# openxrlab/xrslam

Hardware: AMD Instinct MI355X
Metric: frames/sec, full per-frame hot path (KLT tracker + sliding-window VI-BA), one sequence per GPU (higher is better)
Workload: dtype u8/i16 images, f32 LK with exact i64 reductions, f64 BA

## Files before the change

include/xrslam_hip.h:

```cpp
#ifndef XRSLAM_HIP_H
#define XRSLAM_HIP_H

#include <stddef.h>
#include <stdint.h>

#ifdef __cplusplus
extern "C" {
#endif

#define XRHIP_OK 0
#define XRHIP_ENODEVICE (-1)
#define XRHIP_EINVAL (-2)
#define XRHIP_EHIP (-3)
#define XRHIP_ENOMEM (-4)
#define XRHIP_EOVERFLOW (-5)
#define XRHIP_ESTATE (-6)

const char *xrhip_last_error(void);
const char *xrhip_kernel_revision(void);
int xrhip_device_count(void);
int xrhip_set_device(int device);
int xrhip_get_device(int *device);
int xrhip_bind_device(int device);

// ... 35 lines not shown
int xrhip_image_upload_scaled(xrhip_image *img, const void *pixels, int stride_bytes, int format, int bits, int limited_range,
                              int on_device, const xrhip_frame_geometry *geo);
int xrhip_image_upload_scaled_distorted(xrhip_image *img, const void *pixels, int stride_bytes, int format, int bits, int limited_range,
                                        int on_device, const xrhip_frame_geometry *geo);
int xrhip_debug_stream_span(xrhip_klt *ctx, int phase, double *ms);
int xrhip_debug_get_raw(xrhip_image *img, uint8_t *out);
int xrhip_debug_set_fused_pyramid(xrhip_klt *ctx, int on);
int xrhip_debug_get_level_padded(const xrhip_image *img, int level, uint8_t *out, int *rows, int *cols);
void xrhip_image_destroy(xrhip_image *img);

typedef struct xrhip_view_marker { int32_t x, y; uint32_t style; } xrhip_view_marker;
typedef struct xrhip_view_segment { int32_t x0, y0, x1, y1; uint32_t style; } xrhip_view_segment;
int xrhip_image_render_view(xrhip_image *img, const xrhip_view_segment *segs, int n_segs,
                            const xrhip_view_marker *markers, int n_markers,
                            const uint8_t *palette_bgr, int n_palette,
                            void *out, int stride_bytes, int channels, int on_device);
int xrhip_debug_view_timing(xrhip_klt *ctx, int enable, double *ms_sum, long long *n, int reset);

int xrhip_image_preprocess(xrhip_image *img, double clip_limit, int tiles_x, int tiles_y);

int xrhip_image_release(xrhip_image *img);

int xrhip_image_prefetch_detect(xrhip_image *img);
int xrhip_image_detect(xrhip_image *img, const double *existing_xy, int n_exist, int max_points,
                       double min_distance, double *out_xy, int *n_out);

int xrhip_image_track(const xrhip_image *cur, const xrhip_image *next, const double *curr_xy,
                      double *next_xy_inout, int has_guess, uint8_t *status, int n);

int xrhip_image_lk(const xrhip_image *prev, const xrhip_image *next, const float *prev_xy, float *next_xy_inout,
                   uint8_t *status, int n);

int xrhip_image_level_dims(const xrhip_image *img, int level, int *w, int *h);
int xrhip_image_download_level(const xrhip_image *img, int level, uint8_t *img_out, int16_t *deriv_out);
int xrhip_image_download_harris(xrhip_image *img, float *resp_out);

typedef struct xrhip_klt_stats {
    double ms_preprocess;
    double ms_track;
    double ms_detect;
    long long n_preprocess, n_track, n_detect;
    long long lk_templates;
    long long lk_iterations;
    long long lk_points;
    long long detect_full_list;
} xrhip_klt_stats;
typedef struct xrhip_lk_params { int win; int max_level; int max_count; double epsilon; } xrhip_lk_params;
int xrhip_klt_set_lk_params(xrhip_klt *ctx, const xrhip_lk_params *p);
int xrhip_klt_get_lk_params(const xrhip_klt *ctx, xrhip_lk_params *out);
int xrhip_debug_force_general_lk(xrhip_klt *ctx, int on);
int xrhip_klt_set_profiling(xrhip_klt *ctx, int enable);
int xrhip_klt_get_stats(xrhip_klt *ctx, xrhip_klt_stats *out, int reset);
int xrhip_klt_synchronize(xrhip_klt *ctx);


#define XRHIP_STATE_DIM 16
#define XRHIP_ES_DIM 15
#define XRHIP_IMU_DIM 281

#define XRHIP_FIX_POSE 1
#define XRHIP_FIX_MOTION 2

typedef struct xrhip_ba_problem {
    int n_frames;
    double *frame_state;
    const uint8_t *frame_fix;
    double cam_q_bc[4], cam_p_bc[3];
    double imu_q_bi[4], imu_p_bi[3];
    double sqrt_inv_cov[2];
    int n_landmarks;
    double *inv_depth;
    const uint8_t *landmark_fix;
    int n_obs;
    const int *obs_tgt, *obs_ref, *obs_lm;
    const double *obs_z_tgt, *obs_z_ref;
    int n_rot;
    const int *rot_tgt, *rot_ref;
    const double *rot_z_tgt, *rot_z_ref;
    int n_imu;
    const int *imu_i, *imu_j;
    const double *imu_data;
    int prior_n;
    const int *prior_frames;
    const double *prior_sqrt_info;
    const double *prior_infovec;
    const double *prior_lin;
    int max_iterations;
} xrhip_ba_problem;

#define XRHIP_BA_CONVERGENCE 0
#define XRHIP_BA_NO_CONVERGENCE 1
#define XRHIP_BA_FAILURE 2

typedef struct xrhip_ba_summary {
    int iterations;
    int successful_steps;
    int termination;
    int usable;
    double initial_cost, final_cost;
    double ms_solve;
} xrhip_ba_summary;

typedef struct xrhip_marg_problem {
    int n_frames;
    int victim;
    const double *frame_state;
    double cam_q_bc[4], cam_p_bc[3], imu_q_bi[4], imu_p_bi[3], sqrt_inv_cov[2];
    int prior_n;
    const int *prior_frames;
    const double *prior_sqrt_info, *prior_infovec, *prior_lin;
    int n_imu;
    const int *imu_i, *imu_j;
    const double *imu_data;
    int n_landmarks;
    const double *inv_depth;
    int n_obs;
    const int *obs_tgt, *obs_ref, *obs_lm;
    const double *obs_z_tgt, *obs_z_ref;
} xrhip_marg_problem;

typedef struct xrhip_ba xrhip_ba;
int xrhip_ba_create(int max_frames, int max_landmarks, int max_obs, xrhip_ba **out);
void xrhip_ba_destroy(xrhip_ba *ctx);
int xrhip_ba_solve(xrhip_ba *ctx, const xrhip_ba_problem *problem, xrhip_ba_summary *summary);
int xrhip_ba_solve_overlapped(xrhip_ba *ctx, const xrhip_ba_problem *problem, xrhip_ba_summary *summary, void (*host_work)(void *), void *arg);

int xrhip_ba_solve_chained(xrhip_ba *ctx_first, const xrhip_ba_problem *first, xrhip_ba_summary *summary_first, int link_first,
                           xrhip_ba *ctx_second, const xrhip_ba_problem *second, xrhip_ba_summary *summary_second, int link_second,
                           void (*host_work)(void *), void *arg);
int xrhip_ba_solve_begin(xrhip_ba *ctx, const xrhip_ba_problem *first);
int xrhip_ba_solve_linked(xrhip_ba *ctx_second, const xrhip_ba_problem *second, xrhip_ba_summary *summary_second, int link_second,
                          xrhip_ba *ctx_first, int link_first, void (*host_work)(void *), void *arg);
int xrhip_ba_solve_end(xrhip_ba *ctx, xrhip_ba_summary *summary);
int xrhip_ba_solve_abort(xrhip_ba *ctx);

typedef struct xrhip_ba_stats {
    long n_solve_try;
    long n_trials;
    double ms_solve_try;
    long n_timed;
    double flops_solve_try;
    long n_tiny;
    long n_chain_timed;
    double ms_chain;
    double bytes_chain;
    long n_cov_launches;
} xrhip_ba_stats;
int xrhip_ba_set_profiling(xrhip_ba *ctx, int enable);
int xrhip_ba_get_stats(xrhip_ba *ctx, xrhip_ba_stats *out, int reset);
int xrhip_ba_marginalize(xrhip_ba *ctx, const xrhip_marg_problem *problem, double *out_sqrt_info,
                         double *out_infovec, double *out_lin);
int xrhip_ba_marginalize_begin(xrhip_ba *ctx, const xrhip_marg_problem *problem);
int xrhip_ba_marginalize_end(xrhip_ba *ctx, double *out_sqrt_info, double *out_infovec, double *out_lin);
int xrhip_ba_preintegrate(xrhip_ba *ctx, const double *samples, int n, double t_end, const double *bg,
                          const double *ba, const double *noise_cov36, int compute_jacobian,
                          int compute_covariance, double *out);
int xrhip_ba_preintegrate_batch(xrhip_ba *ctx, const double *samples, const int *sample_begin,
                                const int *sample_count, const double *t_end, const double *bg, const double *ba,
                                int n_jobs, const double *noise_cov36, int compute_jacobian, int compute_covariance,
                                double *out);

int xrhip_ba_preintegrate_begin(xrhip_ba *ctx, const double *samples, const int *sample_begin, const int *sample_count,
                                const double *t_end, const double *bg, const double *ba, int n_jobs,
                                const double *noise_cov36, int compute_jacobian, int compute_covariance);
int xrhip_ba_preintegrate_end(xrhip_ba *ctx, double *out);
int xrhip_ba_preintegrate_early(xrhip_ba *ctx, int job, double *out_delta11);
int xrhip_ba_preintegrate_cancel(xrhip_ba *ctx);
int xrhip_ba_preintegrate_after_solve(xrhip_ba *ctx, const double *samples, const int *sample_begin, const int *sample_count,
                                      const double *t_end, const int *bias_frame, int n_jobs, const double *noise_cov36,
                                      int compute_jacobian, int compute_covariance);

typedef struct xrhip_group xrhip_group;
int xrhip_group_create(xrhip_group **out);
int xrhip_group_destroy(xrhip_group *group);
int xrhip_klt_join_group(xrhip_klt *ctx, xrhip_group *group);
int xrhip_ba_join_group(xrhip_ba *ctx, xrhip_group *group);
int xrhip_klt_frame_gate(xrhip_klt *ctx);
int xrhip_klt_group_busy(xrhip_klt *ctx, int busy);
#define XRHIP_GK_CALL 0
#define XRHIP_GK_UPLOAD 1
#define XRHIP_GK_PREPROCESS 2
#define XRHIP_GK_TRACK 3
#define XRHIP_GK_DETECT 4
#define XRHIP_GK_CHAIN 5
#define XRHIP_GK_PREINT 6
#define XRHIP_GK_WROUND 7
#define XRHIP_GK_WTRIALS 8
#define XRHIP_GK_GATE 11
typedef struct xrhip_group_stats {
    long long batches[12];
    long long entries[12];
    double ms[12];
    long long timed[12];
} xrhip_group_stats;
int xrhip_group_set_profiling(xrhip_group *group, int enable);
int xrhip_group_get_stats(xrhip_group *group, xrhip_group_stats *out, int reset);
int xrhip_group_queue_split(xrhip_group *group);

typedef struct xrhip_cov_request {
    int n_sel; const int *sel_frames;
    double *out_blocks;
    double *out_inv_depth_var;
    int *status;
    double *rcond_estimate;
} xrhip_cov_request;
int xrhip_ba_covariance(xrhip_ba *ctx, const xrhip_ba_problem *problem, const xrhip_cov_request *req);
int xrhip_ba_debug_cov_times(xrhip_ba *ctx, double *ms4);

int xrhip_ba_debug_linearize(xrhip_ba *ctx, const xrhip_ba_problem *problem, double *H, double *g, double *hll,
                             double *gl, double *W, double *cost);
int xrhip_ba_debug_schur(xrhip_ba *ctx, const double *W, const double *w, int L, int P, double *out);
int xrhip_ba_debug_marg_guard(xrhip_ba *ctx, double *lambda_bound, int *status8);
int xrhip_ba_debug_set_schur_precision(xrhip_ba *ctx, int mode);
int xrhip_ba_debug_last_route(xrhip_ba *ctx, int *out8);
int xrhip_study_schur_precision(const double *W, const double *w, int L, int P, int reps, double *out64, double *out32,
                                double *out16, float ms_per_launch[3]);
void xrhip_debug_kprof(long long *out32, int reset);
void xrhip_debug_lkprof(long long *out8, int reset);

#ifdef __cplusplus
}
#endif
#endif
```

xrslam_amd/abi.py:

```python
import copy
import ctypes as C

import numpy as np

STATE_DIM = 16
ES_DIM = 15
IMU_DIM = 281
FIX_POSE = 1
FIX_MOTION = 2

_dp = C.POINTER(C.c_double)
_ip = C.POINTER(C.c_int)
_bp = C.POINTER(C.c_uint8)


class BaProblem(C.Structure):
    _fields_ = [
        ("n_frames", C.c_int), ("frame_state", _dp), ("frame_fix", _bp),
        ("cam_q_bc", C.c_double * 4), ("cam_p_bc", C.c_double * 3),
        ("imu_q_bi", C.c_double * 4), ("imu_p_bi", C.c_double * 3),
        ("sqrt_inv_cov", C.c_double * 2),
        ("n_landmarks", C.c_int), ("inv_depth", _dp), ("landmark_fix", _bp),
        ("n_obs", C.c_int), ("obs_tgt", _ip), ("obs_ref", _ip), ("obs_lm", _ip),
        ("obs_z_tgt", _dp), ("obs_z_ref", _dp),
        ("n_rot", C.c_int), ("rot_tgt", _ip), ("rot_ref", _ip), ("rot_z_tgt", _dp), ("rot_z_ref", _dp),
        ("n_imu", C.c_int), ("imu_i", _ip), ("imu_j", _ip), ("imu_data", _dp),
        ("prior_n", C.c_int), ("prior_frames", _ip), ("prior_sqrt_info", _dp), ("prior_infovec", _dp),
        ("prior_lin", _dp),
        ("max_iterations", C.c_int),
    ]


class BaSummary(C.Structure):
    _fields_ = [("iterations", C.c_int), ("successful_steps", C.c_int), ("termination", C.c_int),
                ("usable", C.c_int), ("initial_cost", C.c_double), ("final_cost", C.c_double),
                ("ms_solve", C.c_double)]


class CovRequest(C.Structure):
    _fields_ = [("n_sel", C.c_int), ("sel_frames", _ip), ("out_blocks", _dp), ("out_inv_depth_var", _dp), ("status", _ip),
                ("rcond_estimate", _dp)]


class MargProblem(C.Structure):
    _fields_ = [
        ("n_frames", C.c_int), ("victim", C.c_int), ("frame_state", _dp),
        ("cam_q_bc", C.c_double * 4), ("cam_p_bc", C.c_double * 3),
        ("imu_q_bi", C.c_double * 4), ("imu_p_bi", C.c_double * 3),
        ("sqrt_inv_cov", C.c_double * 2),
        ("prior_n", C.c_int), ("prior_frames", _ip), ("prior_sqrt_info", _dp), ("prior_infovec", _dp),
        ("prior_lin", _dp),
        ("n_imu", C.c_int), ("imu_i", _ip), ("imu_j", _ip), ("imu_data", _dp),
        ("n_landmarks", C.c_int), ("inv_depth", _dp),
        ("n_obs", C.c_int), ("obs_tgt", _ip), ("obs_ref", _ip), ("obs_lm", _ip),
        ("obs_z_tgt", _dp), ("obs_z_ref", _dp),
    ]


def _arr(a, dtype):
    return np.ascontiguousarray(a, dtype=dtype)


def _dpp(a):
    return a.ctypes.data_as(_dp)


def _ipp(a):
    return a.ctypes.data_as(_ip)


class _Factors:

    def _set_obs(self, o):
        o = o or {}
        self.obs_tgt = _arr(o.get("tgt", []), np.int32)
        self.obs_ref = _arr(o.get("ref", []), np.int32)
        self.obs_lm = _arr(o.get("lm", []), np.int32)
        self.obs_z_tgt = _arr(o.get("z_tgt", np.zeros((0, 3))), np.float64).reshape(-1, 3)
        self.obs_z_ref = _arr(o.get("z_ref", np.zeros((0, 3))), np.float64).reshape(-1, 3)

    def _set_imu(self, m):
        m = m or {}
        self.imu_i = _arr(m.get("i", []), np.int32)
        self.imu_j = _arr(m.get("j", []), np.int32)
        self.imu_data = _arr(m.get("data", np.zeros((0, IMU_DIM))), np.float64).reshape(-1, IMU_DIM)

    def _set_prior(self, p):
        p = p or {}
        self.prior_frames = _arr(p.get("frames", []), np.int32)
        n = ES_DIM * len(self.prior_frames)
        self.prior_sqrt_info = _arr(p.get("sqrt_info", np.zeros((n, n))), np.float64).reshape(n, n)
        self.prior_infovec = _arr(p.get("infovec", np.zeros(n)), np.float64)
        self.prior_lin = _arr(p.get("lin", np.zeros((len(self.prior_frames), STATE_DIM))), np.float64)

    def _fill_common(self, s):
        s.cam_q_bc[:] = list(self.cam_ext[:4])
        s.cam_p_bc[:] = list(self.cam_ext[4:7])
        s.imu_q_bi[:] = list(self.imu_ext[:4])
        s.imu_p_bi[:] = list(self.imu_ext[4:7])
        s.sqrt_inv_cov[:] = list(self.sqrt_inv_cov[:2])
        s.n_obs = len(self.obs_tgt)
        s.obs_tgt, s.obs_ref, s.obs_lm = _ipp(self.obs_tgt), _ipp(self.obs_ref), _ipp(self.obs_lm)
        s.obs_z_tgt, s.obs_z_ref = _dpp(self.obs_z_tgt), _dpp(self.obs_z_ref)
        s.n_imu = len(self.imu_i)
        s.imu_i, s.imu_j, s.imu_data = _ipp(self.imu_i), _ipp(self.imu_j), _dpp(self.imu_data)
        s.prior_n = len(self.prior_frames)
        s.prior_frames = _ipp(self.prior_frames)
        s.prior_sqrt_info, s.prior_infovec = _dpp(self.prior_sqrt_info), _dpp(self.prior_infovec)
        s.prior_lin = _dpp(self.prior_lin)


class BaProblemData(_Factors):

    def __init__(self, frame_state, frame_fix, cam_ext, imu_ext, sqrt_inv_cov, inv_depth, landmark_fix=None,
                 obs=None, rot=None, imu=None, prior=None, max_iterations=30):
        self.frame_state = _arr(frame_state, np.float64).reshape(-1, STATE_DIM).copy()
        self.frame_fix = _arr(frame_fix, np.uint8).copy()
        self.cam_ext = _arr(cam_ext, np.float64)
        self.imu_ext = _arr(imu_ext, np.float64)
        self.sqrt_inv_cov = _arr(sqrt_inv_cov, np.float64)
        self.inv_depth = _arr(inv_depth, np.float64).copy()
        nl = len(self.inv_depth)
        self.landmark_fix = _arr(landmark_fix if landmark_fix is not None else np.zeros(nl), np.uint8).copy()
        self._set_obs(obs)
        r = rot or {}
        self.rot_tgt = _arr(r.get("tgt", []), np.int32)
        self.rot_ref = _arr(r.get("ref", []), np.int32)
        self.rot_z_tgt = _arr(r.get("z_tgt", np.zeros((0, 3))), np.float64).reshape(-1, 3)
        self.rot_z_ref = _arr(r.get("z_ref", np.zeros((0, 3))), np.float64).reshape(-1, 3)
        self._set_imu(imu)
        self._set_prior(prior)
        self.max_iterations = int(max_iterations)

    def copy(self):
        return copy.deepcopy(self)

    def struct(self):
        s = BaProblem()
        s.n_frames = len(self.frame_state)
        s.frame_state = _dpp(self.frame_state)
        s.frame_fix = self.frame_fix.ctypes.data_as(_bp)
        s.n_landmarks = len(self.inv_depth)
        s.inv_depth = _dpp(self.inv_depth)
        s.landmark_fix = self.landmark_fix.ctypes.data_as(_bp)
        self._fill_common(s)
        s.n_rot = len(self.rot_tgt)
        s.rot_tgt, s.rot_ref = _ipp(self.rot_tgt), _ipp(self.rot_ref)
        s.rot_z_tgt, s.rot_z_ref = _dpp(self.rot_z_tgt), _dpp(self.rot_z_ref)
        s.max_iterations = self.max_iterations
        return s


class MargProblemData(_Factors):
    def __init__(self, frame_state, victim, cam_ext, imu_ext, sqrt_inv_cov, prior, imu, inv_depth, obs):
        self.frame_state = _arr(frame_state, np.float64).reshape(-1, STATE_DIM).copy()
        self.victim = int(victim)
        self.cam_ext = _arr(cam_ext, np.float64)
        self.imu_ext = _arr(imu_ext, np.float64)
        self.sqrt_inv_cov = _arr(sqrt_inv_cov, np.float64)
        self._set_prior(prior)
        self._set_imu(imu)
        self.inv_depth = _arr(inv_depth, np.float64).copy()
        self._set_obs(obs)

    def struct(self):
        s = MargProblem()
        s.n_frames = len(self.frame_state)
        s.victim = self.victim
        s.frame_state = _dpp(self.frame_state)
        self._fill_common(s)
        s.n_landmarks = len(self.inv_depth)
        s.inv_depth = _dpp(self.inv_depth)
        return s
PIXFMT_GRAY8, PIXFMT_BGR8, PIXFMT_BGRA8, PIXFMT_RGB8, PIXFMT_RGBA8, PIXFMT_GRAY16, PIXFMT_YUYV, PIXFMT_UYVY, PIXFMT_NV12, \
    PIXFMT_I420, PIXFMT_P010 = range(11)
PIXFMT_BYTES = {PIXFMT_GRAY8: 1, PIXFMT_BGR8: 3, PIXFMT_BGRA8: 4, PIXFMT_RGB8: 3, PIXFMT_RGBA8: 4, PIXFMT_GRAY16: 2, PIXFMT_YUYV: 2,
                PIXFMT_UYVY: 2, PIXFMT_NV12: 1, PIXFMT_I420: 1, PIXFMT_P010: 2}


class FrameGeometry(C.Structure):
    _fields_ = [("src_width", C.c_int), ("src_height", C.c_int), ("crop_x", C.c_int), ("crop_y", C.c_int), ("crop_width", C.c_int),
                ("crop_height", C.c_int)]
```

xrslam_amd/ba.py:

```python
import ctypes as C

import numpy as np

from . import _lib, abi
from ._lib import check

_L = None

HOST_WORK = C.CFUNCTYPE(None, C.c_void_p)


def configure(lib):
    vp = C.c_void_p
    lib.xrhip_ba_create.argtypes = [C.c_int, C.c_int, C.c_int, C.POINTER(vp)]
    lib.xrhip_ba_destroy.argtypes = [vp]
    lib.xrhip_ba_destroy.restype = None
    lib.xrhip_ba_solve.argtypes = [vp, C.POINTER(abi.BaProblem), C.POINTER(abi.BaSummary)]
    if hasattr(lib, "xrhip_ba_solve_overlapped"):
        lib.xrhip_ba_solve_overlapped.argtypes = [vp, C.POINTER(abi.BaProblem), C.POINTER(abi.BaSummary), HOST_WORK, vp]
    if hasattr(lib, "xrhip_ba_marginalize"):
        lib.xrhip_ba_marginalize.argtypes = [vp, C.POINTER(abi.MargProblem), vp, vp, vp]
    if hasattr(lib, "xrhip_ba_marginalize_begin"):
        lib.xrhip_ba_marginalize_begin.argtypes = [vp, C.POINTER(abi.MargProblem)]
        lib.xrhip_ba_marginalize_end.argtypes = [vp, vp, vp, vp]
    if hasattr(lib, "xrhip_ba_preintegrate"):
        lib.xrhip_ba_preintegrate.argtypes = [vp, vp, C.c_int, C.c_double, vp, vp, vp, C.c_int, C.c_int, vp]
    if hasattr(lib, "xrhip_ba_preintegrate_begin"):
        lib.xrhip_ba_preintegrate_begin.argtypes = [vp, vp, vp, vp, vp, vp, vp, C.c_int, vp, C.c_int, C.c_int]
    if hasattr(lib, "xrhip_ba_preintegrate_end"):
        lib.xrhip_ba_preintegrate_end.argtypes = [vp, vp]
    if hasattr(lib, "xrhip_ba_preintegrate_early"):
        lib.xrhip_ba_preintegrate_early.argtypes = [vp, C.c_int, vp]
    if hasattr(lib, "xrhip_ba_solve_chained"):
        lib.xrhip_ba_solve_chained.argtypes = [vp, C.POINTER(abi.BaProblem), C.POINTER(abi.BaSummary), C.c_int, vp,
                                               C.POINTER(abi.BaProblem), C.POINTER(abi.BaSummary), C.c_int, HOST_WORK, vp]
    if hasattr(lib, "xrhip_ba_solve_begin"):
        lib.xrhip_ba_solve_begin.argtypes = [vp, C.POINTER(abi.BaProblem)]
        lib.xrhip_ba_solve_end.argtypes = [vp, C.POINTER(abi.BaSummary)]
        lib.xrhip_ba_solve_abort.argtypes = [vp]
    if hasattr(lib, "xrhip_ba_preintegrate_cancel"):
        lib.xrhip_ba_preintegrate_cancel.argtypes = [vp]
    if hasattr(lib, "xrhip_ba_preintegrate_after_solve"):
        lib.xrhip_ba_preintegrate_after_solve.argtypes = [vp, vp, vp, vp, vp, vp, C.c_int, vp, C.c_int, C.c_int]
    if hasattr(lib, "xrhip_ba_debug_linearize"):
        lib.xrhip_ba_debug_linearize.argtypes = [vp, C.POINTER(abi.BaProblem), vp, vp, vp, vp, vp, vp]
    if hasattr(lib, "xrhip_ba_debug_schur"):
        lib.xrhip_ba_debug_schur.argtypes = [vp, vp, vp, C.c_int, C.c_int, vp]
    if hasattr(lib, "xrhip_ba_debug_set_schur_precision"):
        lib.xrhip_ba_debug_set_schur_precision.argtypes = [vp, C.c_int]
    if hasattr(lib, "xrhip_ba_debug_last_route"):
        lib.xrhip_ba_debug_last_route.argtypes = [vp, vp]
    return lib


def L():
    global _L
    if _L is None:
        _L = configure(_lib.lib())
    return _L


def _p(a):
    return a.ctypes.data_as(C.c_void_p)


def study_schur_precision(W, w, reps=20):
    lib = L()
    W = np.ascontiguousarray(W, np.float64)
    w = np.ascontiguousarray(w, np.float64)
    Ln, P = W.shape
    outs = [np.zeros((P, P)) for _ in range(3)]
    ms = (C.c_float * 3)()
    lib.xrhip_study_schur_precision.argtypes = [C.c_void_p, C.c_void_p, C.c_int, C.c_int, C.c_int, C.c_void_p, C.c_void_p,
                                                C.c_void_p, C.POINTER(C.c_float)]
    check(lib.xrhip_study_schur_precision(_p(W), _p(w), Ln, P, int(reps), _p(outs[0]), _p(outs[1]), _p(outs[2]), ms))
    names = ("f64", "f32", "bf16")
    return dict(zip(names, outs)), dict(zip(names, [float(v) for v in ms]))


class BaContext:

    def __init__(self, max_frames=24, max_landmarks=1024, max_obs=8192, lib=None):
        self._lib = lib if lib is not None else L()
        h = C.c_void_p()
        check(self._lib.xrhip_ba_create(int(max_frames), int(max_landmarks), int(max_obs), C.byref(h)))
        self._h = h

    def close(self):
        if getattr(self, "_h", None):
            self._lib.xrhip_ba_destroy(self._h)
            self._h = None

    def __del__(self):
        try:
            self.close()
        except Exception:
            pass

    def solve(self, pd, host_work=None):
        s = pd.struct()
        sm = abi.BaSummary()
        if host_work is None:
            check(self._lib.xrhip_ba_solve(self._h, C.byref(s), C.byref(sm)))
        else:
            raised = []

            def run(_arg):
                try:
                    host_work()
                except BaseException as e:
                    raised.append(e)
            cb = HOST_WORK(run)
            rc = self._lib.xrhip_ba_solve_overlapped(self._h, C.byref(s), C.byref(sm), cb, None)
            if raised:
                raise raised[0]
            check(rc)
        return sm

    def solve_chained(self, pd_first, link_first, second_ctx, pd_second, link_second, host_work=None):
        s1, s2 = pd_first.struct(), pd_second.struct()
        m1, m2 = abi.BaSummary(), abi.BaSummary()
        raised = []

        def run(_arg):
            try:
                if host_work is not None:
                    host_work()
            except BaseException as e:
                raised.append(e)
        cb = HOST_WORK(run)
        rc = self._lib.xrhip_ba_solve_chained(self._h, C.byref(s1), C.byref(m1), int(link_first), second_ctx._h, C.byref(s2),
                                              C.byref(m2), int(link_second), cb, None)
        if raised:
            raise raised[0]
        check(rc)
        return m1, m2

    def solve_begin(self, pd):
        self._begun = (pd, pd.struct())
        rc = self._lib.xrhip_ba_solve_begin(self._h, C.byref(self._begun[1]))
        if rc < 0:
            check(rc)
        return rc == 1

    def solve_end(self):
        sm = abi.BaSummary()
        check(self._lib.xrhip_ba_solve_end(self._h, C.byref(sm)))
        self._begun = None
        return sm

    def solve_abort(self):
        check(self._lib.xrhip_ba_solve_abort(self._h))
        self._begun = None

    def preintegrate_begin(self, samples, t_end, bg, ba, noise36, jac=True, cov=True):
        samples = np.ascontiguousarray(samples, np.float64).reshape(-1, 7)
        bg, ba, noise36 = [np.ascontiguousarray(v, np.float64) for v in (bg, ba, noise36)]
        begin, count = (np.array([v], np.int32) for v in (0, len(samples)))
        t = np.array([t_end], np.float64)
        check(self._lib.xrhip_ba_preintegrate_begin(self._h, _p(samples), _p(begin), _p(count), _p(t), _p(bg), _p(ba), 1, _p(noise36),
                                                    int(jac), int(cov)))

    def preintegrate_early(self, job=0):
        out = np.zeros(11)
        check(self._lib.xrhip_ba_preintegrate_early(self._h, int(job), _p(out)))
        return out

    def marginalize(self, md):
        s = md.struct()
        k = len(md.frame_state) - 1
        n = 15 * k
        si = np.zeros((n, n))
        iv = np.zeros(n)
        lin = np.zeros((k, 16))
        check(self._lib.xrhip_ba_marginalize(self._h, C.byref(s), _p(si), _p(iv), _p(lin)))
        return si, iv, lin

    def marg_guard(self):
        lam = C.c_double()
        st = (C.c_int * 8)()
        self._lib.xrhip_ba_debug_marg_guard.argtypes = [C.c_void_p, C.POINTER(C.c_double), C.POINTER(C.c_int)]
        check(self._lib.xrhip_ba_debug_marg_guard(self._h, C.byref(lam), st))
        return lam.value, list(st)

    def marginalize_begin(self, md):
        self._marg_k = len(md.frame_state) - 1
        check(self._lib.xrhip_ba_marginalize_begin(self._h, C.byref(md.struct())))

    def marginalize_end(self):
        k = self._marg_k
        n = 15 * k
        si = np.zeros((n, n))
        iv = np.zeros(n)
        lin = np.zeros((k, 16))
        check(self._lib.xrhip_ba_marginalize_end(self._h, _p(si), _p(iv), _p(lin)))
        return si, iv, lin

    def preintegrate(self, samples, t_end, bg, ba, noise36, jac=True, cov=True):
        samples = np.ascontiguousarray(samples, np.float64).reshape(-1, 7)
        bg, ba, noise36 = [np.ascontiguousarray(v, np.float64) for v in (bg, ba, noise36)]
        out = np.zeros(abi.IMU_DIM)
        check(self._lib.xrhip_ba_preintegrate(self._h, _p(samples), len(samples), float(t_end), _p(bg), _p(ba), _p(noise36),
                                        int(jac), int(cov), _p(out)))
        return out

    def preintegrate_after_solve(self, samples, t_end, bias_frame, noise36, jac=True, cov=True):
        samples = np.ascontiguousarray(samples, np.float64).reshape(-1, 7)
        noise36 = np.ascontiguousarray(noise36, np.float64)
        begin, count, frame = (np.array([v], np.int32) for v in (0, len(samples), bias_frame))
        t = np.array([t_end], np.float64)
        check(self._lib.xrhip_ba_preintegrate_after_solve(self._h, _p(samples), _p(begin), _p(count), _p(t), _p(frame), 1, _p(noise36),
                                                    int(jac), int(cov)))

    def preintegrate_end(self, n_jobs=1):
        out = np.zeros((n_jobs, abi.IMU_DIM))
        check(self._lib.xrhip_ba_preintegrate_end(self._h, _p(out)))
        return out[0] if n_jobs == 1 else out

    def debug_linearize(self, pd):
        s = pd.struct()
        F, Ln = len(pd.frame_state), len(pd.inv_depth)
        H = np.zeros((15 * F, 15 * F))
        g = np.zeros(15 * F)
        hll = np.zeros(max(Ln, 1))
        gl = np.zeros(max(Ln, 1))
        W = np.zeros((max(Ln, 1), 6 * F))
        cost = C.c_double()
        check(self._lib.xrhip_ba_debug_linearize(self._h, C.byref(s), _p(H), _p(g), _p(hll), _p(gl), _p(W), C.byref(cost)))
        return dict(H=H, g=g, hll=hll[:Ln], gl=gl[:Ln], W=W[:Ln], cost=cost.value)

    def covariance(self, pd, sel, landmarks=False, prefill=None):
        sel = np.ascontiguousarray(sel, np.int32).reshape(-1)
        fill = np.nan if prefill is None else prefill
        blocks = np.full((len(sel), 15, 15), fill)
        var = np.full(max(len(pd.inv_depth), 1), fill) if landmarks else None
        status = np.full(1, -1, np.int32)
        rcond = np.zeros(1)
        s = pd.struct()
        rq = abi.CovRequest(len(sel), sel.ctypes.data_as(C.POINTER(C.c_int)), blocks.ctypes.data_as(C.POINTER(C.c_double)),
                            var.ctypes.data_as(C.POINTER(C.c_double)) if landmarks else None,
                            status.ctypes.data_as(C.POINTER(C.c_int)), rcond.ctypes.data_as(C.POINTER(C.c_double)))
        self._lib.xrhip_ba_covariance.argtypes = [C.c_void_p, C.POINTER(abi.BaProblem), C.POINTER(abi.CovRequest)]
        check(self._lib.xrhip_ba_covariance(self._h, C.byref(s), C.byref(rq)))
        return dict(blocks=blocks, var=var[:len(pd.inv_depth)] if landmarks else None, status=int(status[0]), rcond=float(rcond[0]))

    def stats(self, reset=False):
        from .harness.runner import BaStats
        st = BaStats()
        self._lib.xrhip_ba_get_stats.argtypes = [C.c_void_p, C.c_void_p, C.c_int]
        check(self._lib.xrhip_ba_get_stats(self._h, C.byref(st), 1 if reset else 0))
        return st

    def cov_times(self):
        out = np.zeros(4)
        self._lib.xrhip_ba_debug_cov_times.argtypes = [C.c_void_p, C.c_void_p]
        check(self._lib.xrhip_ba_debug_cov_times(self._h, _p(out)))
        return out

    ROUTES = {0: "none", 1: "tiny", 2: "chain", 3: "small_mid", 4: "multi"}

    def debug_last_route(self):
        out = np.zeros(8, np.int32)
        check(self._lib.xrhip_ba_debug_last_route(self._h, _p(out)))
        v = [int(x) for x in out]
        return dict(route=self.ROUTES[v[0]], use_lds=v[1], sred_tiled=v[2], block=v[3], wide_trials=v[4], wide_first=v[5], na=v[6],
                    F=v[7])

    def set_schur_precision(self, mode):
        check(self._lib.xrhip_ba_debug_set_schur_precision(self._h, int(mode)))

    def debug_schur(self, W, w):
        W = np.ascontiguousarray(W, np.float64)
        w = np.ascontiguousarray(w, np.float64)
        Ln, P = W.shape
        out = np.zeros((P, P))
        check(self._lib.xrhip_ba_debug_schur(self._h, _p(W), _p(w), Ln, P, _p(out)))
        return out
```

xrslam_amd/csrc/ba_api.hip:

```cpp
#include "../../include/xrslam_hip.h"
#include "ba_kernels.hip.h"
#include "ba_chain.hip.h"
#include "ba_plan.hpp"
#include "marg_kernels.hip.h"
#include "cov_kernels.hip.h"
#include "host/covariance.hpp"
#include "common.hip.h"
#include "group.hip.h"

#include <cstdlib>
#include <chrono>
#include <algorithm>
#include <cmath>
#include <cstring>
#include <limits>
#include <vector>

using namespace xrhip;

namespace {

struct Arena {
    char *dev = nullptr, *host = nullptr;
    size_t cap = 0, used = 0;
    size_t take(size_t bytes) {
        size_t off = (used + 255) & ~size_t(255);
        used = off + bytes;
        return off;
    }
};

inline int round_up(int v, int m) { return (v + m - 1) / m * m; }

struct ChainPayload {
    StageArgs stage;
    ChainArgs chain;
    size_t lds = 0;
    bool with_preint = false;
    PreintArgs preint;
};
struct ChainSubmitted {
    int seq = 0;
    hipStream_t stream = nullptr;
    GroupRequest *rq = nullptr;
    hipEvent_t e0 = nullptr, e1 = nullptr;
};
struct WindowPayload {
    WinEntry e;
    bool relin = false;
    bool with_stage = false;
    StageArgs stage;
    int np = 0;
    gptr<const double> pS, pinfo;
    gptr<double> pLam, pc0;
    size_t lds_lin = 0, lds_solve = 0, lds_wide = 0;
};

}

struct xrhip_ba {
    hipStream_t stream = nullptr;
    int device = 0;
    xrhip_group *group = nullptr;
    GroupRequest rq_chain, rq_preint, rq_window;
    WindowPayload a_window;
    ChainPayload a_chain;
    PreintArgs a_preint;
    GroupRequest *preint_rq = nullptr;
    hipStream_t preint_stream = nullptr;
    struct Begun {
        bool active = false;
        const xrhip_ba_problem *P = nullptr;
        BaDims d{};
        SolvePlan plan;
        BaPtrs p{};
        ChainSubmitted sub;
        std::chrono::steady_clock::time_point t0;
        bool handed_over = false;
        std::chrono::steady_clock::time_point t_hand;
    } begun;
    Arena in;
    char *work = nullptr;
    size_t work_cap = 0;
    char *work2 = nullptr;
    size_t work2_cap = 0;
    char *h_stage = nullptr;
    size_t h_stage_cap = 0;
    BaCtl *h_ctl = nullptr;
    int *h_seq = nullptr;
    int seq = 0;
    struct MargPending {
        bool pending = false;
        int K = 0, victim = 0, R = 0;
        std::vector<double> lin;
        int *dst = nullptr, *dsup = nullptr;
        double *lam = nullptr;
        double *As = nullptr, *bs = nullptr, *B = nullptr, *V = nullptr, *Ss = nullptr, *ivs = nullptr, *dsi = nullptr, *div = nullptr;
    } marg;
    int preint_pending = 0;
    size_t preint_o_out = 0, preint_o_st = 0;
    int preint_deferred = 0, preint_def_jac = 0, preint_def_cov = 0;
    size_t preint_o_jobs = 0, preint_o_smp = 0, preint_o_noise = 0;
    bool profiling = false;
    struct Timed {
        hipEvent_t e0, e1;
        double flops_fixed, flops_per_trial;
        int iter_before;
    };
    std::vector<Timed> pending;
    struct TimedChain {
        hipEvent_t e0, e1;
        double bytes;
    };
    std::vector<TimedChain> pending_chain;
    std::vector<std::pair<hipEvent_t, hipEvent_t>> free_events;
    xrhip_ba_stats stats = {0, 0, 0.0, 0, 0.0, 0, 0, 0.0, 0.0, 0};
    char *cov_dev = nullptr;
    size_t cov_cap = 0;
    hipEvent_t cov_ev[5] = {nullptr, nullptr, nullptr, nullptr, nullptr};
    double cov_ms[4] = {0.0, 0.0, 0.0, 0.0};
    const TinyArgs *tiny_args = nullptr;
    hipStream_t stream2 = nullptr;
    hipEvent_t ev_mid = nullptr, ev_spec = nullptr;
    hipEvent_t ev_marg = nullptr;
    char *work_spec = nullptr;
    size_t work_spec_cap = 0;
    bool spec_outstanding = false;
    long spec_launched = 0, spec_taken = 0;
    const uint4 *stage_src = nullptr;
    uint4 *stage_dst = nullptr;
    size_t stage_n16 = 0;
    void (*overlap_fn)(void *) = nullptr;
    void *overlap_arg = nullptr;
    double *h_out = nullptr;
    size_t h_out_cap = 0;
    int lds_limit = 150 * 1024;
    int schur_mode = 0;
    SolvePlan plan;
    BaDims dims{};
    BaPtrs ptrs{};
    bool have_lin = false;
};

static int ensure_arena(xrhip_ba *c, size_t in_bytes, size_t work_bytes, size_t out_doubles) {
    if (in_bytes > c->in.cap) {
        if (c->in.dev) hipFree(c->in.dev);
        if (c->in.host) hipHostFree(c->in.host);
        c->in.dev = c->in.host = nullptr;
        size_t cap = std::max(in_bytes * 2, size_t(1) << 20);
        XR_HIP(hipMalloc(&c->in.dev, cap));
        XR_HIP(hipHostMalloc(&c->in.host, cap, hipHostMallocDefault));
        c->in.cap = cap;
    }
    if (work_bytes > c->work_cap) {
        if (c->work) hipFree(c->work);
        c->work = nullptr;
        size_t cap = std::max(work_bytes * 2, size_t(1) << 20);
        XR_HIP(hipMalloc(&c->work, cap));
        c->work_cap = cap;
    }
    if (out_doubles > c->h_out_cap) {
        if (c->h_out) hipHostFree(c->h_out);
        c->h_out = nullptr;
        XR_HIP(hipHostMalloc(&c->h_out, sizeof(double) * out_doubles * 2, hipHostMallocDefault));
        c->h_out_cap = out_doubles * 2;
    }
    return XRHIP_OK;
}

static int validate(const xrhip_ba_problem *P) {
    if (!P || P->n_frames <= 0 || !P->frame_state || !P->frame_fix) return xr_fail(XRHIP_EINVAL, "xrhip_ba_solve: frames missing");
    if (P->n_landmarks < 0 || P->n_obs < 0 || P->n_rot < 0 || P->n_imu < 0 || P->prior_n < 0)
        return xr_fail(XRHIP_EINVAL, "xrhip_ba_solve: negative count");
    for (int o = 0; o < P->n_obs; ++o)
        if (P->obs_tgt[o] < 0 || P->obs_tgt[o] >= P->n_frames || P->obs_ref[o] < 0 || P->obs_ref[o] >= P->n_frames ||
            P->obs_lm[o] < 0 || P->obs_lm[o] >= P->n_landmarks || P->obs_tgt[o] == P->obs_ref[o])
            return xr_fail(XRHIP_EINVAL, "xrhip_ba_solve: observation index out of range");
    for (int o = 0; o < P->n_rot; ++o)
        if (P->rot_tgt[o] < 0 || P->rot_tgt[o] >= P->n_frames || P->rot_ref[o] < 0 || P->rot_ref[o] >= P->n_frames)
            return xr_fail(XRHIP_EINVAL, "xrhip_ba_solve: rotation factor index out of range");
    for (int k = 0; k < P->n_imu; ++k)
        if (P->imu_i[k] < 0 || P->imu_i[k] >= P->n_frames || P->imu_j[k] < 0 || P->imu_j[k] >= P->n_frames ||
            P->imu_i[k] == P->imu_j[k])
            return xr_fail(XRHIP_EINVAL, "xrhip_ba_solve: imu factor index out of range");
    for (int k = 0; k < P->prior_n; ++k)
        if (P->prior_frames[k] < 0 || P->prior_frames[k] >= P->n_frames)
            return xr_fail(XRHIP_EINVAL, "xrhip_ba_solve: prior frame index out of range");
    return XRHIP_OK;
}

static int launch_stage_copy(xrhip_ba *c, hipStream_t s) {
    const int blocks = (int)std::min<size_t>((c->stage_n16 + 255) / 256, 128);
    Batch<StageArgs> b;
    std::memset(&b, 0, sizeof(b));
    b.e[0] = StageArgs{c->stage_src, c->stage_dst, c->stage_n16};
    hipLaunchKernelGGL(kb_stage, dim3(blocks, 1, 1), dim3(256), 0, s, b);
    XR_HIP(hipGetLastError());
    return XRHIP_OK;
}

static int launch_preint_batch(GroupRequest **r, int n, hipStream_t s, hipStream_t = nullptr) {
    for (int base = 0; base < n; base += XB) {
        const int m = std::min(XB, n - base);
        Batch<PreintArgs> b;
        std::memset(&b, 0, sizeof(b));
        int most = 1;
        for (int i = 0; i < m; ++i) {
            b.e[i] = *static_cast<const PreintArgs *>(r[base + i]->payload);
            most = std::max(most, b.e[i].n_jobs);
        }
        hipLaunchKernelGGL(kp_preintegrate, dim3(most, 1, m), dim3(PI_NT), 0, s, b);
    }
    XR_HIP(hipGetLastError());
    return XRHIP_OK;
}

static int launch_chain_batch(GroupRequest **r, int n, hipStream_t s, hipStream_t = nullptr) {
    std::vector<StageArgs> stages;
    std::vector<std::pair<ChainArgs, size_t>> first, second;
    std::vector<PreintArgs> preints;
    for (int i = 0; i < n; ++i) {
        const ChainPayload &p = *static_cast<const ChainPayload *>(r[i]->payload);
        stages.push_back(p.stage);
        (p.chain.link_src ? second : first).emplace_back(p.chain, p.lds);
        if (p.with_preint) preints.push_back(p.preint);
    }
    for (size_t base = 0; base < stages.size(); base += XB) {
        const int m = (int)std::min<size_t>(XB, stages.size() - base);
        Batch<StageArgs> bs;
        std::memset(&bs, 0, sizeof(bs));
        size_t most16 = 0;
        for (int i = 0; i < m; ++i) {
            bs.e[i] = stages[base + i];
            most16 = std::max(most16, bs.e[i].n16);
        }
        hipLaunchKernelGGL(kb_stage, dim3((int)std::min<size_t>((most16 + 255) / 256, 128), 1, m), dim3(256), 0, s, bs);
    }
    for (const auto *list : {&first, &second})
        for (size_t base = 0; base < list->size(); base += XB) {
            const int m = (int)std::min<size_t>(XB, list->size() - base);
            Batch<ChainArgs> bc;
            std::memset(&bc, 0, sizeof(bc));
            size_t lds = 0;
            for (int i = 0; i < m; ++i) {
                bc.e[i] = (*list)[base + i].first;
                lds = std::max(lds, (*list)[base + i].second);
            }
            hipLaunchKernelGGL(kb_chain, dim3(1, 1, m), dim3(CHAIN_THREADS), lds, s, bc);
        }
    for (size_t base = 0; base < preints.size(); base += XB) {
        const int m = (int)std::min<size_t>(XB, preints.size() - base);
        Batch<PreintArgs> bp;
        std::memset(&bp, 0, sizeof(bp));
        int most_jobs = 1;
        for (int i = 0; i < m; ++i) {
            bp.e[i] = preints[base + i];
            most_jobs = std::max(most_jobs, bp.e[i].n_jobs);
        }
        hipLaunchKernelGGL(kp_preintegrate, dim3(most_jobs, 1, m), dim3(PI_NT), 0, s, bp);
    }
    XR_HIP(hipGetLastError());
    return XRHIP_OK;
}

static int launch_wround_batch(GroupRequest **r, int n, hipStream_t s, hipStream_t = nullptr) {
    for (int base = 0; base < n; base += XB) {
        const int m = std::min(XB, n - base);
        const WindowPayload *w[XB];
        for (int i = 0; i < m; ++i) w[i] = static_cast<const WindowPayload *>(r[base + i]->payload);
        Batch<StageArgs> bs;
        std::memset(&bs, 0, sizeof(bs));
        size_t most16 = 0;
        for (int i = 0; i < m; ++i)
            if (w[i]->with_stage) {
                bs.e[i] = w[i]->stage;
                most16 = std::max(most16, bs.e[i].n16);
            }
        if (most16) hipLaunchKernelGGL(kb_stage, dim3((int)std::min<size_t>((most16 + 255) / 256, 128), 1, m), dim3(256), 0, s, bs);
        for (int i = 0; i < m; ++i)
            if (w[i]->with_stage && w[i]->np) {
                const int np = w[i]->np;
                hipLaunchKernelGGL(kb_prior_lambda, dim3(((np + 15) / 16) * ((np + 15) / 16 + 1)), dim3(256), 0, s, np, w[i]->pS, w[i]->pLam, w[i]->pinfo,
                                   w[i]->pc0);
            }
        Batch<WinEntry> b;
        std::memset(&b, 0, sizeof(b));
        int g_lin = 0, g_lv = 0, g_asm = 0, g_sa = 0;
        size_t lds_lin = 0, lds_solve = 0, lds_wide = 0;
        for (int i = 0; i < m; ++i) {
            b.e[i] = w[i]->e;
            if (!w[i]->relin) b.e[i].g_lin = b.e[i].g_lv = b.e[i].g_asm = 0;
            g_lin = std::max(g_lin, b.e[i].g_lin);
            g_lv = std::max(g_lv, b.e[i].g_lv);
            g_asm = std::max(g_asm, b.e[i].g_asm);
            g_sa = std::max(g_sa, b.e[i].g_sa);
            lds_lin = std::max(lds_lin, w[i]->lds_lin);
            lds_solve = std::max(lds_solve, w[i]->lds_solve);
            lds_wide = std::max(lds_wide, w[i]->lds_wide);
        }
        if (g_lin) {
            hipLaunchKernelGGL(kw_lin_all, dim3(g_lin, 1, m), dim3(256), lds_lin, s, b);
            hipLaunchKernelGGL(kw_landmark_vision, dim3(std::max(g_lv, 1), 1, m), dim3(64), 0, s, b);
            hipLaunchKernelGGL(kw_assemble, dim3(std::max(g_asm, 1), 1, m), dim3(256), 0, s, b);
        }
        hipLaunchKernelGGL(kw_prepare, dim3(1, 1, m), dim3(256), 0, s, b);
        hipLaunchKernelGGL(kw_schur_aux, dim3(std::max(g_sa, 1), 1, m), dim3(256), 0, s, b);
        hipLaunchKernelGGL(kw_solve_try, dim3(1, 1, m), dim3(512), lds_solve, s, b);
        for (int i = 0; i < m; ++i) b.e[i].first = 1;
        hipLaunchKernelGGL(kw_trials_wide, dim3(WIDE_G, 1, m), dim3(256), lds_wide, s, b);
    }
    XR_HIP(hipGetLastError());
    return XRHIP_OK;
}
static int launch_wtrials_batch(GroupRequest **r, int n, hipStream_t s, hipStream_t = nullptr) {
    for (int base = 0; base < n; base += XB) {
        const int m = std::min(XB, n - base);
        Batch<WinEntry> b;
        std::memset(&b, 0, sizeof(b));
        size_t lds_wide = 0;
        for (int i = 0; i < m; ++i) {
            const WindowPayload *w = static_cast<const WindowPayload *>(r[base + i]->payload);
            b.e[i] = w->e;
            b.e[i].first = 0;
            b.e[i].mode = 0;
            lds_wide = std::max(lds_wide, w->lds_wide);
        }
        hipLaunchKernelGGL(kw_trials_wide, dim3(WIDE_G, 1, m), dim3(256), lds_wide, s, b);
    }
    XR_HIP(hipGetLastError());
    return XRHIP_OK;
}

namespace {
struct RegisterBaLaunchers {
    RegisterBaLaunchers() {
        group_register(GK_PREINT, launch_preint_batch);
        group_register(GK_CHAIN, launch_chain_batch);
        group_register(GK_WROUND, launch_wround_batch);
        group_register(GK_WTRIALS, launch_wtrials_batch);
    }
} g_register_ba_launchers;
}

static int stage_problem(xrhip_ba *c, const xrhip_ba_problem *P, BaDims &d, SolvePlan &pl, BaPtrs &p, Ext &cam, Ext &imu, bool defer_copy = false) {
    d.F = P->n_frames;
    d.n = 15 * d.F;
    d.PF = round_up(6 * d.F, 16);
    d.L = P->n_landmarks;
    d.Lp = std::max(16, round_up(d.L, 16));
    d.M = P->n_obs;
    d.MR = P->n_rot;
    d.NI = P->n_imu;
    d.NP = P->prior_n;
    d.np = 15 * d.NP;
    d.NV = d.n + d.L;
    d.robust = 1;
    d.schur_mode = c->schur_mode;
    const int F = d.F, L = d.L, M = d.M, MR = d.MR, NI = d.NI, NP = d.NP, np = d.np, n = d.n;

    std::vector<uint8_t> lact(std::max(L, 1), 0);
    for (int o = 0; o < M; ++o) lact[P->obs_lm[o]] = 1;
    for (int l = 0; l < L; ++l)
        if (P->landmark_fix && P->landmark_fix[l]) lact[l] = 0;
    std::vector<int> lm_start(L + 1, 0), lm_obs(std::max(M, 1));
    for (int o = 0; o < M; ++o) lm_start[P->obs_lm[o] + 1]++;
    for (int l = 0; l < L; ++l) lm_start[l + 1] += lm_start[l];
    {
        std::vector<int> fill(lm_start.begin(), lm_start.end() - 1);
        for (int o = 0; o < M; ++o) lm_obs[fill[P->obs_lm[o]]++] = o;
    }
    std::vector<int> pair_start((size_t)F * F + 1, 0), pair_items(std::max(4 * M, 1));
    auto pair_count = [&](int a, int b) { pair_start[(size_t)a * F + b + 1]++; };
    for (int o = 0; o < M; ++o) {
        const int t = P->obs_tgt[o], r = P->obs_ref[o];
        pair_count(t, t);
        pair_count(r, r);
        pair_count(t, r);
        pair_count(r, t);
    }
    for (size_t i = 0; i < (size_t)F * F; ++i) pair_start[i + 1] += pair_start[i];
    {
        std::vector<int> fill(pair_start.begin(), pair_start.end() - 1);
        for (int o = 0; o < M; ++o) {
            const int t = P->obs_tgt[o], r = P->obs_ref[o];
            pair_items[fill[(size_t)t * F + t]++] = (o << 1) | 0;
            pair_items[fill[(size_t)r * F + r]++] = (o << 1) | 1;
            pair_items[fill[(size_t)t * F + r]++] = (o << 1) | 0;
            pair_items[fill[(size_t)r * F + t]++] = (o << 1) | 1;
        }
    }
    std::vector<int> rotf_start(F + 1, 0), rotf_items(std::max(MR, 1));
    for (int o = 0; o < MR; ++o) rotf_start[P->rot_tgt[o] + 1]++;
    for (int f = 0; f < F; ++f) rotf_start[f + 1] += rotf_start[f];
    {
        std::vector<int> fill(rotf_start.begin(), rotf_start.end() - 1);
        for (int o = 0; o < MR; ++o) rotf_items[fill[P->rot_tgt[o]]++] = o;
    }
    std::vector<int> act_idx;
    for (int a = 0; a < 15 * F; ++a) {
        const int f = a / 15, k = a % 15;
        if (k < 6 ? !(P->frame_fix[f] & XRHIP_FIX_POSE) : !(P->frame_fix[f] & XRHIP_FIX_MOTION)) act_idx.push_back(a);
    }
    d.na = (int)act_idx.size();
    std::vector<int> act_inv((size_t)15 * F, -1);
    for (size_t i = 0; i < act_idx.size(); ++i) act_inv[act_idx[i]] = (int)i;
    d.nla = 0;
    for (int l = 0; l < L; ++l) d.nla += lact[l] ? 1 : 0;
    d.lm_rows = d.Lp;
    d.nfree = 0;
    for (int f = 0; f < F; ++f) d.nfree += (P->frame_fix[f] & 3) != 3 ? 1 : 0;
    d.nffp = 0;
    for (int o = 0; o < M; ++o)
        d.nffp += (!(P->frame_fix[P->obs_tgt[o]] & XRHIP_FIX_POSE) && !(P->frame_fix[P->obs_ref[o]] & XRHIP_FIX_POSE)) ? 1 : 0;
    std::vector<int> imuf(2 * F, -1), priorf(F, -1);
    for (int k = 0; k < NI; ++k) {
        if (imuf[2 * P->imu_j[k]] >= 0 || imuf[2 * P->imu_i[k] + 1] >= 0)
            return xr_fail(XRHIP_EINVAL, "xrhip_ba_solve: a frame may end at most one IMU factor and start at most one");
        imuf[2 * P->imu_j[k]] = k;
        imuf[2 * P->imu_i[k] + 1] = k;
    }
    for (int k = 0; k < NP; ++k) priorf[P->prior_frames[k]] = k;

    Arena &A = c->in;
    A.used = 0;
    struct Item {
        size_t off;
        const void *src;
        size_t bytes;
    };
    std::vector<Item> items;
    auto put = [&](const void *src, size_t bytes) {
        size_t off = A.take(std::max(bytes, size_t(8)));
        items.push_back({off, src, bytes});
        return off;
    };
    std::vector<double> bias_ref((size_t)6 * std::max(NI, 1));
    for (int k = 0; k < NI; ++k)
        for (int i = 0; i < 6; ++i) bias_ref[6 * k + i] = P->frame_state[16 * P->imu_i[k] + 10 + i];
    BaCtl ctl;
    std::memset(&ctl, 0, sizeof(ctl));
    ctl.radius = 1e4;
    ctl.mu = 1e-8;
    ctl.first = 1;
    ctl.linear_ok = 1;
    ctl.max_iterations = P->max_iterations;
    ctl.termination = XRHIP_BA_NO_CONVERGENCE;
    ctl.accepted_slot = -1;
    const size_t o_state = put(P->frame_state, sizeof(double) * 16 * F);
    const size_t o_fix = put(P->frame_fix, F);
    const size_t o_depth = put(P->inv_depth, sizeof(double) * L);
    const size_t o_lact = put(lact.data(), std::max(L, 1));
    const size_t o_ot = put(P->obs_tgt, sizeof(int) * M), o_or = put(P->obs_ref, sizeof(int) * M);
    const size_t o_ol = put(P->obs_lm, sizeof(int) * M);
    const size_t o_zt = put(P->obs_z_tgt, sizeof(double) * 3 * M), o_zr = put(P->obs_z_ref, sizeof(double) * 3 * M);
    const size_t o_rt = put(P->rot_tgt, sizeof(int) * MR), o_rr = put(P->rot_ref, sizeof(int) * MR);
    const size_t o_rzt = put(P->rot_z_tgt, sizeof(double) * 3 * MR), o_rzr = put(P->rot_z_ref, sizeof(double) * 3 * MR);
    const size_t o_ii = put(P->imu_i, sizeof(int) * NI), o_ij = put(P->imu_j, sizeof(int) * NI);
    const size_t o_idata = put(P->imu_data, sizeof(double) * XRHIP_IMU_DIM * NI);
    const size_t o_bref = put(bias_ref.data(), sizeof(double) * 6 * NI);
    const size_t o_pf = put(P->prior_frames, sizeof(int) * NP);
    const size_t o_pS = put(P->prior_sqrt_info, sizeof(double) * (size_t)np * np);
    const size_t o_pi = put(P->prior_infovec, sizeof(double) * np);
    const size_t o_pl = put(P->prior_lin, sizeof(double) * 16 * NP);
    const size_t o_lms = put(lm_start.data(), sizeof(int) * (L + 1)), o_lmo = put(lm_obs.data(), sizeof(int) * M);
    const size_t o_ps = put(pair_start.data(), sizeof(int) * ((size_t)F * F + 1));
    const size_t o_pit = put(pair_items.data(), sizeof(int) * 4 * M);
    const size_t o_rfs = put(rotf_start.data(), sizeof(int) * (F + 1)), o_rfi = put(rotf_items.data(), sizeof(int) * MR);
    const size_t o_imuf = put(imuf.data(), sizeof(int) * 2 * F), o_prf = put(priorf.data(), sizeof(int) * F);
    const size_t o_act = put(act_idx.data(), sizeof(int) * act_idx.size());
    const size_t o_ainv = put(act_inv.data(), sizeof(int) * act_inv.size());
    const size_t o_ctl = put(&ctl, sizeof(ctl));
    const size_t o_args = put(nullptr, sizeof(TinyArgs));
    const size_t in_bytes = A.used + 256;

    size_t w = 0;
    auto carve = [&](size_t bytes) {
        size_t off = (w + 255) & ~size_t(255);
        w = off + std::max(bytes, size_t(8));
        return off;
    };
    const size_t D8 = sizeof(double);
    const size_t w_cand = carve(D8 * 16 * F * TRY_B), w_dcand = carve(D8 * L * TRY_B);
    const size_t w_pLam = carve(D8 * (size_t)np * np), w_pc0 = carve(D8 * np);
    const size_t w_orec = carve(D8 * OREC * M), w_ocost = carve(D8 * M);
    const size_t w_rrec = carve(D8 * RREC * MR), w_rcost = carve(D8 * MR);
    const size_t w_ir = carve(D8 * 15 * NI), w_iJi = carve(D8 * 225 * NI), w_iJj = carve(D8 * 225 * NI);
    const size_t w_ic = carve(D8 * NI);
    const size_t w_pr = carve(D8 * np), w_pt = carve(D8 * np), w_pJq = carve(D8 * 9 * NP), w_pc = carve(D8 * (1 + (np + 15) / 16));
    const size_t w_H = carve(D8 * (size_t)n * n), w_g = carve(D8 * n);
    const size_t w_hll = carve(D8 * d.Lp), w_gl = carve(D8 * d.Lp), w_Wt = carve(D8 * (size_t)d.Lp * d.PF);
    const size_t w_sp = carve(D8 * n), w_sl = carve(D8 * d.Lp), w_om = carve(D8 * d.Lp);
    const size_t w_T = carve(D8 * (size_t)d.PF * d.PF), w_S = carve(D8 * (size_t)n * n);
    const size_t w_dD = carve(D8 * d.NV), w_gr = carve(D8 * d.NV), w_gn = carve(D8 * d.NV), w_gs = carve(D8 * d.NV);
    const size_t w_st = carve(D8 * d.NV), w_de = carve(D8 * d.NV * TRY_B), w_part = carve(D8 * (size_t)(aux_quad_blocks_n(d.n, std::max(d.L, 1)) + 8));
    const size_t w_wog = carve(D8 * d.PF * WOG_CH);
    const size_t w_wide = carve(D8 * WIDE_G * 4 * WIDE_B);
    const size_t w_Hv = carve(D8 * 36 * (size_t)F * F * VIS_CH), w_gv = carve(D8 * 6 * F * VIS_CH);
    int rc = ensure_arena(c, in_bytes, w + 256, (size_t)16 * F + L + 8);
    if (rc) return rc;
    for (const Item &it : items)
        if (it.bytes && it.src) std::memcpy(A.host + it.off, it.src, it.bytes);

    char *I = A.dev, *W = c->work;
    p.state = (double *)(I + o_state);
    p.cand = (double *)(W + w_cand);
    p.fix = (const uint8_t *)(I + o_fix);
    p.depth = (double *)(I + o_depth);
    p.depth_cand = (double *)(W + w_dcand);
    p.lact = (const uint8_t *)(I + o_lact);
    p.obs_tgt = (const int *)(I + o_ot);
    p.obs_ref = (const int *)(I + o_or);
    p.obs_lm = (const int *)(I + o_ol);
    p.obs_zt = (const double *)(I + o_zt);
    p.obs_zr = (const double *)(I + o_zr);
    p.rot_tgt = (const int *)(I + o_rt);
    p.rot_ref = (const int *)(I + o_rr);
    p.rot_zt = (const double *)(I + o_rzt);
    p.rot_zr = (const double *)(I + o_rzr);
    p.imu_i = (const int *)(I + o_ii);
    p.imu_j = (const int *)(I + o_ij);
    p.imu_data = (const double *)(I + o_idata);
    p.bias_ref = (double *)(I + o_bref);
    p.prior_frames = (const int *)(I + o_pf);
    p.pS = (const double *)(I + o_pS);
    p.pinfo = (const double *)(I + o_pi);
    p.plin = (const double *)(I + o_pl);
    p.pLam = (double *)(W + w_pLam);
    p.pc0 = (double *)(W + w_pc0);
    p.lm_start = (const int *)(I + o_lms);
    p.lm_obs = (const int *)(I + o_lmo);
    p.pair_start = (const int *)(I + o_ps);
    p.pair_items = (const int *)(I + o_pit);
    p.rotf_start = (const int *)(I + o_rfs);
    p.rotf_items = (const int *)(I + o_rfi);
    p.imuf = (const int *)(I + o_imuf);
    p.priorf = (const int *)(I + o_prf);
    p.act_idx = (const int *)(I + o_act);
    p.act_inv = (const int *)(I + o_ainv);
    p.Hv = (double *)(W + w_Hv);
    p.gv = (double *)(W + w_gv);
    p.orec = (double *)(W + w_orec);
    p.ocost = (double *)(W + w_ocost);
    p.rrec = (double *)(W + w_rrec);
    p.rcost = (double *)(W + w_rcost);
    p.imu_r = (double *)(W + w_ir);
    p.imu_Ji = (double *)(W + w_iJi);
    p.imu_Jj = (double *)(W + w_iJj);
    p.imu_cost = (double *)(W + w_ic);
    p.pr = (double *)(W + w_pr);
    p.pt = (double *)(W + w_pt);
    p.pJq = (double *)(W + w_pJq);
    p.pcost = (double *)(W + w_pc);
    p.Hpp = (double *)(W + w_H);
    p.gp = (double *)(W + w_g);
    p.hll = (double *)(W + w_hll);
    p.gl = (double *)(W + w_gl);
    p.Wt = (double *)(W + w_Wt);
    p.sp = (double *)(W + w_sp);
    p.sl = (double *)(W + w_sl);
    p.omega = (double *)(W + w_om);
    p.T = (double *)(W + w_T);
    p.Sred = (double *)(W + w_S);
    p.diagD = (double *)(W + w_dD);
    p.grad = (double *)(W + w_gr);
    p.gn = (double *)(W + w_gn);
    p.gs = (double *)(W + w_gs);
    p.step = (double *)(W + w_st);
    p.delta = (double *)(W + w_de);
    p.partial = (double *)(W + w_part);
    p.wog = (double *)(W + w_wog);
    p.wide_part = (double *)(W + w_wide);
    p.ctl = (BaCtl *)(I + o_ctl);
    XR_HIP(hipHostGetDevicePointer((void **)&p.host_ctl, c->h_ctl, 0));
    XR_HIP(hipHostGetDevicePointer((void **)&p.host_out, c->h_out, 0));
    XR_HIP(hipHostGetDevicePointer((void **)&p.host_seq, c->h_seq, 0));
    cam.q = Q4{P->cam_q_bc[0], P->cam_q_bc[1], P->cam_q_bc[2], P->cam_q_bc[3]};
    cam.p = V3{P->cam_p_bc[0], P->cam_p_bc[1], P->cam_p_bc[2]};
    imu.q = Q4{P->imu_q_bi[0], P->imu_q_bi[1], P->imu_q_bi[2], P->imu_q_bi[3]};
    imu.p = V3{P->imu_p_bi[0], P->imu_p_bi[1], P->imu_p_bi[2]};
    pl = plan_solve(d, (size_t)c->lds_limit, ba_switches());
    d.sred_tiled = pl.sred_tiled;
    {
        TinyArgs *ta = reinterpret_cast<TinyArgs *>(A.host + o_args);
        ta->d = d;
        ta->p = p;
        ta->cam = cam;
        ta->imu = imu;
        ta->sx = P->sqrt_inv_cov[0];
        ta->sy = P->sqrt_inv_cov[1];
        c->tiny_args = reinterpret_cast<const TinyArgs *>(I + o_args);
    }
    {
        char *host_dev = nullptr;
        XR_HIP(hipHostGetDevicePointer((void **)&host_dev, A.host, 0));
        c->stage_src = (const uint4 *)host_dev;
        c->stage_dst = (uint4 *)A.dev;
        c->stage_n16 = (in_bytes + 15) / 16;
        if (!defer_copy) return launch_stage_copy(c, c->stream);
    }
    return XRHIP_OK;
}

static int landmark_vision_blocks(const BaDims &d) { return d.lm_rows + d.F * d.F * VIS_CH; }
static int assemble_blocks(const BaDims &d) { return (d.n * d.n + 255) / 256; }
static size_t lin_all_lds(const BaDims &d) { return sizeof(double) * (size_t)std::max(d.np, 1); }
static int schur_aux_blocks(const BaDims &d) {
    const int tiles = d.PF / 16;
    const int nrest = sred_rest_blocks(d);
    return nrest + (d.nla ? tiles * tiles + aux_quad_blocks_n(d.n, d.L) + aux_wog_blocks(d.F) : aux_quad_blocks_n(d.n, d.L)) + 1;
}

static void launch_linearize(xrhip_ba *c, const BaDims &d, const SolvePlan &pl, const BaPtrs &p, const Ext &cam, const Ext &imu, double sx,
                             double sy, bool for_solver) {
    hipStream_t s = c->stream;
    hipLaunchKernelGGL(kb_lin_all, dim3(lin_all_blocks(d.M, d.MR, d.NI, d.np)), dim3(256), lin_all_lds(d), s, d, p, cam, imu, sx, sy);
    hipLaunchKernelGGL(kb_landmark_vision, dim3(landmark_vision_blocks(d)), dim3(64), 0, s, d, p);
    if (for_solver && pl.route == ROUTE_SMALL_MID) return;
    hipLaunchKernelGGL(kb_assemble, dim3(assemble_blocks(d)), dim3(256), 0, s, d, p);
    if (for_solver) hipLaunchKernelGGL(kb_prepare, dim3(1), dim3(256), 0, s, d, p);
    else hipLaunchKernelGGL(kb_sum_cost, dim3(1), dim3(256), 0, s, d, p);
}

constexpr int LINEARIZE_LAUNCHES = 4;

static void launch_schur_aux(const BaDims &d, const BaPtrs &p, hipStream_t s) {
    hipLaunchKernelGGL(kb_schur_aux, dim3(schur_aux_blocks(d)), dim3(256), 0, s, d, p);
}

static int take_event_pair(xrhip_ba *c, hipEvent_t *e0, hipEvent_t *e1) {
    if (!c->free_events.empty()) {
        *e0 = c->free_events.back().first;
        *e1 = c->free_events.back().second;
        c->free_events.pop_back();
    } else {
        XR_HIP(hipEventCreate(e0));
        XR_HIP(hipEventCreate(e1));
    }
    return XRHIP_OK;
}

static int launch_solve_try(xrhip_ba *c, const BaDims &d, const SolvePlan &pl, const BaPtrs &p, const Ext &cam, const Ext &imu, double sx,
                            double sy, bool prepare, int mode, int seq, bool skip_front = false, const BaPtrs *spec_set = nullptr) {
    const bool mark_mid = spec_set != nullptr;
    const int commit = (spec_set && skip_front) ? 1 : 0;
    double *state2 = spec_set ? static_cast<double *>(spec_set->state) : nullptr;
    double *depth2 = spec_set ? static_cast<double *>(spec_set->depth) : nullptr;
    BaCtl *ctl2 = spec_set ? static_cast<BaCtl *>(spec_set->ctl) : nullptr;
    hipStream_t s = c->stream;
    const bool mid = pl.route == ROUTE_SMALL_MID;
    if (!skip_front) {
        if (mid) hipLaunchKernelGGL(kb_small_mid, dim3(1), dim3(256), 0, s, d, p, prepare ? 0 : 1);
        if (!mid && prepare) hipLaunchKernelGGL(kb_prepare, dim3(1), dim3(256), 0, s, d, p);
        if (!mid) launch_schur_aux(d, p, s);
    }
    const size_t lds = pl.try_lds;
    const int use_lds = pl.use_lds, wide = pl.wide_trials ? 1 : 0;
    hipEvent_t e0 = nullptr, e1 = nullptr;
    if (c->profiling) {
        int rc = take_event_pair(c, &e0, &e1);
        if (rc) return rc;
        XR_HIP(hipEventRecord(e0, s));
    }
    if (pl.wide_first)
        hipLaunchKernelGGL((kb_solve_try<512, true>), dim3(1), dim3(512), lds, s, d, p, cam, imu, sx, sy, use_lds, mode, seq, 2, state2, depth2, ctl2, commit);
    else if (pl.block == 256)
        hipLaunchKernelGGL((kb_solve_try<256, false>), dim3(1), dim3(256), lds, s, d, p, cam, imu, sx, sy, use_lds, mode, seq, wide,
                           (double *)nullptr, (double *)nullptr, (BaCtl *)nullptr, 0);
    else
        hipLaunchKernelGGL((kb_solve_try<512, false>), dim3(1), dim3(512), lds, s, d, p, cam, imu, sx, sy, use_lds, mode, seq, wide,
                           (double *)nullptr, (double *)nullptr, (BaCtl *)nullptr, 0);
    XR_HIP(hipGetLastError());
    if (c->profiling) XR_HIP(hipEventRecord(e1, s));
    if (pl.wide_first) {
        hipStream_t st = s;
        if (mark_mid) {
            XR_HIP(hipEventRecord(c->ev_mid, s));
            XR_HIP(hipStreamWaitEvent(c->stream2, c->ev_mid, 0));
            st = c->stream2;
        }
        hipLaunchKernelGGL(kb_trials_wide, dim3(WIDE_G), dim3(256), pl.wide_lds, st, d, p, cam, imu, sx, sy, seq, 1, mode);
        XR_HIP(hipGetLastError());
    }
    if (c->profiling) {
        const double na = d.na;
        c->pending.push_back({e0, e1, na * na * na / 3.0 + 2.0 * na * na,
                              pl.wide_first ? 0.0 : 450.0 * d.M + 3000.0 * d.NI + 2.0 * (double)d.np * d.np, -1});
    }
    c->stats.n_solve_try++;
    return XRHIP_OK;
}

static void run_overlap(xrhip_ba *c) {
    if (!c->overlap_fn) return;
    void (*fn)(void *) = c->overlap_fn;
    c->overlap_fn = nullptr;
    fn(c->overlap_arg);
}
static int wait_mailbox(xrhip_ba *c, int seq, hipStream_t publisher = nullptr, GroupRequest *rq = nullptr) {
    run_overlap(c);
    return wait_flag(c->h_seq, seq, publisher ? publisher : c->stream, rq, "xrhip_ba_solve");
}

static long long g_kprof[32];
static void kprof_accumulate(const BaCtl &ctl, int na) {
    static const int min_na = std::getenv("XRHIP_KPROF_MIN_NA") ? std::atoi(std::getenv("XRHIP_KPROF_MIN_NA")) : 0;
    static const int max_na = std::getenv("XRHIP_KPROF_MAX_NA") ? std::atoi(std::getenv("XRHIP_KPROF_MAX_NA")) : 1 << 30;
    if (na < min_na || na > max_na) return;
    for (int i = 0; i < 31; ++i) g_kprof[i] += ctl.prof[i];
    g_kprof[31] += 1;
}

extern "C" {

static void ba_resolve_pending(xrhip_ba *c) {
    for (auto &t : c->pending) {
        float ms = 0.f;
        if (hipEventSynchronize(t.e1) == hipSuccess && hipEventElapsedTime(&ms, t.e0, t.e1) == hipSuccess) {
            c->stats.ms_solve_try += ms;
            c->stats.n_timed += 1;
            c->stats.flops_solve_try += t.flops_fixed + t.flops_per_trial * std::max(t.iter_before, 0);
        }
        c->free_events.push_back({t.e0, t.e1});
    }
    c->pending.clear();
    for (auto &t : c->pending_chain) {
        float ms = 0.f;
        if (hipEventSynchronize(t.e1) == hipSuccess && hipEventElapsedTime(&ms, t.e0, t.e1) == hipSuccess) {
            c->stats.ms_chain += ms;
            c->stats.n_chain_timed += 1;
            c->stats.bytes_chain += t.bytes;
        }
        c->free_events.push_back({t.e0, t.e1});
    }
    c->pending_chain.clear();
}

int xrhip_ba_set_profiling(xrhip_ba *c, int enable) {
    if (!c) return xr_fail(XRHIP_EINVAL, "xrhip_ba_set_profiling: null context");
    if (!enable) ba_resolve_pending(c);
    c->profiling = enable != 0;
    return XRHIP_OK;
}

int xrhip_ba_get_stats(xrhip_ba *c, xrhip_ba_stats *out, int reset) {
    if (!c || !out) return xr_fail(XRHIP_EINVAL, "xrhip_ba_get_stats: null argument");
    ba_resolve_pending(c);
    *out = c->stats;
    if (reset) c->stats = {0, 0, 0.0, 0, 0.0, 0, 0, 0.0, 0.0, 0};
    return XRHIP_OK;
}

void xrhip_debug_kprof(long long *out32, int reset) {
    for (int i = 0; i < 32; ++i) {
        if (out32) out32[i] = g_kprof[i];
        if (reset) g_kprof[i] = 0;
    }
}

int xrhip_ba_create(int max_frames, int max_landmarks, int max_obs, xrhip_ba **out) {
    if (!out || max_frames <= 0 || max_landmarks < 0 || max_obs < 0) return xr_fail(XRHIP_EINVAL, "xrhip_ba_create: bad arguments");
    int rc = xr_require_device();
    if (rc) return rc;
    xrhip_ba *c = new xrhip_ba();
    XR_HIP(hipGetDevice(&c->device));
    XR_HIP(hipStreamCreateWithFlags(&c->stream, hipStreamNonBlocking));
    XR_HIP(hipStreamCreateWithFlags(&c->stream2, hipStreamNonBlocking));
    XR_HIP(hipEventCreateWithFlags(&c->ev_mid, hipEventDisableTiming));
    XR_HIP(hipEventCreateWithFlags(&c->ev_spec, hipEventDisableTiming));
    XR_HIP(hipHostMalloc(&c->h_ctl, sizeof(BaCtl), hipHostMallocDefault));
    XR_HIP(hipHostMalloc(&c->h_seq, 64, hipHostMallocDefault));
    *c->h_seq = 0;
    XR_HIP(hipFuncSetAttribute((const void *)kb_solve_try<512, true>, hipFuncAttributeMaxDynamicSharedMemorySize, c->lds_limit));
    XR_HIP(hipFuncSetAttribute((const void *)kb_solve_try<512, false>, hipFuncAttributeMaxDynamicSharedMemorySize, c->lds_limit));
    XR_HIP(hipFuncSetAttribute((const void *)kb_solve_try<256, false>, hipFuncAttributeMaxDynamicSharedMemorySize, c->lds_limit));
    XR_HIP(hipFuncSetAttribute((const void *)kb_chain, hipFuncAttributeMaxDynamicSharedMemorySize, c->lds_limit));
    XR_HIP(hipFuncSetAttribute((const void *)kb_trials_wide, hipFuncAttributeMaxDynamicSharedMemorySize, c->lds_limit));
    XR_HIP(hipFuncSetAttribute((const void *)kw_solve_try, hipFuncAttributeMaxDynamicSharedMemorySize, c->lds_limit));
    XR_HIP(hipFuncSetAttribute((const void *)kw_trials_wide, hipFuncAttributeMaxDynamicSharedMemorySize, c->lds_limit));
    XR_HIP(hipFuncSetAttribute((const void *)km_chol, hipFuncAttributeMaxDynamicSharedMemorySize, c->lds_limit));
    XR_HIP(hipFuncSetAttribute((const void *)km_jacobi, hipFuncAttributeMaxDynamicSharedMemorySize, c->lds_limit));
    size_t in_guess = (size_t)max_obs * 96 + (size_t)max_frames * max_frames * 15 * 15 * 8 + (size_t)max_frames * 3000 + 65536;
    rc = ensure_arena(c, in_guess, in_guess * 4, (size_t)16 * max_frames + max_landmarks + 8);
    if (rc) return rc;
    *out = c;
    return XRHIP_OK;
}

int xrhip_ba_join_group(xrhip_ba *c, xrhip_group *g) {
    if (!c) return xr_fail(XRHIP_EINVAL, "xrhip_ba_join_group: null context");
    if (c->group == g) return XRHIP_OK;
    if (g && group_device(g) != c->device)
        return xr_fail(XRHIP_EINVAL, "xrhip_ba_join_group: the context and the group live on different devices");
    if (c->preint_pending) {
        if (c->preint_rq) {
            int rc = group_wait_launched(c->preint_rq);
            if (rc) return rc;
        }
        XR_HIP(hipStreamSynchronize(c->preint_stream ? c->preint_stream : c->stream));
        c->preint_rq = nullptr;
        c->preint_stream = c->stream;
    }
    XR_HIP(hipStreamSynchronize(c->stream));
    if (c->group) {
        int rc = group_drain(c->group, GQ_CHAIN, c);
        if (!rc) rc = group_drain(c->group, GQ_PREINT, c);
        if (!rc) rc = group_drain(c->group, GQ_WINDOW, c);
        if (rc) return rc;
        group_member_remove(c->group, false);
    }
    c->group = g;
    if (g) group_member_add(g, false);
    return XRHIP_OK;
}

void xrhip_ba_destroy(xrhip_ba *c) {
    if (!c) return;
    if (c->begun.active) xrhip_ba_solve_abort(c);
    if (c->group) {
        xrhip_ba_preintegrate_cancel(c);
        xrhip_ba_join_group(c, nullptr);
    }
    hipStreamSynchronize(c->stream);
    if (c->stream2) hipStreamSynchronize(c->stream2);
    if (std::getenv("XRHIP_HOSTPROF") && c->spec_launched)
        std::fprintf(stderr, "[hostprof] speculative linearisations: %ld launched, %ld taken\n", c->spec_launched, c->spec_taken);
    hipFree(c->work_spec);
    hipFree(c->cov_dev);
    for (hipEvent_t e : c->cov_ev)
        if (e) hipEventDestroy(e);
    if (c->ev_mid) hipEventDestroy(c->ev_mid);
    if (c->ev_marg) hipEventDestroy(c->ev_marg);
    if (c->ev_spec) hipEventDestroy(c->ev_spec);
    if (c->stream2) hipStreamDestroy(c->stream2);
    hipFree(c->in.dev);
    hipHostFree(c->in.host);
    hipFree(c->work);
    hipFree(c->work2);
    hipHostFree(c->h_stage);
    hipHostFree(c->h_ctl);
    hipHostFree(c->h_seq);
    ba_resolve_pending(c);
    for (auto &e : c->free_events) {
        hipEventDestroy(e.first);
        hipEventDestroy(e.second);
    }
    hipHostFree(c->h_out);
    hipStreamDestroy(c->stream);
    delete c;
}

static int preint_launch_deferred(xrhip_ba *c, const xrhip_ba_problem *P, const double *state_dev);
static int preint_fill_deferred(xrhip_ba *c, const xrhip_ba_problem *P, const double *state_dev, PreintArgs *out, bool *have);

static int ba_solve_impl(xrhip_ba *c, const xrhip_ba_problem *P, xrhip_ba_summary *summary);
int xrhip_ba_solve(xrhip_ba *c, const xrhip_ba_problem *P, xrhip_ba_summary *summary) {
    if (!c) return xr_fail(XRHIP_EINVAL, "xrhip_ba_solve: null context");
    if (c->begun.active) return xr_fail(XRHIP_ESTATE, "xrhip_ba_solve: a solve begun on this context has not been collected (xrhip_ba_solve_end)");
    const int rc = ba_solve_impl(c, P, summary);
    if (rc) c->preint_deferred = 0;
    return rc;
}
int xrhip_ba_solve_overlapped(xrhip_ba *c, const xrhip_ba_problem *P, xrhip_ba_summary *summary, void (*host_work)(void *), void *arg) {
    if (!c) return xr_fail(XRHIP_EINVAL, "xrhip_ba_solve_overlapped: null context");
    c->overlap_fn = host_work;
    c->overlap_arg = arg;
    const int rc = xrhip_ba_solve(c, P, summary);
    run_overlap(c);
    return rc;
}
static int preint_deferred_check(xrhip_ba *c, const xrhip_ba_problem *P) {
    const PreintJob *jobs = (const PreintJob *)(c->h_stage + c->preint_o_jobs);
    for (int k = 0; k < c->preint_deferred; ++k)
        if (jobs[k].bias_frame < 0 || jobs[k].bias_frame >= P->n_frames) {
            c->preint_deferred = 0;
            return xr_fail(XRHIP_EINVAL, "xrhip_ba_preintegrate_after_solve: bias frame is not a frame of the solve");
        }
    return XRHIP_OK;
}

static bool any_free_block(const xrhip_ba_problem *P) {
    for (int f = 0; f < P->n_frames; ++f)
        if ((P->frame_fix[f] & 3) != 3) return true;
    return false;
}
static bool inputs_finite(const xrhip_ba_problem *P) {
    bool ok = true;
    for (int i = 0; i < 16 * P->n_frames; ++i) ok &= std::isfinite(P->frame_state[i]);
    for (int o = 0; o < P->n_obs; ++o) ok &= std::isfinite(P->inv_depth[P->obs_lm[o]]);
    return ok;
}
static void refuse_summary(xrhip_ba_summary *sm) {
    if (!sm) return;
    std::memset(sm, 0, sizeof(*sm));
    sm->termination = XRHIP_BA_FAILURE;
    sm->usable = 0;
    sm->initial_cost = sm->final_cost = std::numeric_limits<double>::quiet_NaN();
}
static void fill_summary(const BaCtl &ctl, float ms, xrhip_ba_summary *sm) {
    if (!sm) return;
    std::memset(sm, 0, sizeof(*sm));
    sm->iterations = ctl.iteration;
    sm->successful_steps = ctl.successful_steps;
    sm->termination = ctl.termination;
    sm->usable = ctl.termination != XRHIP_BA_FAILURE;
    sm->initial_cost = ctl.initial_cost;
    sm->final_cost = ctl.x_cost;
    sm->ms_solve = ms;
}
static float ms_since(std::chrono::steady_clock::time_point t0, std::chrono::steady_clock::time_point t1 = std::chrono::steady_clock::now()) {
    return std::chrono::duration<float, std::milli>(t1 - t0).count();
}

static double chain_bytes(const BaDims &d, const BaCtl &ctl) {
    const double nf = (double)d.M + d.MR, rounds = ctl.successful_steps + 1.0, trials = ctl.iteration;
    return rounds * (384.0 * nf + 8.0 * (double)d.na * d.na + 2248.0 * d.NI) + trials * (280.0 * nf + 2248.0 * d.NI);
}

static int submit_chain(xrhip_ba *c, const xrhip_ba_problem *P, const SolvePlan &pl, const BaPtrs &p, const double *link_src, int link_dst,
                        hipStream_t own_stream, xrhip_ba *timed, ChainSubmitted *out) {
    int rc = c->group ? group_wait_launched(&c->rq_chain) : XRHIP_OK;
    if (rc) return rc;
    ChainPayload &cp = c->a_chain;
    rc = preint_fill_deferred(c, P, p.state, &cp.preint, &cp.with_preint);
    if (rc) return rc;
    ChainSubmitted sub;
    sub.seq = ++c->seq;
    cp.stage = StageArgs{c->stage_src, c->stage_dst, c->stage_n16};
    cp.chain = ChainArgs{c->tiny_args, sub.seq, 4 * (P->max_iterations + 8), pl.chain_opts, link_src, link_dst};
    cp.lds = pl.chain_lds;
    c->rq_chain.kind = GK_CHAIN;
    c->rq_chain.owner = c;
    c->rq_chain.payload = &cp;
    c->plan = pl;
    if (c->group) {
        sub.stream = group_stream(c->group, GQ_CHAIN);
        sub.rq = &c->rq_chain;
        rc = group_submit(c->group, GQ_CHAIN, &c->rq_chain);
        if (rc) return rc;
    } else {
        sub.stream = own_stream;
        if (timed->profiling) {
            rc = take_event_pair(timed, &sub.e0, &sub.e1);
            if (rc) return rc;
        }
        rc = launch_stage_copy(c, sub.stream);
        if (rc) return rc;
        Batch<ChainArgs> bc;
        std::memset(&bc, 0, sizeof(bc));
        bc.e[0] = cp.chain;
        if (sub.e0) XR_HIP(hipEventRecord(sub.e0, sub.stream));
        hipLaunchKernelGGL(kb_chain, dim3(1, 1, 1), dim3(CHAIN_THREADS), cp.lds, sub.stream, bc);
        XR_HIP(hipGetLastError());
        if (sub.e1) XR_HIP(hipEventRecord(sub.e1, sub.stream));
        if (cp.with_preint) {
            GroupRequest one;
            one.payload = &cp.preint;
            GroupRequest *pone = &one;
            rc = launch_preint_batch(&pone, 1, sub.stream);
            if (rc) return rc;
        }
    }
    if (cp.with_preint) {
        c->preint_pending = c->preint_deferred;
        c->preint_deferred = 0;
        c->preint_rq = sub.rq;
        c->preint_stream = sub.stream;
    }
    *out = sub;
    return XRHIP_OK;
}

static int collect_chain(xrhip_ba *c, const xrhip_ba_problem *P, const BaDims &d, const BaPtrs &p, const ChainSubmitted &sub, xrhip_ba *timed,
                         const char *who) {
    if (c->h_ctl->status != ST_DONE) {
        char msg[128];
        std::snprintf(msg, sizeof(msg), "%s: trust-region loop did not terminate", who);
        return xr_fail(XRHIP_ESTATE, msg);
    }
    std::memcpy(P->frame_state, c->h_out, sizeof(double) * 16 * d.F);
    const double bytes = chain_bytes(d, *c->h_ctl);
    if (sub.e0) {
        timed->pending_chain.push_back({sub.e0, sub.e1, bytes});
    } else if (c->profiling && c->group) {
        c->stats.n_chain_timed++;
        c->stats.bytes_chain += bytes;
    }
    c->stats.n_tiny++;
    kprof_accumulate(*c->h_ctl, d.na);
    c->dims = d;
    c->ptrs = p;
    c->have_lin = true;
    return XRHIP_OK;
}

int xrhip_ba_solve_begin(xrhip_ba *c, const xrhip_ba_problem *P) {
    if (!c || !P) return xr_fail(XRHIP_EINVAL, "xrhip_ba_solve_begin: null argument");
    if (c->begun.active) return xr_fail(XRHIP_ESTATE, "xrhip_ba_solve_begin: a solve is already in flight on this context");
    int rc = validate(P);
    if (rc) return rc;
    const BaSwitches &sw = ba_switches();
    if (sw.no_chained_solves || (c->group && !sw.group_chained_solves) || c->preint_deferred || !any_free_block(P) || !inputs_finite(P))
        return 0;
    xrhip_ba::Begun &B = c->begun;
    B.t0 = std::chrono::steady_clock::now();
    Ext cam, imu;
    rc = stage_problem(c, P, B.d, B.plan, B.p, cam, imu, true);
    if (rc) return rc;
    if (B.plan.route != ROUTE_CHAIN) return 0;
    rc = submit_chain(c, P, B.plan, B.p, nullptr, -1, c->stream, c, &B.sub);
    if (rc) return rc;
    B.P = P;
    B.active = true;
    B.handed_over = false;
    return 1;
}

int xrhip_ba_solve_end(xrhip_ba *c, xrhip_ba_summary *summary) {
    if (!c) return xr_fail(XRHIP_EINVAL, "xrhip_ba_solve_end: null context");
    xrhip_ba::Begun &B = c->begun;
    if (!B.active) return xr_fail(XRHIP_ESTATE, "xrhip_ba_solve_end: nothing in flight");
    B.active = false;
    int rc = wait_flag(c->h_seq, B.sub.seq, B.sub.stream, B.sub.rq, "xrhip_ba_solve_end");
    if (rc) return rc;
    rc = collect_chain(c, B.P, B.d, B.p, B.sub, c, "xrhip_ba_solve_end");
    if (rc) return rc;
    fill_summary(*c->h_ctl, B.handed_over ? ms_since(B.t0, B.t_hand) : ms_since(B.t0), summary);
    B.handed_over = false;
    return XRHIP_OK;
}

int xrhip_ba_solve_abort(xrhip_ba *c) {
    if (!c) return xr_fail(XRHIP_EINVAL, "xrhip_ba_solve_abort: null context");
    xrhip_ba::Begun &B = c->begun;
    if (!B.active) return XRHIP_OK;
    B.active = false;
    if (B.sub.rq) group_wait_launched(B.sub.rq);
    XR_HIP(hipStreamSynchronize(B.sub.stream));
    if (B.sub.e0) c->free_events.push_back({B.sub.e0, B.sub.e1});
    return XRHIP_OK;
}

int xrhip_ba_solve_linked(xrhip_ba *c2, const xrhip_ba_problem *P2, xrhip_ba_summary *s2, int link_second, xrhip_ba *c1, int link_first,
                          void (*host_work)(void *), void *arg) {
    if (!c1 || !c2 || c1 == c2 || !P2) return xr_fail(XRHIP_EINVAL, "xrhip_ba_solve_linked: two distinct contexts and a problem are needed");
    xrhip_ba::Begun &A = c1->begun;
    if (!A.active) return xr_fail(XRHIP_ESTATE, "xrhip_ba_solve_linked: the first context has no solve in flight (xrhip_ba_solve_begin)");
    int rc = validate(P2);
    if (rc) return rc;
    if (link_first < 0 || link_first >= A.d.F || link_second < 0 || link_second >= P2->n_frames)
        return xr_fail(XRHIP_EINVAL, "xrhip_ba_solve_linked: linked frame is not a frame of its problem");
    auto sequential = [&]() {
        int r = wait_flag(c1->h_seq, A.sub.seq, A.sub.stream, A.sub.rq, "xrhip_ba_solve_linked");
        if (r) return r;
        std::memcpy(P2->frame_state + 16 * (size_t)link_second, c1->h_out + 16 * (size_t)link_first, sizeof(double) * 16);
        return xrhip_ba_solve_overlapped(c2, P2, s2, host_work, arg);
    };
    if (c1->group != c2->group || c2->begun.active || !any_free_block(P2) || !inputs_finite(P2)) return sequential();
    const auto t_begin = std::chrono::steady_clock::now();
    BaDims d2;
    SolvePlan pl2;
    BaPtrs p2;
    Ext cam2, imu2;
    rc = stage_problem(c2, P2, d2, pl2, p2, cam2, imu2, true);
    if (rc) return rc;
    if (pl2.route != ROUTE_CHAIN) return sequential();
    ChainSubmitted sub;
    rc = submit_chain(c2, P2, pl2, p2, static_cast<const double *>(A.p.state) + 16 * (size_t)link_first, link_second, A.sub.stream, c1, &sub);
    if (rc) return rc;
    A.handed_over = true;
    A.t_hand = t_begin;
    if (host_work) host_work(arg);
    rc = wait_flag(c2->h_seq, sub.seq, sub.stream, sub.rq, "xrhip_ba_solve_linked");
    if (rc) return rc;
    rc = collect_chain(c2, P2, d2, p2, sub, c1, "xrhip_ba_solve_linked");
    if (rc) return rc;
    fill_summary(*c2->h_ctl, ms_since(t_begin), s2);
    return XRHIP_OK;
}

int xrhip_ba_solve_chained(xrhip_ba *c1, const xrhip_ba_problem *P1, xrhip_ba_summary *s1, int link_first, xrhip_ba *c2,
                           const xrhip_ba_problem *P2, xrhip_ba_summary *s2, int link_second, void (*host_work)(void *), void *arg) {
    if (!c1 || !c2 || c1 == c2 || !P1 || !P2) return xr_fail(XRHIP_EINVAL, "xrhip_ba_solve_chained: two distinct contexts and two problems are needed");
    int rc = validate(P1);
    if (!rc) rc = validate(P2);
    if (rc) return rc;
    if (link_first < 0 || link_first >= P1->n_frames || link_second < 0 || link_second >= P2->n_frames)
        return xr_fail(XRHIP_EINVAL, "xrhip_ba_solve_chained: linked frame is not a frame of its problem");
    const int begun = xrhip_ba_solve_begin(c1, P1);
    if (begun < 0) return begun;
    if (begun == 0) {
        rc = xrhip_ba_solve_overlapped(c1, P1, s1, host_work, arg);
        if (rc) return rc;
        std::memcpy(P2->frame_state + 16 * (size_t)link_second, P1->frame_state + 16 * (size_t)link_first, sizeof(double) * 16);
        return xrhip_ba_solve(c2, P2, s2);
    }
    rc = xrhip_ba_solve_linked(c2, P2, s2, link_second, c1, link_first, host_work, arg);
    const int rc1 = xrhip_ba_solve_end(c1, s1);
    return rc ? rc : rc1;
}

static int ba_solve_impl(xrhip_ba *c, const xrhip_ba_problem *P, xrhip_ba_summary *summary) {
    int rc = validate(P);
    if (rc) return rc;
    rc = preint_deferred_check(c, P);
    if (rc) return rc;
    c->plan = SolvePlan{};
    c->plan.F = P->n_frames;
    bool any_free = any_free_block(P);
    if (!any_free) {
        std::vector<char> used(std::max(P->n_landmarks, 1), 0);
        for (int o = 0; o < P->n_obs; ++o) used[P->obs_lm[o]] = 1;
        for (int l = 0; l < P->n_landmarks; ++l)
            if (used[l] && !(P->landmark_fix && P->landmark_fix[l])) any_free = true;
    }
    if (!any_free) {
        if (summary) {
            std::memset(summary, 0, sizeof(*summary));
            summary->termination = XRHIP_BA_CONVERGENCE;
            summary->usable = 1;
        }
        return preint_launch_deferred(c, P, nullptr);
    }
    if (!inputs_finite(P)) {
        refuse_summary(summary);
        return preint_launch_deferred(c, P, nullptr);
    }
    BaDims d;
    SolvePlan pl;
    BaPtrs p;
    Ext cam, imu;
    const auto t_begin = std::chrono::steady_clock::now();
    {
        HostProfScope hp(8, "ba_solve: stage_problem");
        rc = stage_problem(c, P, d, pl, p, cam, imu, true);
    }
    if (rc) return rc;
    HostProfScope hp_rounds(9, "ba_solve: rounds (launch+wait)");
    if (pl.route == ROUTE_CHAIN) {
        ChainSubmitted sub;
        rc = submit_chain(c, P, pl, p, nullptr, -1, c->stream, c, &sub);
        if (rc) return rc;
        rc = wait_mailbox(c, sub.seq, sub.stream, sub.rq);
        if (rc) return rc;
        rc = collect_chain(c, P, d, p, sub, c, "xrhip_ba_solve");
        if (rc) return rc;
        fill_summary(*c->h_ctl, ms_since(t_begin), summary);
        return XRHIP_OK;
    }
    c->plan = pl;
    const BaSwitches &sw = ba_switches();
    const bool wbatch = c->group && !sw.group_no_window_batch && pl.wide_first && d.nla > 0 && !sw.group_spec;
    if (!wbatch) {
        rc = launch_stage_copy(c, c->stream);
        if (rc) return rc;
    }
    if (!d.nla) d.lm_rows = 0;
    const double sx = P->sqrt_inv_cov[0], sy = P->sqrt_inv_cov[1];
    hipStream_t s = c->stream;
    if (d.np && !wbatch) hipLaunchKernelGGL(kb_prior_lambda, dim3(((d.np + 15) / 16) * ((d.np + 15) / 16 + 1)), dim3(256), 0, s, d.np, p.pS, p.pLam, p.pinfo, p.pc0);
    bool done = false, relinearise = true;
    bool wfirst = true;
    hipStream_t wstream = wbatch ? group_stream(c->group, GQ_WINDOW) : nullptr;
    auto submit_window = [&](int kind, int seq_, int mode_) -> int {
        int r = group_wait_launched(&c->rq_window);
        if (r) return r;
        WindowPayload &wp = c->a_window;
        wp.e = WinEntry{c->tiny_args, lin_all_blocks(d.M, d.MR, d.NI, d.np), landmark_vision_blocks(d), assemble_blocks(d), schur_aux_blocks(d),
                        pl.use_lds, mode_, seq_, 1};
        wp.relin = relinearise;
        wp.with_stage = wfirst;
        wp.stage = StageArgs{c->stage_src, c->stage_dst, c->stage_n16};
        wp.np = d.np;
        wp.pS = p.pS;
        wp.pLam = p.pLam;
        wp.pinfo = p.pinfo;
        wp.pc0 = p.pc0;
        wp.lds_lin = lin_all_lds(d);
        wp.lds_solve = pl.try_lds;
        wp.lds_wide = pl.wide_lds;
        c->rq_window.kind = kind;
        c->rq_window.owner = c;
        c->rq_window.payload = &wp;
        wfirst = false;
        return group_submit(c->group, GQ_WINDOW, &c->rq_window);
    };
    int mode = 1, iter_seen = 0;
    struct BusyElsewhere {
        xrhip_group *g;
        explicit BusyElsewhere(xrhip_group *gg) : g(gg) { group_busy_elsewhere(g, 1); }
        ~BusyElsewhere() { group_busy_elsewhere(g, -1); }
    } busy_elsewhere(c->group);
    if (pl.route == ROUTE_TINY) {
        const int seq = ++c->seq;
        hipLaunchKernelGGL(kb_tiny, dim3(1), dim3(256), pl.try_lds, s, c->tiny_args, pl.use_lds, seq, 4 * (P->max_iterations + 8));
        XR_HIP(hipGetLastError());
        rc = wait_mailbox(c, seq);
        if (rc) return rc;
        if (c->h_ctl->status != ST_DONE) return xr_fail(XRHIP_ESTATE, "xrhip_ba_solve: trust-region loop did not terminate");
        c->stats.n_tiny++;
        done = true;
    }
    const bool spec = !sw.no_spec && pl.wide_first && !(c->group && !sw.group_spec);
    BaPtrs p2 = p;
    if (spec) {
        const size_t extra = sizeof(double) * (16 * (size_t)d.F + (size_t)std::max(d.L, 1)) + sizeof(BaCtl) + 1024;
        if (c->work_spec_cap < c->work_cap + extra) {
            if (c->work_spec) hipFree(c->work_spec);
            c->work_spec = nullptr;
            XR_HIP(hipMalloc(&c->work_spec, c->work_cap + extra));
            c->work_spec_cap = c->work_cap + extra;
        }
        auto shift = [&](auto &member) {
            using T = std::remove_reference_t<decltype(*(static_cast<decltype(&*member)>(nullptr)))>;
            member = reinterpret_cast<T *>(c->work_spec + (reinterpret_cast<const char *>(static_cast<T *>(member)) - c->work));
        };
        shift(p2.orec); shift(p2.ocost); shift(p2.rrec); shift(p2.rcost);
        shift(p2.imu_r); shift(p2.imu_Ji); shift(p2.imu_Jj); shift(p2.imu_cost);
        shift(p2.pr); shift(p2.pt); shift(p2.pJq); shift(p2.pcost);
        shift(p2.hll); shift(p2.gl); shift(p2.Wt); shift(p2.Hv); shift(p2.gv);
        shift(p2.Hpp); shift(p2.gp); shift(p2.diagD); shift(p2.gs); shift(p2.omega);
        shift(p2.T); shift(p2.Sred); shift(p2.partial); shift(p2.wog);
        char *x = c->work_spec + ((c->work_cap + 255) & ~size_t(255));
        p2.state = reinterpret_cast<double *>(x);
        p2.depth = reinterpret_cast<double *>(x + sizeof(double) * 16 * (size_t)d.F);
        p2.ctl = reinterpret_cast<BaCtl *>(x + ((sizeof(double) * (16 * (size_t)d.F + (size_t)std::max(d.L, 1)) + 255) & ~size_t(255)));
    }
    auto swap_sets = [&]() {
        std::swap(p.orec, p2.orec); std::swap(p.ocost, p2.ocost); std::swap(p.rrec, p2.rrec); std::swap(p.rcost, p2.rcost);
        std::swap(p.imu_r, p2.imu_r); std::swap(p.imu_Ji, p2.imu_Ji); std::swap(p.imu_Jj, p2.imu_Jj); std::swap(p.imu_cost, p2.imu_cost);
        std::swap(p.pr, p2.pr); std::swap(p.pt, p2.pt); std::swap(p.pJq, p2.pJq); std::swap(p.pcost, p2.pcost);
        std::swap(p.hll, p2.hll); std::swap(p.gl, p2.gl); std::swap(p.Wt, p2.Wt); std::swap(p.Hv, p2.Hv); std::swap(p.gv, p2.gv);
        std::swap(p.Hpp, p2.Hpp); std::swap(p.gp, p2.gp); std::swap(p.diagD, p2.diagD); std::swap(p.gs, p2.gs); std::swap(p.omega, p2.omega);
        std::swap(p.T, p2.T); std::swap(p.Sred, p2.Sred); std::swap(p.partial, p2.partial); std::swap(p.wog, p2.wog);
    };
    bool spec_ready = false;
    for (int guard = 0; guard < 4 * (P->max_iterations + 8) && !done; ++guard) {
        const int seq = ++c->seq;
        if (wbatch) {
            rc = submit_window(GK_WROUND, seq, mode);
        } else if (spec_ready) {
            rc = launch_solve_try(c, d, pl, p, cam, imu, sx, sy, false, mode, seq, true, &p2);
        } else {
            if (relinearise) launch_linearize(c, d, pl, p, cam, imu, sx, sy, true);
            rc = launch_solve_try(c, d, pl, p, cam, imu, sx, sy, !relinearise, mode, seq, false, spec ? &p2 : nullptr);
        }
        if (rc) return rc;
        spec_ready = false;
        bool spec_launched = false;
        if (spec) {
            BaPtrs q = p2;
            launch_linearize(c, d, pl, q, cam, imu, sx, sy, true);
            launch_schur_aux(d, q, s);
            XR_HIP(hipGetLastError());
            spec_launched = true;
            c->spec_launched++;
        }
        rc = wbatch ? wait_mailbox(c, seq, wstream, &c->rq_window)
                    : wait_mailbox(c, seq, spec ? c->stream2 : nullptr);
        if (rc) return rc;
        const bool first_batch_accept = spec_launched && c->h_ctl->status == ST_ACCEPTED && c->h_ctl->accepted_slot == 0;
        {
            const int it_now = c->h_ctl->iteration;
            const int trials = std::max(0, it_now - iter_seen);
            iter_seen = it_now;
            c->stats.n_trials += trials;
            if (c->profiling && !wbatch && !c->pending.empty()) c->pending.back().iter_before = trials;
        }
        int st = c->h_ctl->status;
        for (int wguard = 0; st == ST_NEED_TRIALS && wguard < 64; ++wguard) {
            const int wseq = ++c->seq;
            if (wbatch) {
                rc = submit_window(GK_WTRIALS, wseq, 0);
                if (rc) return rc;
                rc = wait_mailbox(c, wseq, wstream, &c->rq_window);
            } else {
                hipLaunchKernelGGL(kb_trials_wide, dim3(WIDE_G), dim3(256), pl.wide_lds, spec ? c->stream2 : s, d, p, cam, imu, sx, sy, wseq, 0, 0);
                XR_HIP(hipGetLastError());
                rc = wait_mailbox(c, wseq, spec ? c->stream2 : nullptr);
            }
            if (rc) return rc;
            const int it_now = c->h_ctl->iteration;
            c->stats.n_trials += std::max(0, it_now - iter_seen);
            iter_seen = it_now;
            st = c->h_ctl->status;
        }
        if (st == ST_DONE) {
            done = true;
        } else if (st == ST_ACCEPTED) {
            relinearise = true;
            mode = 1;
            if (first_batch_accept) {
                swap_sets();
                spec_ready = true;
                c->spec_taken++;
            }
        } else if (st == ST_RESOLVE || st == ST_RESOLVE_INNER) {
            relinearise = false;
            mode = (st == ST_RESOLVE) ? 2 : 3;
        } else {
            return xr_fail(XRHIP_ESTATE, "xrhip_ba_solve: unexpected device status");
        }
    }
    if (!done) return xr_fail(XRHIP_ESTATE, "xrhip_ba_solve: trust-region loop did not terminate");
    std::memcpy(P->frame_state, c->h_out, sizeof(double) * 16 * d.F);
    if (d.L && d.nla) std::memcpy(P->inv_depth, c->h_out + 16 * d.F, sizeof(double) * d.L);
    rc = preint_launch_deferred(c, P, nullptr);
    if (rc) return rc;
    kprof_accumulate(*c->h_ctl, d.na);
    fill_summary(*c->h_ctl, ms_since(t_begin), summary);
    c->dims = d;
    c->ptrs = p;
    c->have_lin = true;
    return XRHIP_OK;
}

int xrhip_ba_debug_marg_guard(xrhip_ba *c, double *lambda_bound, int *status8) {
    if (!c || !lambda_bound || !status8) return xr_fail(XRHIP_EINVAL, "xrhip_ba_debug_marg_guard: null argument");
    if (c->marg.pending || !c->marg.lam) return xr_fail(XRHIP_ESTATE, "xrhip_ba_debug_marg_guard: no collected marginalisation on this context");
    XR_HIP(hipStreamSynchronize(c->stream));
    XR_HIP(hipMemcpy(lambda_bound, c->marg.lam, sizeof(double), hipMemcpyDeviceToHost));
    XR_HIP(hipMemcpy(status8, c->marg.dst, sizeof(int) * 8, hipMemcpyDeviceToHost));
    return XRHIP_OK;
}

int xrhip_ba_debug_set_schur_precision(xrhip_ba *c, int mode) {
// ... 89 lines not shown
        XR_HIP(hipStreamSynchronize(c->stream));
        if (c->cov_dev) hipFree(c->cov_dev);
        c->cov_dev = nullptr;
        c->cov_cap = 0;
        const size_t cap = std::max((w + 256) * 2, size_t(1) << 20);
        XR_HIP(hipMalloc(&c->cov_dev, cap));
        c->cov_cap = cap;
    }
    char *S = c->cov_dev;
    CovStatus *st = (CovStatus *)(S + o_st);
    double *A = (double *)(S + o_A), *Li = (double *)(S + o_Li), *ds = (double *)(S + o_ds), *B = (double *)(S + o_B);
    double *Sig = (double *)(S + o_Sig), *dout = (double *)(S + o_out), *dvar = (double *)(S + o_var);
    int *dcols = (int *)(S + o_cols);
    std::vector<int> cols(16 * (size_t)(n_sel + nt), -1);
    for (int k = 0; k < n_sel; ++k)
        for (int q = 0; q < 15; ++q) cols[16 * (size_t)k + q] = act_inv[15 * req->sel_frames[k] + q];
    for (int t = 0; t < nt; ++t)
        for (int q = 0; q < 16; ++q) cols[16 * (size_t)(n_sel + t) + q] = (16 * t + q < na) ? 16 * t + q : -1;
    hipStream_t s = c->stream;
    const bool timed = c->profiling;
    if (timed)
        for (hipEvent_t &e : c->cov_ev)
            if (!e) XR_HIP(hipEventCreate(&e));
    long launches = 1;
    XR_HIP(hipMemsetAsync(st, 0, sizeof(CovStatus), s));
    XR_HIP(hipMemcpyAsync(dcols, cols.data(), sizeof(int) * cols.size(), hipMemcpyHostToDevice, s));
    if (timed) XR_HIP(hipEventRecord(c->cov_ev[0], s));
    if (d.np) {
        hipLaunchKernelGGL(kb_prior_lambda, dim3(((d.np + 15) / 16) * ((d.np + 15) / 16 + 1)), dim3(256), 0, s, d.np, p.pS, p.pLam, p.pinfo, p.pc0);
        ++launches;
    }
    launch_linearize(c, d, pl, p, cam, imu, P->sqrt_inv_cov[0], P->sqrt_inv_cov[1], false);
    launches += LINEARIZE_LAUNCHES;
    if (d.nla) {
        hipLaunchKernelGGL(kc_weights, dim3((d.L + 255) / 256), dim3(256), 0, s, d.L, p.lact, p.hll, p.omega);
        const int tiles = d.PF / 16;
        hipLaunchKernelGGL(kb_schur_mfma, dim3(tiles * tiles), dim3(256), 0, s, d, p);
        launches += 2;
    }
    hipLaunchKernelGGL(kc_compact, dim3((unsigned)(((size_t)n16 * n16 + 255) / 256)), dim3(256), 0, s, d, p, n16, A, ds);
    if (timed) XR_HIP(hipEventRecord(c->cov_ev[1], s));
    hipLaunchKernelGGL(kc_factor, dim3(1), dim3(COV_NT), 0, s, na, n16, A, Li, st);
    if (timed) XR_HIP(hipEventRecord(c->cov_ev[2], s));
    launches += 2;
    if (full) {
        hipLaunchKernelGGL(kc_selected_inverse, dim3(nt), dim3(256), 0, s, na, n16, A, Li, ds, dcols + 16 * (size_t)n_sel, B, 1, Sig, st);
        ++launches;
        if (n_sel) {
            hipLaunchKernelGGL(kc_gather_blocks, dim3(n_sel), dim3(256), 0, s, n16, Sig, dcols, dout, st);
            ++launches;
        }
    } else {
        for (int base = 0; base < n_sel; base += SEL_BATCH) {
            hipLaunchKernelGGL(kc_selected_inverse, dim3(std::min(SEL_BATCH, n_sel - base)), dim3(256), 0, s, na, n16, A, Li, ds,
                               dcols + 16 * (size_t)base, B, 0, dout + 225 * (size_t)base, st);
            ++launches;
        }
    }
    if (timed) XR_HIP(hipEventRecord(c->cov_ev[3], s));
    if (full) {
        hipLaunchKernelGGL(kc_landmark_var, dim3((d.L + 3) / 4), dim3(64), 0, s, d, p, n16, Sig, dvar, st);
        ++launches;
    }
    if (timed) XR_HIP(hipEventRecord(c->cov_ev[4], s));
    XR_HIP(hipGetLastError());
    c->stats.n_cov_launches += launches;
    CovStatus hst;
    XR_HIP(hipMemcpyAsync(&hst, st, sizeof(CovStatus), hipMemcpyDeviceToHost, s));
    XR_HIP(hipStreamSynchronize(s));
    *req->status = hst.status ? 1 : 0;
    if (hst.status) {
        std::snprintf(xr_err_buf(), 512, "xrhip_ba_covariance: pivot %d of %d is not positive to working precision (status 1)", hst.pivot, na);
        return XRHIP_OK;
    }
    if (req->rcond_estimate) *req->rcond_estimate = hst.max_pivot > 0.0 ? hst.min_pivot / hst.max_pivot : 0.0;
    if (n_sel) XR_HIP(hipMemcpyAsync(req->out_blocks, dout, D8 * 225 * (size_t)n_sel, hipMemcpyDeviceToHost, s));
    if (full) XR_HIP(hipMemcpyAsync(req->out_inv_depth_var, dvar, D8 * d.L, hipMemcpyDeviceToHost, s));
    XR_HIP(hipStreamSynchronize(s));
    if (want_var && !full) std::memset(req->out_inv_depth_var, 0, D8 * d.L);
    if (timed) {
        float ms = 0.f;
        for (int k = 0; k < 4; ++k) {
            const int a = k == 3 ? 0 : k + 1, b = k == 3 ? 4 : k + 2;
            c->cov_ms[k] = hipEventElapsedTime(&ms, c->cov_ev[a], c->cov_ev[b]) == hipSuccess ? ms : 0.0;
        }
        if (!full) c->cov_ms[2] = 0.0;
    }
    return XRHIP_OK;
}

int xrhip_ba_debug_cov_times(xrhip_ba *c, double *ms4) {
    if (!c || !ms4) return xr_fail(XRHIP_EINVAL, "xrhip_ba_debug_cov_times: null argument");
    std::memcpy(ms4, c->cov_ms, sizeof(c->cov_ms));
    return XRHIP_OK;
}

int xrhip_ba_debug_schur(xrhip_ba *c, const double *W, const double *w, int L, int P, double *out) {
    if (!c || !W || !w || !out || L <= 0 || P <= 0) return xr_fail(XRHIP_EINVAL, "xrhip_ba_debug_schur: bad arguments");
    BaDims d;
    std::memset(&d, 0, sizeof(d));
    BaPtrs p;
    std::memset(&p, 0, sizeof(p));
    d.PF = round_up(P, 16);
    d.L = L;
    d.Lp = std::max(16, round_up(L, 16));
    std::vector<double> wt((size_t)d.Lp * d.PF, 0.0), om(d.Lp, 0.0);
    for (int l = 0; l < L; ++l) {
        om[l] = w[l];
        for (int a = 0; a < P; ++a) wt[(size_t)l * d.PF + a] = W[(size_t)l * P + a];
    }
    double *dW = nullptr, *dw = nullptr, *dT = nullptr;
    XR_HIP(hipMalloc(&dW, sizeof(double) * wt.size()));
    XR_HIP(hipMalloc(&dw, sizeof(double) * om.size()));
    XR_HIP(hipMalloc(&dT, sizeof(double) * (size_t)d.PF * d.PF));
    XR_HIP(hipMemcpy(dW, wt.data(), sizeof(double) * wt.size(), hipMemcpyHostToDevice));
    XR_HIP(hipMemcpy(dw, om.data(), sizeof(double) * om.size(), hipMemcpyHostToDevice));
    p.Wt = dW;
    p.omega = dw;
    p.T = dT;
    const int tiles = d.PF / 16;
    hipLaunchKernelGGL(kb_schur_mfma, dim3(tiles * tiles), dim3(256), 0, c->stream, d, p);
    XR_HIP(hipGetLastError());
    XR_HIP(hipStreamSynchronize(c->stream));
    std::vector<double> T((size_t)d.PF * d.PF);
    XR_HIP(hipMemcpy(T.data(), dT, sizeof(double) * T.size(), hipMemcpyDeviceToHost));
    for (int a = 0; a < P; ++a)
        for (int b = 0; b < P; ++b) out[(size_t)a * P + b] = T[(size_t)a * d.PF + b];
    hipFree(dW);
    hipFree(dw);
    hipFree(dT);
    return XRHIP_OK;
}

}

static int ensure_work2(xrhip_ba *c, size_t dev_bytes, size_t host_bytes) {
    if (dev_bytes > c->work2_cap) {
        if (c->work2) hipFree(c->work2);
        c->work2 = nullptr;
        size_t cap = std::max(dev_bytes * 2, size_t(1) << 20);
        XR_HIP(hipMalloc(&c->work2, cap));
        c->work2_cap = cap;
    }
    if (host_bytes > c->h_stage_cap) {
        if (c->h_stage) hipHostFree(c->h_stage);
        c->h_stage = nullptr;
        size_t cap = std::max(host_bytes * 2, size_t(1) << 20);
        XR_HIP(hipHostMalloc(&c->h_stage, cap, hipHostMallocDefault));
        c->h_stage_cap = cap;
    }
    return XRHIP_OK;
}

extern "C" {


static int marg_launch(xrhip_ba *c, const xrhip_marg_problem *M) {
    if (c->marg.pending) return xr_fail(XRHIP_ESTATE, "xrhip_ba_marginalize: a marginalisation is already in flight");
    if (M->n_frames < 2 || M->victim < 0 || M->victim >= M->n_frames)
        return xr_fail(XRHIP_EINVAL, "xrhip_ba_marginalize: bad frame count / victim");
    const int K = M->n_frames;
    std::vector<double> state(M->frame_state, M->frame_state + 16 * (size_t)K);
    std::vector<uint8_t> fix(K, 0);
    std::vector<double> depth(M->inv_depth, M->inv_depth + std::max(M->n_landmarks, 0));
    std::vector<uint8_t> lfix(std::max(M->n_landmarks, 1), 0);
    xrhip_ba_problem P;
    std::memset(&P, 0, sizeof(P));
    P.n_frames = K;
    P.frame_state = state.data();
    P.frame_fix = fix.data();
    std::memcpy(P.cam_q_bc, M->cam_q_bc, sizeof(P.cam_q_bc));
    std::memcpy(P.cam_p_bc, M->cam_p_bc, sizeof(P.cam_p_bc));
    std::memcpy(P.imu_q_bi, M->imu_q_bi, sizeof(P.imu_q_bi));
    std::memcpy(P.imu_p_bi, M->imu_p_bi, sizeof(P.imu_p_bi));
    std::memcpy(P.sqrt_inv_cov, M->sqrt_inv_cov, sizeof(P.sqrt_inv_cov));
    P.n_landmarks = M->n_landmarks;
    P.inv_depth = depth.data();
    P.landmark_fix = lfix.data();
    P.n_obs = M->n_obs;
    P.obs_tgt = M->obs_tgt;
    P.obs_ref = M->obs_ref;
    P.obs_lm = M->obs_lm;
    P.obs_z_tgt = M->obs_z_tgt;
    P.obs_z_ref = M->obs_z_ref;
    P.n_imu = M->n_imu;
    P.imu_i = M->imu_i;
    P.imu_j = M->imu_j;
    P.imu_data = M->imu_data;
    P.prior_n = M->prior_n;
    P.prior_frames = M->prior_frames;
    P.prior_sqrt_info = M->prior_sqrt_info;
    P.prior_infovec = M->prior_infovec;
    P.prior_lin = M->prior_lin;
    P.max_iterations = 0;
    int rc = validate(&P);
    if (rc) return rc;
    BaDims d;
    SolvePlan pl;
    BaPtrs p;
    Ext cam, imu;
    rc = stage_problem(c, &P, d, pl, p, cam, imu);
    if (rc) return rc;
    d.robust = 0;
    d.schur_mode = 0;
    const int N = d.n, R = N - 15;
    if (R > 512) return xr_fail(XRHIP_EINVAL, "xrhip_ba_marginalize: window too large");
    const size_t D8 = sizeof(double);
    size_t w = 0;
    auto carve = [&](size_t bytes) {
        size_t off = (w + 255) & ~size_t(255);
        w = off + std::max(bytes, size_t(8));
        return off;
    };
    const size_t o_Hm = carve(D8 * (size_t)N * N), o_bm = carve(D8 * N), o_T2 = carve(D8 * (size_t)R * 15);
    const size_t o_A = carve(D8 * (size_t)R * R), o_bp = carve(D8 * R), o_B = carve(D8 * (size_t)R * R);
    const size_t o_V = carve(D8 * (size_t)R * R), o_si = carve(D8 * (size_t)R * R), o_iv = carve(D8 * R);
    const size_t o_st = carve(sizeof(int) * 8), o_lam = carve(D8 * 2), o_sup = carve(sizeof(int) * (size_t)R);
    const size_t o_As = carve(D8 * (size_t)R * R), o_bs = carve(D8 * R), o_Ss = carve(D8 * (size_t)R * R), o_ivs = carve(D8 * R);
    rc = ensure_work2(c, w + 256, D8 * ((size_t)R * R + R) + 64 + sizeof(int) * 8);
    if (rc) return rc;
    char *W2 = c->work2;
    double *Hm = (double *)(W2 + o_Hm), *bm = (double *)(W2 + o_bm), *T2 = (double *)(W2 + o_T2);
    double *A = (double *)(W2 + o_A), *bp = (double *)(W2 + o_bp), *B = (double *)(W2 + o_B), *V = (double *)(W2 + o_V);
    double *dsi = (double *)(W2 + o_si), *div = (double *)(W2 + o_iv);
    int *dst = (int *)(W2 + o_st);
    hipStream_t s = c->stream;
    XR_HIP(hipMemsetAsync(dst, 0, sizeof(int) * 8, s));
    if (d.np) hipLaunchKernelGGL(kb_prior_lambda, dim3(((d.np + 15) / 16) * ((d.np + 15) / 16 + 1)), dim3(256), 0, s, d.np, p.pS, p.pLam, p.pinfo, p.pc0);
    launch_linearize(c, d, pl, p, cam, imu, M->sqrt_inv_cov[0], M->sqrt_inv_cov[1], false);
    hipLaunchKernelGGL(km_omega, dim3((std::max(d.L, 1) + 255) / 256), dim3(256), 0, s, d, p);
    const int tiles = d.PF / 16;
    hipLaunchKernelGGL(kb_schur_mfma, dim3(tiles * tiles), dim3(256), 0, s, d, p);
    hipLaunchKernelGGL(km_wog, dim3(aux_wog_blocks(d.F)), dim3(256), 0, s, d, p);
    hipLaunchKernelGGL(km_permute, dim3((N * N + 255) / 256), dim3(256), 0, s, d, p, M->victim, Hm, bm);
    hipLaunchKernelGGL(km_victim, dim3(1), dim3(256), 0, s, N, Hm, T2, dst);
    hipLaunchKernelGGL(km_complement, dim3((R * R + 255) / 256), dim3(256), 0, s, N, Hm, bm, T2, A, bp);
    double *hs = (double *)c->h_stage;
    int *dsup = (int *)(W2 + o_sup), *dsn = dst + 1;
    double *As = (double *)(W2 + o_As), *bs = (double *)(W2 + o_bs), *Ss = (double *)(W2 + o_Ss), *ivs = (double *)(W2 + o_ivs);
    const int lds_doubles = c->lds_limit / (int)D8;
    hipLaunchKernelGGL(km_support, dim3(1), dim3(512), 0, s, R, A, bp, dsup, dsn, As, bs);
    hipLaunchKernelGGL(km_chol, dim3(1), dim3(512), (size_t)c->lds_limit, s, dsn, lds_doubles, As, bs, dsup, R, dsi, div,
                       (double *)(W2 + o_lam), dst);
    XR_HIP(hipGetLastError());
    hipLaunchKernelGGL(km_jacobi, dim3(1), dim3(1024), (size_t)c->lds_limit, s, dst + 5, lds_doubles, As, bs, B, V, Ss, ivs, 60, dst + 2,
                       dsup, R, dsi, div);
    XR_HIP(hipGetLastError());
    XR_HIP(hipMemcpyAsync(hs, dsi, D8 * (size_t)R * R, hipMemcpyDeviceToHost, s));
    XR_HIP(hipMemcpyAsync(hs + (size_t)R * R, div, D8 * R, hipMemcpyDeviceToHost, s));
    XR_HIP(hipMemcpyAsync(hs + (size_t)R * R + R, dst, sizeof(int) * 8, hipMemcpyDeviceToHost, s));
    if (!c->ev_marg) XR_HIP(hipEventCreateWithFlags(&c->ev_marg, hipEventDisableTiming));
    XR_HIP(hipEventRecord(c->ev_marg, s));
    xrhip_ba::MargPending &mp = c->marg;
    mp.pending = true;
    mp.K = K;
    mp.victim = M->victim;
    mp.R = R;
    mp.lin.assign(M->frame_state, M->frame_state + 16 * (size_t)K);
    mp.dst = dst;
    mp.dsup = dsup;
    mp.lam = (double *)(W2 + o_lam);
    mp.As = As;
    mp.bs = bs;
    mp.B = B;
    mp.V = V;
    mp.Ss = Ss;
    mp.ivs = ivs;
    mp.dsi = dsi;
    mp.div = div;
    return XRHIP_OK;
}

static int marg_collect(xrhip_ba *c, double *out_sqrt_info, double *out_infovec, double *out_lin) {
    xrhip_ba::MargPending &mp = c->marg;
    if (!mp.pending) return xr_fail(XRHIP_ESTATE, "xrhip_ba_marginalize_end: nothing in flight");
    mp.pending = false;
    hipStream_t s = c->stream;
    const size_t D8 = sizeof(double);
    const int R = mp.R, K = mp.K;
    double *hs = (double *)c->h_stage;
    XR_HIP(hipEventSynchronize(c->ev_marg));
    int hst[8];
    std::memcpy(hst, hs + (size_t)R * R + R, sizeof(hst));
    if (hst[0]) return xr_fail(XRHIP_ESTATE, "xrhip_ba_marginalize: singular victim block");
    if (hst[4] && std::getenv("XRHIP_HOSTPROF"))
        std::fprintf(stderr, "[hostprof] marginalisation took the eigen path on the device: guard %s, support %d of %d, %d sweeps\n",
                     hst[3] ? "failed" : "ok", hst[1], R, hst[2]);
    if ((hst[2] != 0 || hst[3] != 0) && !hst[4]) {
        if (std::getenv("XRHIP_HOSTPROF"))
            std::fprintf(stderr, "[hostprof] marginalisation falls back to the eigen path: cholesky %s, guard %s, support %d of %d\n",
                         hst[2] ? "failed" : "ok", hst[3] ? "failed" : "ok", hst[1], R);
        const int lds_doubles = c->lds_limit / (int)D8;
        int *dsn = mp.dst + 1;
        hipLaunchKernelGGL(km_jacobi, dim3(1), dim3(1024), (size_t)c->lds_limit, s, dsn, lds_doubles, mp.As, mp.bs, mp.B, mp.V, mp.Ss,
                           mp.ivs, 60, mp.dst + 2);
        hipLaunchKernelGGL(km_expand, dim3((R * R + 255) / 256), dim3(256), 0, s, R, mp.dsup, dsn, mp.Ss, mp.ivs, mp.dsi, mp.div);
        XR_HIP(hipGetLastError());
        XR_HIP(hipMemcpyAsync(hs, mp.dsi, D8 * (size_t)R * R, hipMemcpyDeviceToHost, s));
        XR_HIP(hipMemcpyAsync(hs + (size_t)R * R, mp.div, D8 * R, hipMemcpyDeviceToHost, s));
        XR_HIP(hipStreamSynchronize(s));
    }
    std::memcpy(out_sqrt_info, hs, D8 * (size_t)R * R);
    std::memcpy(out_infovec, hs + (size_t)R * R, D8 * R);
    int j = 0;
    for (int i = 0; i < K; ++i) {
        if (i == mp.victim) continue;
        std::memcpy(out_lin + 16 * (size_t)j, mp.lin.data() + 16 * (size_t)i, D8 * 16);
        ++j;
    }
    return XRHIP_OK;
}

int xrhip_ba_marginalize(xrhip_ba *c, const xrhip_marg_problem *M, double *out_sqrt_info, double *out_infovec,
                         double *out_lin) {
    if (!c || !M || !out_sqrt_info || !out_infovec || !out_lin) return xr_fail(XRHIP_EINVAL, "xrhip_ba_marginalize: null argument");
    int rc = marg_launch(c, M);
    if (rc) return rc;
    return marg_collect(c, out_sqrt_info, out_infovec, out_lin);
}

int xrhip_ba_marginalize_begin(xrhip_ba *c, const xrhip_marg_problem *M) {
    if (!c || !M) return xr_fail(XRHIP_EINVAL, "xrhip_ba_marginalize_begin: null argument");
    return marg_launch(c, M);
}

int xrhip_ba_marginalize_end(xrhip_ba *c, double *out_sqrt_info, double *out_infovec, double *out_lin) {
    if (!c || !out_sqrt_info || !out_infovec || !out_lin) return xr_fail(XRHIP_EINVAL, "xrhip_ba_marginalize_end: null argument");
    return marg_collect(c, out_sqrt_info, out_infovec, out_lin);
}

static int preint_stage(xrhip_ba *c, const double *samples, const int *sample_begin, const int *sample_count,
                        const double *t_end, const double *bg, const double *ba, const int *bias_frame, int n_jobs,
                        const double *noise_cov36) {
    if (c->preint_pending || c->preint_deferred)
        return xr_fail(XRHIP_ESTATE, "xrhip_ba_preintegrate_begin: a batch is already in flight on this context");
    int total = 0;
    for (int k = 0; k < n_jobs; ++k) {
        if (sample_count[k] <= 0 || sample_begin[k] < 0) return xr_fail(XRHIP_EINVAL, "xrhip_ba_preintegrate: empty IMU segment");
        total = std::max(total, sample_begin[k] + sample_count[k]);
    }
    const size_t D8 = sizeof(double);
    const size_t b_jobs = sizeof(PreintJob) * n_jobs, b_smp = D8 * 7 * (size_t)total, b_noise = D8 * 36;
    const size_t o_jobs = 0, o_smp = (b_jobs + 255) & ~size_t(255), o_noise = (o_smp + b_smp + 255) & ~size_t(255);
    const size_t o_out = (o_noise + b_noise + 255) & ~size_t(255), o_st = o_out + D8 * XRHIP_IMU_DIM * (size_t)n_jobs;
    const size_t bytes = o_st + 2 * sizeof(int) * n_jobs + 256;
    int rc = ensure_work2(c, 0, bytes);
    if (rc) return rc;
    char *H = c->h_stage;
    PreintJob *jobs = (PreintJob *)(H + o_jobs);
    for (int k = 0; k < n_jobs; ++k) {
        jobs[k].sample_begin = sample_begin[k];
        jobs[k].sample_count = sample_count[k];
        jobs[k].t_end = t_end[k];
        for (int i = 0; i < 3; ++i) {
            jobs[k].bg[i] = bg ? bg[3 * k + i] : 0.0;
            jobs[k].ba[i] = ba ? ba[3 * k + i] : 0.0;
        }
        jobs[k].bias_frame = bias_frame ? bias_frame[k] : -1;
        jobs[k].pad_ = 0;
    }
    std::memcpy(H + o_smp, samples, b_smp);
    std::memcpy(H + o_noise, noise_cov36, b_noise);
    std::memset(H + o_st, 0, 2 * sizeof(int) * n_jobs);
    c->preint_o_jobs = o_jobs;
    c->preint_o_smp = o_smp;
    c->preint_o_noise = o_noise;
    c->preint_o_out = o_out;
    c->preint_o_st = o_st;
    return XRHIP_OK;
}

static int preint_args(xrhip_ba *c, int n_jobs, int jac, int cov, const double *state_dev, PreintArgs *a) {
    char *Dv = nullptr;
    XR_HIP(hipHostGetDevicePointer((void **)&Dv, c->h_stage, 0));
    *a = PreintArgs{(const PreintJob *)(Dv + c->preint_o_jobs), (const double *)(Dv + c->preint_o_smp), (const double *)(Dv + c->preint_o_noise),
                    jac ? 1 : 0, cov ? 1 : 0, (double *)(Dv + c->preint_o_out), (int *)(Dv + c->preint_o_st),
                    (int *)(Dv + c->preint_o_st) + n_jobs, state_dev, n_jobs, {}};
    const PreintJob *hj = (const PreintJob *)(c->h_stage + c->preint_o_jobs);
    for (int k = 0; k < std::min(n_jobs, PI_HEAD); ++k) a->head[k] = hj[k];
    return XRHIP_OK;
}

static int preint_launch(xrhip_ba *c, int n_jobs, int jac, int cov, const double *state_dev) {
    if (c->group) {
        int rc = group_wait_launched(&c->rq_preint);
        if (rc) return rc;
    }
    int rc = preint_args(c, n_jobs, jac, cov, state_dev, &c->a_preint);
    if (rc) return rc;
    c->rq_preint.kind = GK_PREINT;
    c->rq_preint.owner = c;
    c->rq_preint.payload = &c->a_preint;
    if (c->group) {
        rc = group_submit(c->group, GQ_PREINT, &c->rq_preint);
        c->preint_rq = &c->rq_preint;
        c->preint_stream = group_stream(c->group, GQ_PREINT);
    } else {
        GroupRequest *one = &c->rq_preint;
        rc = launch_preint_batch(&one, 1, c->stream);
        c->preint_rq = nullptr;
        c->preint_stream = c->stream;
    }
    if (rc) return rc;
    c->preint_pending = n_jobs;
    c->preint_deferred = 0;
    return XRHIP_OK;
}

static int preint_fill_deferred(xrhip_ba *c, const xrhip_ba_problem *P, const double *state_dev, PreintArgs *out, bool *have) {
    *have = false;
    if (!c->preint_deferred) return XRHIP_OK;
    int rc = preint_deferred_check(c, P);
    if (!rc) rc = preint_args(c, c->preint_deferred, c->preint_def_jac, c->preint_def_cov, state_dev, out);
    if (rc) return rc;
    *have = true;
    return XRHIP_OK;
}

static int preint_launch_deferred(xrhip_ba *c, const xrhip_ba_problem *P, const double *state_dev) {
    if (!c->preint_deferred) return XRHIP_OK;
    const int rc = preint_deferred_check(c, P);
    if (rc) return rc;
    const int n_jobs = c->preint_deferred;
    PreintJob *jobs = (PreintJob *)(c->h_stage + c->preint_o_jobs);
    for (int k = 0; k < n_jobs; ++k) {
        const int f = jobs[k].bias_frame;
        if (!state_dev) {
            for (int i = 0; i < 3; ++i) {
                jobs[k].bg[i] = P->frame_state[16 * f + 10 + i];
                jobs[k].ba[i] = P->frame_state[16 * f + 13 + i];
            }
            jobs[k].bias_frame = -1;
        }
    }
    return preint_launch(c, n_jobs, c->preint_def_jac, c->preint_def_cov, state_dev);
}

int xrhip_ba_preintegrate_begin(xrhip_ba *c, const double *samples, const int *sample_begin, const int *sample_count,
                                const double *t_end, const double *bg, const double *ba, int n_jobs,
                                const double *noise_cov36, int compute_jacobian, int compute_covariance) {
    if (!c || !samples || !sample_begin || !sample_count || !t_end || !bg || !ba || !noise_cov36 || n_jobs <= 0)
        return xr_fail(XRHIP_EINVAL, "xrhip_ba_preintegrate: bad arguments");
    int rc = preint_stage(c, samples, sample_begin, sample_count, t_end, bg, ba, nullptr, n_jobs, noise_cov36);
    if (rc) return rc;
    return preint_launch(c, n_jobs, compute_jacobian, compute_covariance, nullptr);
}

int xrhip_ba_preintegrate_after_solve(xrhip_ba *c, const double *samples, const int *sample_begin, const int *sample_count,
                                      const double *t_end, const int *bias_frame, int n_jobs, const double *noise_cov36,
                                      int compute_jacobian, int compute_covariance) {
    if (!c || !samples || !sample_begin || !sample_count || !t_end || !bias_frame || !noise_cov36 || n_jobs <= 0)
        return xr_fail(XRHIP_EINVAL, "xrhip_ba_preintegrate_after_solve: bad arguments");
    for (int k = 0; k < n_jobs; ++k)
        if (bias_frame[k] < 0) return xr_fail(XRHIP_EINVAL, "xrhip_ba_preintegrate_after_solve: negative bias frame");
    int rc = preint_stage(c, samples, sample_begin, sample_count, t_end, nullptr, nullptr, bias_frame, n_jobs, noise_cov36);
    if (rc) return rc;
    c->preint_deferred = n_jobs;
    c->preint_def_jac = compute_jacobian ? 1 : 0;
    c->preint_def_cov = compute_covariance ? 1 : 0;
    return XRHIP_OK;
}

int xrhip_ba_preintegrate_cancel(xrhip_ba *c) {
    if (!c) return xr_fail(XRHIP_EINVAL, "xrhip_ba_preintegrate_cancel: null context");
    if (c->preint_pending) {
        if (c->preint_rq) group_wait_launched(c->preint_rq);
        XR_HIP(hipStreamSynchronize(c->preint_stream ? c->preint_stream : c->stream));
        c->preint_pending = 0;
    }
    c->preint_deferred = 0;
    return XRHIP_OK;
}

int xrhip_ba_preintegrate_early(xrhip_ba *c, int job, double *out_delta11) {
    if (!c || !out_delta11 || job < 0) return xr_fail(XRHIP_EINVAL, "xrhip_ba_preintegrate_early: bad arguments");
    if (!c->preint_pending || job >= c->preint_pending)
        return xr_fail(XRHIP_ESTATE, "xrhip_ba_preintegrate_early: no such job in flight");
    char *H = c->h_stage;
    const int n_jobs = c->preint_pending;
    volatile int *early = (volatile int *)(H + c->preint_o_st) + n_jobs;
    if (c->preint_rq) {
// ... 60 lines not shown
```

xrslam_amd/csrc/host/map.hpp:

```cpp
#pragma once
#include <deque>
#include <functional>
#include <map>
#include <memory>
#include <optional>
#include <vector>

#include "../../../include/xrslam_hip.h"
#include "geometry.hpp"

namespace xrh {

inline constexpr size_t nil() { return size_t(-1); }

struct ImuData {
    double t;
    V3 w, a;
};

enum FrameTag { FT_KEYFRAME = 0, FT_NO_TRANSLATION, FT_FIX_POSE, FT_FIX_MOTION, FT_COUNT };
enum TrackTag { TT_VALID = 0, TT_TRIANGULATED, TT_FIX_INVD, TT_TRASH, TT_STATIC, TT_OUTLIER, TT_TEMP, TT_COUNT };

struct Extrinsic {
    Quat q_cs;
// ... 40 lines not shown
    size_t frame = 0, track = 0;
};

class Frame {
  public:
    size_t id = 0;
    unsigned long ba_gen = 0;
    int ba_index = -1;
    bool tags[FT_COUNT] = {false, false, false, false};
    Map *map = nullptr;
    Intrinsics K;
    double sqrt_inv_cov[2] = {1, 1};
    std::shared_ptr<HipImage> image;
    PoseState pose;
    MotionState motion;
    Extrinsic camera, imu;
    PreInt preintegration, keyframe_preintegration;
    std::vector<std::unique_ptr<Frame>> subframes;
    std::vector<V3> bearings;
    std::vector<Track *> tracks;

    bool &tag(FrameTag t) { return tags[t]; }
    bool tag(FrameTag t) const { return tags[t]; }
    size_t keypoint_num() const { return bearings.size(); }
    const V3 &get_keypoint(size_t i) const { return bearings[i]; }
    Track *get_track(size_t i) const { return tracks[i]; }
    Track *get_track(size_t i, Map *allocation_map);
    void append_keypoint(const V3 &b) {
        bearings.push_back(b);
        tracks.push_back(nullptr);
    }
    std::unique_ptr<Frame> clone() const {
        auto f = std::make_unique<Frame>();
        f->id = id;
        for (int i = 0; i < FT_COUNT; ++i) f->tags[i] = tags[i];
        f->K = K;
        f->sqrt_inv_cov[0] = sqrt_inv_cov[0];
        f->sqrt_inv_cov[1] = sqrt_inv_cov[1];
        f->image = image;
        f->pose = pose;
        f->motion = motion;
        f->camera = camera;
        f->imu = imu;
        f->preintegration = preintegration;
        f->bearings = bearings;
        f->tracks.assign(bearings.size(), nullptr);
        return f;
    }
    PoseState get_pose(const Extrinsic &s) const { return {pose.q * s.q_cs, pose.p + pose.q * s.p_cs}; }
    void set_pose(const Extrinsic &s, const PoseState &ps) {
        pose.q = ps.q * s.q_cs.conjugate();
        pose.p = ps.p - pose.q * s.p_cs;
    }
};

struct FrameIdLess {
    bool operator()(const Frame *a, const Frame *b) const { return a->id < b->id; }
};

class FrameRefs {
  public:
    using value_type = std::pair<Frame *, size_t>;
    using const_iterator = std::vector<value_type>::const_iterator;
    const_iterator begin() const { return v_.begin(); }
    const_iterator end() const { return v_.end(); }
    size_t size() const { return v_.size(); }
    bool empty() const { return v_.empty(); }
    const_iterator find(Frame *f) const {
        auto it = lower(f);
        return (it != v_.end() && !FrameIdLess()(f, it->first)) ? it : v_.end();
    }
    size_t count(Frame *f) const { return find(f) != v_.end() ? 1 : 0; }
    size_t at(Frame *f) const {
        auto it = find(f);
        if (it == v_.end()) throw std::out_of_range("FrameRefs::at");
        return it->second;
    }
    size_t &operator[](Frame *f) {
        auto it = v_.begin() + (lower(f) - v_.begin());
        if (it == v_.end() || FrameIdLess()(f, it->first)) it = v_.insert(it, value_type(f, 0));
        return it->second;
    }
    void erase(Frame *f) {
        auto it = find(f);
        if (it != v_.end()) v_.erase(v_.begin() + (it - v_.begin()));
    }

  private:
    const_iterator lower(Frame *f) const {
        return std::lower_bound(v_.begin(), v_.end(), f, [](const value_type &a, Frame *b) { return FrameIdLess()(a.first, b); });
    }
    std::vector<value_type> v_;
};

struct LandmarkState {
    double inv_depth = 0, reprojection_error = 0;
};

class Track {
  public:
    size_t id = 0;
    unsigned long ba_gen = 0;
    int ba_index = -1;
    unsigned long visit_gen = 0;
    bool tags[TT_COUNT] = {false, false, false, false, true, false, false};
    size_t map_index = 0;
    Map *map = nullptr;
    LandmarkState landmark;
    size_t m_life = 0;
    FrameRefs keypoint_refs;

    bool &tag(TrackTag t) { return tags[t]; }
    bool tag(TrackTag t) const { return tags[t]; }
    bool all_tagged(std::initializer_list<TrackTag> ts) const {
        for (TrackTag t : ts)
            if (!tags[t]) return false;
        return true;
    }
    size_t keypoint_num() const { return keypoint_refs.size(); }
    std::pair<Frame *, size_t> first_keypoint() const { return *keypoint_refs.begin(); }
    Frame *first_frame() const { return keypoint_refs.begin()->first; }
    bool has_keypoint(Frame *f) const { return keypoint_refs.count(f) > 0; }
    size_t get_keypoint_index(Frame *f) const {
        auto it = keypoint_refs.find(f);
        return it == keypoint_refs.end() ? nil() : it->second;
    }
    void add_keypoint(Frame *frame, size_t keypoint_index) {
        keypoint_refs[frame] = keypoint_index;
        frame->tracks[keypoint_index] = this;
        if (tag(TT_TRIANGULATED)) m_life++;
        else m_life = 1;
    }
    void remove_keypoint(Frame *frame, bool suicide_if_empty = true);
    std::optional<V3> triangulate();
    V3 get_landmark_point() const {
        auto [frame, ki] = first_keypoint();
        PoseState cam = frame->get_pose(frame->camera);
        return cam.q * frame->get_keypoint(ki) / landmark.inv_depth + cam.p;
    }
    void set_landmark_point(const V3 &p) {
        auto [frame, ki] = first_keypoint();
        (void)ki;
        PoseState cam = frame->get_pose(frame->camera);
        landmark.inv_depth = 1.0 / norm(cam.q.conjugate() * (p - cam.p));
    }
};

struct MargPrior {
    std::vector<Frame *> frames;
    std::vector<double> lin;
    std::vector<double> sqrt_info;
    std::vector<double> infovec;
    bool pending = false;
};

class Map {
  public:
    explicit Map(IdSource *ids) : ids_(ids) {}
    size_t frame_num() const { return frames.size(); }
    Frame *get_frame(size_t i) const { return frames[i].get(); }
    void attach_frame(std::unique_ptr<Frame> frame, size_t position = nil()) {
        frame->map = this;
        if (position == nil()) frames.emplace_back(std::move(frame));
        else frames.emplace(frames.begin() + position, std::move(frame));
    }
    std::unique_ptr<Frame> detach_frame(size_t index) {
        std::unique_ptr<Frame> f = std::move(frames[index]);
        frames.erase(frames.begin() + index);
        f->map = nullptr;
        return f;
    }
    void untrack_frame(Frame *frame) {
        for (size_t i = 0; i < frame->keypoint_num(); ++i)
            if (Track *t = frame->get_track(i)) t->remove_keypoint(frame);
    }
    void erase_frame(size_t index) {
        untrack_frame(frames[index].get());
        detach_frame(index);
    }
    size_t frame_index_by_id(size_t id) const {
        auto it = std::lower_bound(frames.begin(), frames.end(), id,
                                   [](const std::unique_ptr<Frame> &f, size_t v) { return f->id < v; });
        if (it == frames.end() || id < (*it)->id) return nil();
        return (size_t)std::distance(frames.begin(), it);
    }
    size_t track_num() const { return tracks.size(); }
    Track *get_track(size_t i) const { return tracks[i].get(); }
    Track *create_track() {
        auto t = std::make_unique<Track>();
        t->id = ++ids_->track;
        t->map_index = tracks.size();
        t->map = this;
        tracks.emplace_back(std::move(t));
        return tracks.back().get();
    }
    void recycle_track(Track *track) {
        if (track->map_index != tracks.back()->map_index) {
            tracks[track->map_index].swap(tracks.back());
            tracks[track->map_index]->map_index = track->map_index;
        }
        tracks.pop_back();
    }
    void erase_track(Track *track) {
        while (track->keypoint_num() > 0) track->remove_keypoint(track->keypoint_refs.begin()->first, false);
        recycle_track(track);
    }
    void prune_tracks(const std::function<bool(const Track *)> &cond) {
        std::vector<Track *> victims;
        for (size_t i = 0; i < track_num(); ++i)
            if (cond(get_track(i))) victims.push_back(get_track(i));
        for (Track *t : victims) erase_track(t);
    }
    IdSource *ids() const { return ids_; }

    std::unique_ptr<MargPrior> marginalization_factor;
    std::deque<std::unique_ptr<Frame>> frames;
    std::vector<std::unique_ptr<Track>> tracks;

  private:
    IdSource *ids_;
};

inline Track *Frame::get_track(size_t i, Map *allocation_map) {
    if (!allocation_map) allocation_map = map;
    if (tracks[i] == nullptr) {
        Track *t = allocation_map->create_track();
        t->add_keypoint(this, i);
    }
    return tracks[i];
}

inline void Track::remove_keypoint(Frame *frame, bool suicide_if_empty) {
    size_t ki = keypoint_refs.at(frame);
    std::optional<V3> lm;
    if (frame == first_frame()) lm = get_landmark_point();
    frame->tracks[ki] = nullptr;
    keypoint_refs.erase(frame);
    if (!keypoint_refs.empty()) {
        if (lm.has_value()) set_landmark_point(lm.value());
    } else {
        tag(TT_VALID) = false;
        if (suicide_if_empty) map->recycle_track(this);
    }
}

inline std::optional<V3> Track::triangulate() {
    std::vector<P34> Ps;
    std::vector<V3> zs;
    for (const auto &[frame, ki] : keypoint_refs) {
        PoseState pose = frame->get_pose(frame->camera);
        M3 R = to_matrix(pose.q.conjugate());
        V3 T = -(R * pose.p);
        P34 P;
        for (int r = 0; r < 3; ++r) {
            for (int c = 0; c < 3; ++c) P.m[4 * r + c] = R(r, c);
            P.m[4 * r + 3] = T[r];
        }
        Ps.push_back(P);
        zs.push_back(frame->get_keypoint(ki));
    }
    auto h = triangulate_point(Ps, zs);
    for (size_t i = 0; i < zs.size(); ++i) {
        const double q2 = Ps[i].m[8] * h[0] + Ps[i].m[9] * h[1] + Ps[i].m[10] * h[2] + Ps[i].m[11] * h[3];
        if (!(q2 * h[3] > 0)) return {};
    }
    m_life = 1;
    return V3{h[0] / h[3], h[1] / h[3], h[2] / h[3]};
}

}
```

xrslam_amd/csrc/host/pipeline.hpp:

```cpp
#pragma once
#include <chrono>
#include <climits>
#include <algorithm>
#include <cstdio>
#include <cstring>
#include <atomic>
#include <condition_variable>
#include <deque>
#include <exception>
#include <functional>
#include <mutex>
#include <optional>
#include <stdexcept>
#include <thread>
#include <tuple>
#include <unordered_map>
#include <unordered_set>

#include "../host_select.hpp"
#include "../hostprof.hpp"
#include "ba_dump.hpp"
#include "config.hpp"
#include "covariance.hpp"
#include "map.hpp"
#include "parsac.hpp"
#include "pixel_format.hpp"
#include "two_view.hpp"
#include "undistort_map.hpp"

extern "C" {
int xrhip_image_upload_color(xrhip_image *img, const void *pixels, int stride_bytes, int channels, int on_device) __attribute__((weak));
int xrhip_image_upload_color_distorted(xrhip_image *img, const void *pixels, int stride_bytes, int channels, int on_device) __attribute__((weak));
int xrhip_image_upload_format(xrhip_image *img, const void *pixels, int stride_bytes, int format, int bits, int limited_range, int on_device) __attribute__((weak));
int xrhip_image_upload_format_distorted(xrhip_image *img, const void *pixels, int stride_bytes, int format, int bits, int limited_range, int on_device) __attribute__((weak));
int xrhip_image_upload_scaled(xrhip_image *img, const void *pixels, int stride_bytes, int format, int bits, int limited_range, int on_device, const xrhip_frame_geometry *geo) __attribute__((weak));
int xrhip_image_upload_scaled_distorted(xrhip_image *img, const void *pixels, int stride_bytes, int format, int bits, int limited_range, int on_device, const xrhip_frame_geometry *geo) __attribute__((weak));
int xrhip_image_render_view(xrhip_image *img, const xrhip_view_segment *segs, int n_segs, const xrhip_view_marker *markers, int n_markers,
                            const uint8_t *palette_bgr, int n_palette, void *out, int stride_bytes, int channels, int on_device) __attribute__((weak));
int xrhip_klt_set_lk_params(xrhip_klt *ctx, const xrhip_lk_params *p) __attribute__((weak));
int xrhip_ba_covariance(xrhip_ba *ctx, const xrhip_ba_problem *problem, const xrhip_cov_request *req) __attribute__((weak));
}

namespace xrh {
inline bool have_format_upload() { return xrhip_image_upload_format != nullptr && xrhip_image_upload_format_distorted != nullptr; }
inline bool have_scaled_upload() { return xrhip_image_upload_scaled != nullptr && xrhip_image_upload_scaled_distorted != nullptr; }
inline bool have_color_upload() { return xrhip_image_upload_color != nullptr && xrhip_image_upload_color_distorted != nullptr; }

struct FrameInput {
    const uint8_t *pixels = nullptr;
    int stride = 0;
    bool on_device = false;
    int channels = 1;
    bool by_format = false;
    int format = XRHIP_PIXFMT_GRAY8, bits = 0, limited_range = 0;
    const xrhip_frame_geometry *geo = nullptr;
};

struct HipError : std::runtime_error {
    explicit HipError(const std::string &m) : std::runtime_error(m) {}
};
inline void hip_check(int rc, const char *what) {
    if (rc != 0) throw HipError(std::string(what) + ": " + xrhip_last_error());
}

struct StageTimes {
    double tracker = 0, localize = 0, refine = 0, marginalize = 0, preintegrate = 0;
    long frames = 0, solves = 0, solve_iterations = 0, marginalizations = 0, keyframes = 0;
    double ba_device_ms = 0;
    double w_upload = 0, w_preprocess = 0, w_track = 0, w_detect = 0, w_preintegrate = 0, w_solve = 0, w_marginalize = 0,
           w_frame = 0;
    double w_preintegrate_ft = 0;
    double w_join = 0;
    double scope[16] = {0};
};
enum { SC_FT_TRACK = 0, SC_RANSAC_E, SC_RANSAC_R, SC_FT_DETECT, SC_MIRROR, SC_LOCALIZE, SC_MANAGE_KF, SC_TRACK_LANDMARK,
       SC_REFINE_WINDOW, SC_SLIDE_WINDOW, SC_REFINE_SUBWINDOW, SC_INITIALIZE, SC_RD_JUDGED, SC_RD_OUTLIERS, SC_CONST_COPIES, SC_COUNT };
struct WallTimer {
    double &slot;
    std::chrono::steady_clock::time_point t0 = std::chrono::steady_clock::now();
    explicit WallTimer(double &s) : slot(s) {}
    ~WallTimer() { slot += std::chrono::duration<double>(std::chrono::steady_clock::now() - t0).count(); }
};

class JobThread {
  public:
    explicit JobThread(int device) : device_(device), th_([this] { loop(); }) {}
    ~JobThread() {
        {
            const int s = state_.load(std::memory_order_acquire);
            if (s == POSTED) await([this] { return state_.load(std::memory_order_acquire) == DONE; }, 20000);
        }
        state_.store(QUIT, std::memory_order_release);
        {
            std::lock_guard<std::mutex> lk(m_);
        }
        cv_.notify_all();
        th_.join();
    }
    JobThread(const JobThread &) = delete;
    JobThread &operator=(const JobThread &) = delete;
    void post(std::function<void()> job) {
        job_ = std::move(job);
        error_ = nullptr;
        state_.store(POSTED, std::memory_order_release);
        {
            std::lock_guard<std::mutex> lk(m_);
        }
        cv_.notify_all();
    }
    void wait() {
        await([this] { return state_.load(std::memory_order_acquire) == DONE; }, 20000);
        state_.store(IDLE, std::memory_order_relaxed);
        if (error_) {
            std::exception_ptr e = error_;
            error_ = nullptr;
            std::rethrow_exception(e);
        }
    }

  private:
    enum { IDLE = 0, POSTED, DONE, QUIT };
    static void relax() {
#if defined(__x86_64__) || defined(__i386__)
        __builtin_ia32_pause();
#else
        std::this_thread::yield();
#endif
    }
    template <class Pred> void await(Pred pred, long spin_us) {
        const auto t0 = std::chrono::steady_clock::now();
        for (;;) {
            for (int spin = 0; spin < 256; ++spin) {
                if (pred()) return;
                relax();
            }
            if (std::chrono::steady_clock::now() - t0 > std::chrono::microseconds(spin_us)) break;
        }
        std::unique_lock<std::mutex> lk(m_);
        cv_.wait(lk, pred);
    }
    void loop() {
        if (device_ >= 0) xrhip_bind_device(device_);
        for (;;) {
            await([this] {
                const int s = state_.load(std::memory_order_acquire);
                return s == POSTED || s == QUIT;
            }, 2000);
            if (state_.load(std::memory_order_acquire) == QUIT) return;
            try {
                job_();
            } catch (...) {
                error_ = std::current_exception();
            }
            state_.store(DONE, std::memory_order_release);
            {
                std::lock_guard<std::mutex> lk(m_);
            }
            cv_.notify_all();
        }
    }
    int device_;
    std::function<void()> job_;
    std::exception_ptr error_;
    std::atomic<int> state_{IDLE};
    std::mutex m_;
    std::condition_variable cv_;
    std::thread th_;
};

struct Pipeline {
    Config config;
    xrhip_klt *klt = nullptr;
    xrhip_ba *ba = nullptr;
    xrhip_ba *ba_marg = nullptr;
    xrhip_ba *ba_aux = nullptr;
    xrhip_ba *ba_ft = nullptr;
    xrhip_ba *ba_sub = nullptr;
    std::mutex pool_mutex;
    std::unique_ptr<JobThread> marg_launcher;
    bool marg_launch_pending = false;
    void marg_launch_wait() {
        if (!marg_launch_pending) return;
        marg_launch_pending = false;
        marg_launcher->wait();
    }
    IdSource ids;
    std::vector<xrhip_image *> image_pool;
    double noise36[36];
    StageTimes times;
    struct Covariance {
        bool enabled = false;
        double t = 0.0;
        double state[225] = {0.0};
// ... 345 lines not shown

inline void predict(const PreInt &pre, const Frame *o, Frame *n) {
    const V3 gravity{0, 0, -9.80665};
    const double dt = pre.dt();
    n->motion.bg = o->motion.bg;
    n->motion.ba = o->motion.ba;
    n->motion.v = o->motion.v + gravity * dt + o->pose.q * pre.dv();
    n->pose.p = o->pose.p + 0.5 * gravity * dt * dt + o->motion.v * dt + o->pose.q * pre.dp();
    n->pose.q = o->pose.q * pre.dq();
}

inline void frame_detect_keypoints(Pipeline &P, Frame *f) {
    WallTimer sc_t(P.times.scope[SC_FT_DETECT]);
    const Config &c = P.config;
    std::vector<double> existing(2 * f->keypoint_num());
    for (size_t i = 0; i < f->keypoint_num(); ++i) {
        V2 px = apply_k(f->bearings[i], f->K);
        existing[2 * i] = px.x;
        existing[2 * i + 1] = px.y;
    }
    const int maxp = (int)c.feature_tracker_max_keypoint_detection;
    std::vector<double> fresh(2 * (size_t)std::max(maxp, 1));
    int n_new = 0;
    WallTimer wt_w_detect(P.times.w_detect);
    hip_check(xrhip_image_detect(f->image->h, existing.data(), (int)f->keypoint_num(), maxp,
                                 c.feature_tracker_min_keypoint_distance, fresh.data(), &n_new),
              "xrhip_image_detect");
    for (int i = 0; i < n_new; ++i) f->append_keypoint(remove_k(V2{fresh[2 * i], fresh[2 * i + 1]}, f->K));
}

inline void frame_track_keypoints(Pipeline &P, Frame *cur, Frame *next, std::function<void(Frame *)> *deferred_tag = nullptr) {
    WallTimer sc_t(P.times.scope[SC_FT_TRACK]);
    const Config &c = P.config;
    const size_t n = cur->keypoint_num();
    std::vector<double> curr_px(2 * n), next_px(2 * n);
    for (size_t i = 0; i < n; ++i) {
        V2 px = apply_k(cur->bearings[i], cur->K);
        curr_px[2 * i] = px.x;
        curr_px[2 * i + 1] = px.y;
    }
    int has_guess = 0;
    if (c.feature_tracker_predict_keypoints) {
        Quat dq = (cur->camera.q_cs.conjugate() * cur->imu.q_cs * next->preintegration.dq() *
                   next->imu.q_cs.conjugate() * next->camera.q_cs)
                      .conjugate();
        for (size_t i = 0; i < n; ++i) {
            V2 px = apply_k(dq * cur->bearings[i], next->K);
            next_px[2 * i] = px.x;
            next_px[2 * i + 1] = px.y;
        }
        has_guess = 1;
    }
    std::vector<uint8_t> st8(std::max<size_t>(n, 1), 0);
    {
        WallTimer wt_w_track(P.times.w_track);
        hip_check(xrhip_image_track(cur->image->h, next->image->h, curr_px.data(), next_px.data(), has_guess,
                                    st8.data(), (int)n),
                  "xrhip_image_track");
    }
    xrhip::HostProfScope hp_post(4, "ft_track: after LK (all)");
    std::optional<xrhip::HostProfScope> hp_a(std::in_place, 5, "ft_track: bearings");
    std::vector<char> status(st8.begin(), st8.begin() + n), mask;
    std::vector<V2> cur_h, next_h;
    std::vector<V3> next_bearings;
    cur_h.reserve(n);
    next_h.reserve(n);
    next_bearings.reserve(n);
    for (size_t i = 0; i < n; ++i) {
        const V3 &b = cur->bearings[i];
        cur_h.push_back({b.x / b.z, b.y / b.z});
        V3 nb = remove_k(V2{next_px[2 * i], next_px[2 * i + 1]}, next->K);
        next_h.push_back({nb.x / nb.z, nb.y / nb.z});
        next_bearings.push_back(nb);
    }
    hp_a.reset();
    {
        WallTimer sc_e(P.times.scope[SC_RANSAC_E]);
        find_essential_matrix(cur_h, next_h, mask, 1.0);
    }
    for (size_t i = 0; i < status.size() && i < mask.size(); ++i)
        if (!mask[i]) status[i] = 0;
    M3 R;
    {
        WallTimer sc_r(P.times.scope[SC_RANSAC_R]);
        R = find_rotation_matrix(cur->bearings, next_bearings, mask, (M_PI / 180.0) * c.rotation_ransac_threshold);
    }
    xrhip::HostProfScope hp_b(6, "ft_track: angles+poisson+append");
    std::optional<xrhip::HostProfScope> hp_c(std::in_place, 13, "ft_track: angles");
    {
        std::vector<std::pair<V3, V3>> pairs;
        pairs.reserve(mask.size());
        for (size_t i = 0; i < mask.size(); ++i)
            if (mask[i]) pairs.emplace_back(R * cur->bearings[i], next_bearings[i]);
        const double threshold = c.rotation_misalignment_threshold;
        auto decide = [pairs = std::move(pairs), threshold, next](Frame *copy) {
            std::vector<double> angles;
            angles.reserve(pairs.size());
            for (const auto &pr : pairs) angles.push_back(std::acos(dot(pr.first, pr.second)) * 180 / M_PI);
            std::sort(angles.begin(), angles.end());
            const double misalignment = angles.size() > 0 ? angles[angles.size() * 7 / 10] : 0;
            if (misalignment < threshold) {
                next->tag(FT_NO_TRANSLATION) = true;
                if (copy) copy->tag(FT_NO_TRANSLATION) = true;
            }
        };
        if (deferred_tag) *deferred_tag = std::move(decide);
        else decide(nullptr);
    }

    hp_c.emplace(14, "ft_track: by_length+poisson");
    std::vector<std::pair<size_t, size_t>> by_length;
    by_length.reserve(n);
    for (size_t i = 0; i < n; ++i) {
        if (status[i] == 0) continue;
        Track *t = cur->get_track(i);
        if (t == nullptr) continue;
        by_length.emplace_back(i, t->keypoint_num());
    }
    std::sort(by_length.begin(), by_length.end(), [](const auto &a, const auto &b) { return a.second > b.second; });
    xrhip::PoissonDisk2 filter(c.feature_tracker_min_keypoint_distance, (int)c.cam_resolution[0], (int)c.cam_resolution[1]);
    for (auto &[ki, len] : by_length) {
        (void)len;
        Track *t = cur->get_track(ki);
        if (filter.permit(next_px[2 * ki], next_px[2 * ki + 1]) && (!t || !t->tag(TT_TRASH))) {
            filter.preset(next_px[2 * ki], next_px[2 * ki + 1]);
        } else {
            status[ki] = 0;
        }
    }
    hp_c.reset();
    xrhip::HostProfScope hp_d(15, "ft_track: append");
    for (size_t i = 0; i < n; ++i) {
        if (status[i]) {
            size_t nk = next->keypoint_num();
            next->append_keypoint(next_bearings[i]);
            cur->get_track(i, nullptr)->add_keypoint(next, nk);
        }
    }
}

inline void resolve_marginalization(Pipeline &P, MargPrior *prior) {
    if (!prior || !prior->pending) return;
    P.marg_launch_wait();
    const size_t n = prior->frames.size(), R = 15 * n;
    std::vector<double> si(R * R), iv(R), lin(16 * n);
    {
        WallTimer wt_w_marginalize(P.times.w_marginalize);
        hip_check(xrhip_ba_marginalize_end(P.ba_marg, si.data(), iv.data(), lin.data()), "xrhip_ba_marginalize_end");
    }
    prior->sqrt_info.swap(si);
    prior->infovec.swap(iv);
    prior->lin.swap(lin);
    prior->pending = false;
}

class BaBuilder {
  public:
    explicit BaBuilder(Pipeline &P) : P_(P), gen_(++P.ba_generation) {
        obs_tgt_.reserve(2048);
        obs_ref_.reserve(2048);
        obs_lm_.reserve(2048);
        obs_zt_.reserve(3 * 2048);
        obs_zr_.reserve(3 * 2048);
        tracks_.reserve(512);
        lfix_.reserve(512);
    }
    int frame_index(Frame *f, bool as_parameter, bool with_motion = true) {
        if (f->ba_gen != gen_) {
            f->ba_gen = gen_;
            f->ba_index = (int)frames_.size();
            frames_.push_back(f);
            fix_.push_back(XRHIP_FIX_POSE | XRHIP_FIX_MOTION);
        }
        if (as_parameter) {
            uint8_t fx = 0;
            if (f->tag(FT_FIX_POSE)) fx |= XRHIP_FIX_POSE;
            if (!with_motion || f->tag(FT_FIX_MOTION)) fx |= XRHIP_FIX_MOTION;
            fix_[f->ba_index] = fx;
        }
        return f->ba_index;
    }
    void add_frame_states(Frame *f, bool with_motion = true) { frame_index(f, true, with_motion); }
    int landmark_index(Track *t, bool as_parameter) {
        if (t->ba_gen != gen_) {
            t->ba_gen = gen_;
            t->ba_index = (int)tracks_.size();
            tracks_.push_back(t);
            lfix_.push_back(1);
        }
        if (as_parameter) lfix_[t->ba_index] = 0;
        return t->ba_index;
    }
    void add_track_states(Track *t) { landmark_index(t, true); }
    void add_reprojection_error(Frame *frame, size_t ki) {
        Track *t = frame->get_track(ki);
        auto [ref, kr] = t->first_keypoint();
        push_obs(frame_index(frame, false), frame_index(ref, false), landmark_index(t, false), frame->get_keypoint(ki),
                 ref->get_keypoint(kr));
    }
    void add_reprojection_prior(Frame *frame, size_t ki) {
        Track *t = frame->get_track(ki);
        auto [ref, kr] = t->first_keypoint();
        const_obs_.push_back(obs_tgt_.size());
        push_obs(frame_index(frame, false), const_frame(ref), const_landmark(t), frame->get_keypoint(ki),
                 ref->get_keypoint(kr));
    }
    void add_rotation_prior(Frame *frame, size_t ki) {
        Track *t = frame->get_track(ki);
        auto [ref, kr] = t->first_keypoint();
        const_rot_.push_back(rot_tgt_.size());
        rot_tgt_.push_back(frame_index(frame, false));
        rot_ref_.push_back(const_frame(ref));
        push3(rot_zt_, frame->get_keypoint(ki));
        push3(rot_zr_, ref->get_keypoint(kr));
    }
    void add_preintegration_error(Frame *fi, Frame *fj, const PreInt &pre) {
        imu_i_.push_back(frame_index(fi, false));
        imu_j_.push_back(frame_index(fj, false));
        imu_pre_.push_back(&pre);
    }
    void add_preintegration_prior(Frame *fi, Frame *fj, const PreInt &pre) {
        const_imu_.push_back(imu_i_.size());
        imu_i_.push_back(const_frame(fi));
        imu_j_.push_back(frame_index(fj, false));
        imu_pre_.push_back(&pre);
    }
    void add_marginalization(MargPrior *m) { prior_ = m; }
    void chain_integration(Frame *f, std::vector<ImuData> samples, double t) {
        chain_f_ = f;
        chain_samples_ = std::move(samples);
        chain_t_ = t;
    }
    bool chained() const { return chain_queued_; }

    size_t factor_num() const { return obs_tgt_.size() + rot_tgt_.size() + imu_i_.size() + (prior_ ? 1 : 0); }
    void drop_unreferenced_blocks() {
        const size_t F = frames_.size();
        std::vector<char> pose_used(F, 0), motion_used(F, 0);
        for (size_t o = 0; o < obs_tgt_.size(); ++o) pose_used[obs_tgt_[o]] = pose_used[obs_ref_[o]] = 1;
        for (size_t o = 0; o < rot_tgt_.size(); ++o) pose_used[rot_tgt_[o]] = pose_used[rot_ref_[o]] = 1;
        for (size_t o = 0; o < imu_i_.size(); ++o)
            pose_used[imu_i_[o]] = pose_used[imu_j_[o]] = motion_used[imu_i_[o]] = motion_used[imu_j_[o]] = 1;
        if (prior_)
            for (Frame *f : prior_->frames)
                if (f->ba_gen == gen_) pose_used[f->ba_index] = motion_used[f->ba_index] = 1;
        for (size_t f = 0; f < F; ++f) {
            if (!pose_used[f]) fix_[f] |= XRHIP_FIX_POSE;
            if (!motion_used[f]) fix_[f] |= XRHIP_FIX_MOTION;
        }
    }
    void split_aliased_constants() {
        std::unordered_map<int, int> fcopy, lcopy;
        auto frame_copy = [&](int idx) {
            if (fix_[idx] == (XRHIP_FIX_POSE | XRHIP_FIX_MOTION)) return idx;
            auto it = fcopy.find(idx);
            if (it != fcopy.end()) return it->second;
            const int ni = (int)frames_.size();
            frames_.push_back(frames_[idx]);
            fix_.push_back(XRHIP_FIX_POSE | XRHIP_FIX_MOTION);
            fcopy[idx] = ni;
            P_.times.scope[SC_CONST_COPIES] += 1.0;
            return ni;
        };
        auto landmark_copy = [&](int idx) {
            if (lfix_[idx]) return idx;
            auto it = lcopy.find(idx);
            if (it != lcopy.end()) return it->second;
            const int ni = (int)tracks_.size();
            tracks_.push_back(tracks_[idx]);
            lfix_.push_back(1);
            lcopy[idx] = ni;
            P_.times.scope[SC_CONST_COPIES] += 1.0;
            return ni;
        };
        for (size_t o : const_obs_) {
            obs_ref_[o] = frame_copy(obs_ref_[o]);
            obs_lm_[o] = landmark_copy(obs_lm_[o]);
        }
        for (size_t o : const_rot_) rot_ref_[o] = frame_copy(rot_ref_[o]);
        for (size_t o : const_imu_) imu_i_[o] = frame_copy(imu_i_[o]);
    }

    struct Overlap {
        std::function<void()> early;
        std::function<void()> fn;
        bool done = false, early_done = false;
        std::exception_ptr error;
        void run_early() {
            if (early_done) return;
            early_done = true;
            try {
                if (early) early();
            } catch (...) {
                error = std::current_exception();
            }
        }
        void run() {
            run_early();
            if (done) return;
            done = true;
            if (error) return;
            try {
                if (fn) fn();
            } catch (...) {
                error = std::current_exception();
            }
        }
        static void trampoline(void *self) { static_cast<Overlap *>(self)->run(); }
    };
    void prepare() {
        const Config &c = P_.config;
        split_aliased_constants();
        drop_unreferenced_blocks();
        const int F = (int)frames_.size(), L = (int)tracks_.size();
        std::vector<double> &state = state_, &depth = depth_;
        state.assign(16 * (size_t)F, 0.0);
        depth.assign(std::max(L, 1), 0.0);
        for (int f = 0; f < F; ++f) pack_state(frames_[f], &state[16 * (size_t)f]);
        for (int l = 0; l < L; ++l) depth[l] = tracks_[l]->landmark.inv_depth;
        xrhip_ba_problem &pb = pb_;
        std::memset(&pb, 0, sizeof(pb));
        pb.n_frames = F;
        pb.frame_state = state.data();
        pb.frame_fix = fix_.data();
        Frame *any = frames_[0];
        const Quat &qc = any->camera.q_cs, &qi = any->imu.q_cs;
        const double cq[4] = {qc.x, qc.y, qc.z, qc.w}, iq[4] = {qi.x, qi.y, qi.z, qi.w};
        std::memcpy(pb.cam_q_bc, cq, sizeof(cq));
        std::memcpy(pb.imu_q_bi, iq, sizeof(iq));
        for (int k = 0; k < 3; ++k) {
            pb.cam_p_bc[k] = any->camera.p_cs[k];
            pb.imu_p_bi[k] = any->imu.p_cs[k];
        }
        pb.sqrt_inv_cov[0] = any->sqrt_inv_cov[0];
        pb.sqrt_inv_cov[1] = any->sqrt_inv_cov[1];
        pb.n_landmarks = L;
        pb.inv_depth = depth.data();
        pb.landmark_fix = lfix_.data();
        pb.n_obs = (int)obs_tgt_.size();
        pb.obs_tgt = obs_tgt_.data();
        pb.obs_ref = obs_ref_.data();
        pb.obs_lm = obs_lm_.data();
        pb.obs_z_tgt = obs_zt_.data();
        pb.obs_z_ref = obs_zr_.data();
        pb.n_rot = (int)rot_tgt_.size();
        pb.rot_tgt = rot_tgt_.data();
        pb.rot_ref = rot_ref_.data();
        pb.rot_z_tgt = rot_zt_.data();
        pb.rot_z_ref = rot_zr_.data();
        pb.n_imu = (int)imu_i_.size();
        pb.imu_i = imu_i_.data();
        pb.imu_j = imu_j_.data();
        imu_data_.resize((size_t)XRHIP_IMU_DIM * imu_pre_.size());
        for (size_t k = 0; k < imu_pre_.size(); ++k)
            std::memcpy(&imu_data_[(size_t)XRHIP_IMU_DIM * k], imu_pre_[k]->rec, sizeof(double) * XRHIP_IMU_DIM);
        pb.imu_data = imu_data_.data();
        std::vector<int> &pframes = pframes_;
        pframes.clear();
        if (prior_) {
            resolve_marginalization(P_, prior_);
            for (Frame *f : prior_->frames) pframes.push_back(frame_index(f, false));
            if ((int)frames_.size() != F) throw std::logic_error("prior frame is not part of the problem");
            pb.prior_n = (int)pframes.size();
            pb.prior_frames = pframes.data();
            pb.prior_sqrt_info = prior_->sqrt_info.data();
            pb.prior_infovec = prior_->infovec.data();
            pb.prior_lin = prior_->lin.data();
        }
        pb.max_iterations = (int)c.solver_iteration_limit;
        if (P_.ba_dump.enabled()) P_.ba_dump.maybe_dump(pb, P_.times.frames);
        prepared_ = true;
    }
    bool finish(const xrhip_ba_summary &sm, double *elapsed_device_ms = nullptr) {
        const int F = (int)frames_.size(), L = (int)tracks_.size();
        for (int f = 0; f < F; ++f)
            if (fix_[f] != (XRHIP_FIX_POSE | XRHIP_FIX_MOTION)) unpack_state(&state_[16 * (size_t)f], frames_[f], fix_[f]);
        for (int l = 0; l < L; ++l)
            if (!lfix_[l]) tracks_[l]->landmark.inv_depth = depth_[l];
        P_.times.solves++;
        P_.times.solve_iterations += sm.iterations;
        P_.times.ba_device_ms += sm.ms_solve;
        if (elapsed_device_ms) *elapsed_device_ms = sm.ms_solve;
        return sm.usable != 0;
    }
    bool solve(double *elapsed_device_ms = nullptr, Overlap *overlap = nullptr) {
        xrhip::HostProfScope hp_s(10, "BaBuilder::solve (all)");
        if (!prepared_) prepare();
        xrhip_ba_summary sm;
        WallTimer wt_w_solve(P_.times.w_solve);
        if (chain_f_ && chain_f_->ba_gen == gen_)
            chain_queued_ = P_.integrate_after_solve_begin(chain_samples_, chain_t_, chain_f_->ba_index, true, true);
        if (overlap) {
            const int rc = xrhip_ba_solve_overlapped(P_.ba, &pb_, &sm, &Overlap::trampoline, overlap);
            overlap->run();
            if (overlap->error) std::rethrow_exception(overlap->error);
            hip_check(rc, "xrhip_ba_solve_overlapped");
        } else {
            hip_check(xrhip_ba_solve(P_.ba, &pb_, &sm), "xrhip_ba_solve");
        }
        return finish(sm, elapsed_device_ms);
    }
    void covariance(Frame *f) {
        Pipeline::Covariance &cv = P_.cov;
        cv.t = f->image ? f->image->t : 0.0;
        cv.landmark_var.clear();
        cv.rcond = 0.0;
        std::fill(cv.state, cv.state + 225, 0.0);
        if (!xrhip_ba_covariance) {
            cv.status = -1;
            cv.error = "XRSLAMAmdSetCovariance: this library has no xrhip_ba_covariance";
            return;
        }
        if (!prepared_ || f->ba_gen != gen_) throw std::logic_error("covariance: the frame is not part of the solved problem");
        const int sel = f->ba_index, L = (int)tracks_.size();
        std::vector<double> var(std::max(L, 1), 0.0);
        int status = -1;
        const xrhip_cov_request rq = {1, &sel, cv.state, var.data(), &status, &cv.rcond};
        hip_check(xrhip_ba_covariance(P_.ba, &pb_, &rq), "xrhip_ba_covariance");
        cv.status = status;
        cv.error.clear();
        if (status != 0) {
            std::fill(cv.state, cv.state + 225, 0.0);
            return;
        }
        for (int l = 0; l < L; ++l)
            if (!lfix_[l] && var[l] > 0.0) cv.landmark_var.emplace_back((long long)tracks_[l]->id, var[l]);
    }
    bool begin(xrhip_ba *ctx) {
        if (!prepared_) prepare();
        WallTimer wt_w_solve(P_.times.w_solve);
        const int rc = xrhip_ba_solve_begin(ctx, &pb_);
        if (rc < 0) hip_check(rc, "xrhip_ba_solve_begin");
        return rc == 1;
    }
    bool end(xrhip_ba *ctx, Overlap *overlap = nullptr) {
        xrhip_ba_summary sm;
        WallTimer wt_w_solve(P_.times.w_solve);
        if (overlap) {
            overlap->run();
            if (overlap->error) {
                xrhip_ba_solve_abort(ctx);
                std::rethrow_exception(overlap->error);
            }
        }
        hip_check(xrhip_ba_solve_end(ctx, &sm), "xrhip_ba_solve_end");
        return finish(sm);
    }
    static bool solve_linked(BaBuilder &first, int link_in_first, BaBuilder &second, Frame *link, Overlap *overlap) {
        xrhip::HostProfScope hp_s(10, "BaBuilder::solve (all)");
        Pipeline &P = first.P_;
        if (!first.prepared_ || !second.prepared_ || link->ba_gen != second.gen_) throw std::logic_error("solve_linked: builders are not prepared");
        xrhip_ba_summary sm1, sm2;
        WallTimer wt_w_solve(P.times.w_solve);
        if (second.chain_f_ && second.chain_f_->ba_gen == second.gen_)
            second.chain_queued_ = P.integrate_after_solve_begin(second.chain_samples_, second.chain_t_, second.chain_f_->ba_index, true, true);
        const int rc = xrhip_ba_solve_linked(P.ba, &second.pb_, &sm2, link->ba_index, P.ba_sub, link_in_first,
                                             overlap ? &Overlap::trampoline : nullptr, overlap);
        if (overlap) overlap->run();
        if (rc || (overlap && overlap->error)) {
            xrhip_ba_solve_abort(P.ba_sub);
            if (overlap && overlap->error) std::rethrow_exception(overlap->error);
            hip_check(rc, "xrhip_ba_solve_linked");
        }
        hip_check(xrhip_ba_solve_end(P.ba_sub, &sm1), "xrhip_ba_solve_end");
        first.finish(sm1);
        return second.finish(sm2);
    }
    void repack(Frame *f) {
        if (prepared_ && f->ba_gen == gen_) pack_state(f, &state_[16 * (size_t)f->ba_index]);
    }

    static void pack_state(const Frame *f, double *s) {
        s[0] = f->pose.q.x; s[1] = f->pose.q.y; s[2] = f->pose.q.z; s[3] = f->pose.q.w;
        for (int k = 0; k < 3; ++k) {
            s[4 + k] = f->pose.p[k];
            s[7 + k] = f->motion.v[k];
            s[10 + k] = f->motion.bg[k];
            s[13 + k] = f->motion.ba[k];
        }
    }
    static void unpack_state(const double *s, Frame *f, uint8_t fix) {
        if (!(fix & XRHIP_FIX_POSE)) {
            f->pose.q = Quat{s[0], s[1], s[2], s[3]};
            f->pose.p = {s[4], s[5], s[6]};
        }
        if (!(fix & XRHIP_FIX_MOTION)) {
            f->motion.v = {s[7], s[8], s[9]};
            f->motion.bg = {s[10], s[11], s[12]};
            f->motion.ba = {s[13], s[14], s[15]};
        }
    }

  private:
    int const_frame(Frame *f) { return frame_index(f, false); }
    int const_landmark(Track *t) { return landmark_index(t, false); }
    void push3(std::vector<double> &v, const V3 &a) {
        v.push_back(a.x);
        v.push_back(a.y);
        v.push_back(a.z);
    }
    void push_obs(int ft, int fr, int l, const V3 &zt, const V3 &zr) {
        obs_tgt_.push_back(ft);
        obs_ref_.push_back(fr);
        obs_lm_.push_back(l);
        push3(obs_zt_, zt);
        push3(obs_zr_, zr);
    }
    Pipeline &P_;
    unsigned long gen_;
    std::vector<Frame *> frames_;
    std::vector<Track *> tracks_;
    std::vector<uint8_t> fix_, lfix_;
    std::vector<int> obs_tgt_, obs_ref_, obs_lm_, rot_tgt_, rot_ref_, imu_i_, imu_j_;
    std::vector<double> obs_zt_, obs_zr_, rot_zt_, rot_zr_, imu_data_;
    std::vector<const PreInt *> imu_pre_;
    std::vector<size_t> const_obs_, const_rot_, const_imu_;
    MargPrior *prior_ = nullptr;
    std::vector<double> state_, depth_;
    std::vector<int> pframes_;
    xrhip_ba_problem pb_;
    bool prepared_ = false;
    Frame *chain_f_ = nullptr;
    std::vector<ImuData> chain_samples_;
    double chain_t_ = 0;
    bool chain_queued_ = false;
};

inline std::unique_ptr<MargPrior> create_marginalization_factor(Map *map) {
    auto m = std::make_unique<MargPrior>();
    const size_t n = map->frame_num() - 1;
    m->frames.resize(n);
    m->lin.assign(16 * n, 0.0);
    for (size_t i = 0; i < n; ++i) {
        m->frames[i] = map->get_frame(i);
        BaBuilder::pack_state(map->get_frame(i), &m->lin[16 * i]);
    }
    m->infovec.assign(15 * n, 0.0);
    m->sqrt_info.assign(15 * n * 15 * n, 0.0);
    for (int k = 0; k < 6; ++k) m->sqrt_info[(size_t)k * 15 * n + k] = 1.0e15;
    return m;
}

struct MargJob {
    xrhip_marg_problem mp;
    std::vector<double> state, imu_data, zt, zr, depth;
    std::vector<int> pframes, imu_i, imu_j, ot, orf, ol;
};

inline void marginalize_frame(Pipeline &P, Map *map, size_t index) {
    MargPrior *prior = map->marginalization_factor.get();
    if (!prior) throw std::logic_error("marginalization_factor is not initialized yet");
    resolve_marginalization(P, prior);
    const int K = (int)map->frame_num();
    const unsigned long gen = ++P.ba_generation;
    auto fidx_of = [gen](const Frame *f) { return f->ba_gen == gen ? f->ba_index : -1; };
    auto job = std::make_shared<MargJob>();
    std::vector<double> &state = job->state;
    state.resize(16 * (size_t)K);
    for (int i = 0; i < K; ++i) {
        map->get_frame(i)->ba_gen = gen;
        map->get_frame(i)->ba_index = i;
        BaBuilder::pack_state(map->get_frame(i), &state[16 * (size_t)i]);
    }
    xrhip_marg_problem &mp = job->mp;
    std::memset(&mp, 0, sizeof(mp));
    mp.n_frames = K;
    mp.victim = (int)index;
    mp.frame_state = state.data();
    Frame *any = map->get_frame(0);
    const Quat &qc = any->camera.q_cs, &qi = any->imu.q_cs;
    const double cq[4] = {qc.x, qc.y, qc.z, qc.w}, iq[4] = {qi.x, qi.y, qi.z, qi.w};
    std::memcpy(mp.cam_q_bc, cq, sizeof(cq));
    std::memcpy(mp.imu_q_bi, iq, sizeof(iq));
    for (int k = 0; k < 3; ++k) {
        mp.cam_p_bc[k] = any->camera.p_cs[k];
        mp.imu_p_bi[k] = any->imu.p_cs[k];
    }
    mp.sqrt_inv_cov[0] = any->sqrt_inv_cov[0];
    mp.sqrt_inv_cov[1] = any->sqrt_inv_cov[1];
    std::vector<int> &pframes = job->pframes;
    for (Frame *f : prior->frames) {
        if (fidx_of(f) < 0) throw std::out_of_range("marginalize_frame: prior frame is not in the window");
        pframes.push_back(fidx_of(f));
    }
    mp.prior_n = (int)pframes.size();
    mp.prior_frames = pframes.data();
    mp.prior_sqrt_info = prior->sqrt_info.data();
    mp.prior_infovec = prior->infovec.data();
    mp.prior_lin = prior->lin.data();
    std::vector<int> &imu_i = job->imu_i, &imu_j = job->imu_j;
    std::vector<double> &imu_data = job->imu_data;
    for (size_t j = index; j <= index + 1; ++j) {
        if (j == 0 || j >= (size_t)K) continue;
        Frame *fj = map->get_frame(j);
        imu_i.push_back((int)j - 1);
        imu_j.push_back((int)j);
        imu_data.insert(imu_data.end(), fj->keyframe_preintegration.rec, fj->keyframe_preintegration.rec + XRHIP_IMU_DIM);
    }
    mp.n_imu = (int)imu_i.size();
    mp.imu_i = imu_i.data();
    mp.imu_j = imu_j.data();
    mp.imu_data = imu_data.data();
    std::vector<int> &ot = job->ot, &orf = job->orf, &ol = job->ol;
    std::vector<double> &zt = job->zt, &zr = job->zr, &depth = job->depth;
    Frame *victim = map->get_frame(index);
    ot.reserve(2048); orf.reserve(2048); ol.reserve(2048); zt.reserve(3 * 2048); zr.reserve(3 * 2048); depth.reserve(512);
    for (size_t j = 0; j < victim->keypoint_num(); ++j) {
        Track *track = victim->get_track(j);
        if (!track || !track->tag(TT_VALID)) continue;
        Frame *ref = track->first_frame();
        if (!ref->tag(FT_KEYFRAME)) continue;
        const int fr = fidx_of(ref);
        if (fr < 0) throw std::out_of_range("marginalize_frame: reference frame is not in the window");
        const size_t kr = track->keypoint_refs.at(ref);
        int l = -1;
        for (const auto &[tgt, ki] : track->keypoint_refs) {
            if (tgt == ref) continue;
            const int ft_i = fidx_of(tgt);
            if (ft_i < 0) continue;
            if (l < 0) {
                l = (int)depth.size();
                depth.push_back(track->landmark.inv_depth);
            }
            ot.push_back(ft_i);
            orf.push_back(fr);
            ol.push_back(l);
            const V3 &a = tgt->get_keypoint(ki), &b = ref->get_keypoint(kr);
            zt.insert(zt.end(), {a.x, a.y, a.z});
            zr.insert(zr.end(), {b.x, b.y, b.z});
        }
    }
    mp.n_landmarks = (int)depth.size();
    mp.inv_depth = depth.data();
    mp.n_obs = (int)ot.size();
    mp.obs_tgt = ot.data();
    mp.obs_ref = orf.data();
    mp.obs_lm = ol.data();
    mp.obs_z_tgt = zt.data();
    mp.obs_z_ref = zr.data();
    if (P.ba_dump.enabled()) P.ba_dump.dump_marg(mp, P.times.frames);
    {
        WallTimer wt_w_marginalize(P.times.w_marginalize);
        static const bool sync_launch = std::getenv("XRSLAM_AMD_SYNC_MARG_LAUNCH") != nullptr;
        if (sync_launch) {
            hip_check(xrhip_ba_marginalize_begin(P.ba_marg, &mp), "xrhip_ba_marginalize_begin");
        } else {
            if (!P.marg_launcher) {
                int dev = -1;
                if (xrhip_get_device(&dev) != 0) dev = -1;
                P.marg_launcher = std::make_unique<JobThread>(dev);
            }
            xrhip_ba *ctx = P.ba_marg;
            P.marg_launcher->post([ctx, job] { hip_check(xrhip_ba_marginalize_begin(ctx, &job->mp), "xrhip_ba_marginalize_begin"); });
            P.marg_launch_pending = true;
        }
    }
    prior->pending = true;
    prior->frames.clear();
    for (int i = 0; i < K; ++i)
        if ((size_t)i != index) prior->frames.push_back(map->get_frame(i));
    for (size_t i = 0; i < victim->keypoint_num(); ++i)
        if (Track *t = victim->get_track(i)) t->remove_keypoint(victim);
    map->frames.erase(map->frames.begin() + index);
    P.times.marginalizations++;
}

using LatestState = std::tuple<double, PoseState, MotionState>;

class SlidingWindowTracker {
  public:
    SlidingWindowTracker(Pipeline &P, std::unique_ptr<Map> keyframe_map) : P_(P), map(std::move(keyframe_map)) {
        for (size_t j = 1; j < map->frame_num(); ++j) {
            Frame *fi = map->get_frame(j - 1), *fj = map->get_frame(j);
            P_.integrate(fj->preintegration, fj->image->t, fi->motion.bg, fi->motion.ba, true, true);
        }
    }

    bool mirror_prepare(Map *ft_map, Frame *incoming, const Frame *tracker_from = nullptr) {
        cancel_prepared();
        Frame *keyframe = map->get_frame(map->frame_num() - 1);
        Frame *new_i = keyframe->subframes.empty() ? keyframe : keyframe->subframes.back().get();
        const size_t idx_i = ft_map->frame_index_by_id(new_i->id);
        if (idx_i == nil()) return false;
        if (tracker_from && !(idx_i + 1 == ft_map->frame_num() && tracker_from->id == new_i->id && same3(tracker_from->motion.bg, new_i->motion.bg) &&
                              same3(tracker_from->motion.ba, new_i->motion.ba)))
            return false;
        std::vector<ImuData> nd = incoming->preintegration.data;
        for (size_t index = ft_map->frame_num() - 1; index > idx_i; --index) {
            const std::vector<ImuData> &od = ft_map->get_frame(index)->preintegration.data;
            nd.insert(nd.begin(), od.begin(), od.end());
        }
        prepared_ = P_.integrate_begin(nd, incoming->image->t, new_i->motion.bg, new_i->motion.ba, true, true);
        prepared_id_ = incoming->id;
        prepared_from_ = new_i->id;
        prepared_samples_ = nd.size();
        return prepared_ && tracker_from != nullptr;
    }
    void cancel_prepared() {
        if (prepared_id_ != nil() && prepared_) {
            PreInt scratch;
            P_.integrate_end(scratch);
        }
        prepared_id_ = nil();
        prepared_ = false;
    }
    ~SlidingWindowTracker() {
        try {
            cancel_prepared();
            drain_speculation();
        } catch (...) {
        }
        if (std::getenv("XRHIP_HOSTPROF"))
            std::fprintf(stderr, "[hostprof] subframe re-integrations: %ld speculated, %ld taken from mirror_frame, %ld computed in place\n",
                         spec_hits_, memo_hits_, spec_misses_);
        if (std::getenv("XRHIP_HOSTPROF"))
            std::fprintf(stderr, "[hostprof] mirror_frame: %ld of %ld interval integrations were queued ahead (%ld behind a solve, on the device)\n",
                         mirror_prepared_, mirror_total_, mirror_chained_);
    }
    size_t prepared_id_ = nil(), prepared_from_ = nil(), prepared_samples_ = 0;
    bool prepared_ = false;
    long mirror_prepared_ = 0, mirror_total_ = 0, mirror_chained_ = 0;
    void forget_queued_work() noexcept {
        prepared_id_ = nil();
        prepared_ = false;
        chained_id_ = nil();
        kf_queued_ = false;
        kf_ok_.clear();
        spec_jobs_ = 0;
        spec_.clear();
        memo_id_ = nil();
        std::lock_guard<std::mutex> lk(hint_mutex_);
        hint_.reset();
    }

    struct MirrorHint {
        size_t id, from;
        double t;
        std::vector<ImuData> samples;
    };
    void post_mirror_hint(MirrorHint h) {
        std::lock_guard<std::mutex> lk(hint_mutex_);
        hint_ = std::move(h);
    }
    void drop_mirror_hint() {
        std::lock_guard<std::mutex> lk(hint_mutex_);
        hint_.reset();
    }
    void take_mirror_hint() {
        std::optional<MirrorHint> h;
        {
            std::lock_guard<std::mutex> lk(hint_mutex_);
            h.swap(hint_);
        }
        if (!h) return;
        cancel_prepared();
        Frame *keyframe = map->get_frame(map->frame_num() - 1);
        Frame *new_i = keyframe->subframes.empty() ? keyframe : keyframe->subframes.back().get();
        if (new_i->id != h->from) return;
        prepared_ = P_.integrate_begin(h->samples, h->t, new_i->motion.bg, new_i->motion.ba, true, true);
        prepared_id_ = h->id;
        prepared_from_ = h->from;
        prepared_samples_ = h->samples.size();
    }
    void chain_mirror_hint(BaBuilder &b, Frame *newest) {
        std::optional<MirrorHint> h;
        {
            std::lock_guard<std::mutex> lk(hint_mutex_);
            if (hint_ && hint_->from == newest->id) h.swap(hint_);
        }
        if (!h) return;
        cancel_prepared();
        chained_id_ = h->id;
        chained_from_ = h->from;
        chained_samples_ = h->samples.size();
        b.chain_integration(newest, std::move(h->samples), h->t);
    }
    void chained_solve_done(const BaBuilder &b) {
        if (chained_id_ == nil()) return;
        prepared_ = b.chained();
        if (prepared_) mirror_chained_++;
        prepared_id_ = chained_id_;
        prepared_from_ = chained_from_;
        prepared_samples_ = chained_samples_;
        chained_id_ = nil();
    }
    size_t chained_id_ = nil(), chained_from_ = nil(), chained_samples_ = 0;
    std::mutex hint_mutex_;
    std::optional<MirrorHint> hint_;

    struct MirrorPacket {
        struct Link {
            uint32_t ki, kj;
            Track *ft_track;
            bool trash;
        };
        size_t from_id = nil(), frame_id = nil();
        bool valid = false;
        std::unique_ptr<Frame> frame;
        std::vector<Link> links;
    };
    size_t newest_frame_id() const {
        const Frame *keyframe = map->get_frame(map->frame_num() - 1);
        return keyframe->subframes.empty() ? keyframe->id : keyframe->subframes.back()->id;
    }
    static MirrorPacket make_mirror_packet(Map *ft_map, size_t frame_id, size_t from_id) {
        MirrorPacket pk;
// ... 1871 lines not shown
```

Measured before the change: 1697.

## Keep marginalisation prior resident on device and reuse it in solves

After marginalisation, the prior (sqrt info, infovec, linearisation point) and its precomputed lambda/c0 now stay in a double-buffered device slot. A handle to that slot is armed on the next BA solve and the next marginalisation, so the host no longer re-uploads the prior matrices and the prior-lambda kernel is not relaunched on each solve. Cross-context use is ordered by a stream wait on an event. Host staging vectors are also kept as reusable per-context scratch to avoid per-call allocations. The cost is extra validation (a memcmp of lin) and slot lifetime and ordering complexity between the marg and solve contexts.

```diff
diff --git a/include/xrslam_hip.h b/include/xrslam_hip.h
--- a/include/xrslam_hip.h
+++ b/include/xrslam_hip.h
@@ -211,6 +211,9 @@
                          double *out_infovec, double *out_lin);
 int xrhip_ba_marginalize_begin(xrhip_ba *ctx, const xrhip_marg_problem *problem);
 int xrhip_ba_marginalize_end(xrhip_ba *ctx, double *out_sqrt_info, double *out_infovec, double *out_lin);
+typedef struct xrhip_ba_prior xrhip_ba_prior;
+int xrhip_ba_marginalize_prior_handle(xrhip_ba *ctx, const xrhip_ba_prior **out);
+int xrhip_ba_use_device_prior(xrhip_ba *ctx, const xrhip_ba_prior *prior);
 int xrhip_ba_preintegrate(xrhip_ba *ctx, const double *samples, int n, double t_end, const double *bg,
                           const double *ba, const double *noise_cov36, int compute_jacobian,
                           int compute_covariance, double *out);
diff --git a/xrslam_amd/abi.py b/xrslam_amd/abi.py
--- a/xrslam_amd/abi.py
+++ b/xrslam_amd/abi.py
@@ -55,6 +55,15 @@
         ("n_obs", C.c_int), ("obs_tgt", _ip), ("obs_ref", _ip), ("obs_lm", _ip),
         ("obs_z_tgt", _dp), ("obs_z_ref", _dp),
     ]
+
+
+def declare_device_prior(lib):
+    if hasattr(lib, "xrhip_ba_use_device_prior"):
+        lib.xrhip_ba_marginalize_prior_handle.argtypes = [C.c_void_p, C.POINTER(C.c_void_p)]
+        lib.xrhip_ba_marginalize_prior_handle.restype = C.c_int
+        lib.xrhip_ba_use_device_prior.argtypes = [C.c_void_p, C.c_void_p]
+        lib.xrhip_ba_use_device_prior.restype = C.c_int
+    return lib
 
 
 def _arr(a, dtype):
diff --git a/xrslam_amd/ba.py b/xrslam_amd/ba.py
--- a/xrslam_amd/ba.py
+++ b/xrslam_amd/ba.py
@@ -50,6 +50,7 @@
         lib.xrhip_ba_debug_set_schur_precision.argtypes = [vp, C.c_int]
     if hasattr(lib, "xrhip_ba_debug_last_route"):
         lib.xrhip_ba_debug_last_route.argtypes = [vp, vp]
+    abi.declare_device_prior(lib)
     return lib
 
 
@@ -195,6 +196,14 @@
         lin = np.zeros((k, 16))
         check(self._lib.xrhip_ba_marginalize_end(self._h, _p(si), _p(iv), _p(lin)))
         return si, iv, lin
+
+    def prior_handle(self):
+        h = C.c_void_p()
+        check(self._lib.xrhip_ba_marginalize_prior_handle(self._h, C.byref(h)))
+        return h
+
+    def use_device_prior(self, handle):
+        check(self._lib.xrhip_ba_use_device_prior(self._h, handle))
 
     def preintegrate(self, samples, t_end, bg, ba, noise36, jac=True, cov=True):
         samples = np.ascontiguousarray(samples, np.float64).reshape(-1, 7)
diff --git a/xrslam_amd/csrc/ba_api.hip b/xrslam_amd/csrc/ba_api.hip
--- a/xrslam_amd/csrc/ba_api.hip
+++ b/xrslam_amd/csrc/ba_api.hip
@@ -2,6 +2,7 @@
 #include "ba_kernels.hip.h"
 #include "ba_chain.hip.h"
 #include "ba_plan.hpp"
+#include "ba_prior.hpp"
 #include "marg_kernels.hip.h"
 #include "cov_kernels.hip.h"
 #include "host/covariance.hpp"
@@ -56,7 +57,30 @@
     size_t lds_lin = 0, lds_solve = 0, lds_wide = 0;
 };
 
-}
+struct StageScratch {
+    struct Item {
+        size_t off;
+        const void *src;
+        size_t bytes;
+    };
+    std::vector<uint8_t> lact;
+    std::vector<int> lm_start, lm_obs, fill, pair_start, pair_items, rotf_start, rotf_items, act_idx, act_inv, imuf, priorf;
+    std::vector<double> bias_ref;
+    std::vector<Item> items;
+};
+
+}
+
+struct xrhip_ba_prior {
+    xrhip_ba *owner = nullptr;
+    bool valid = false;
+    int NP = 0, np = 0;
+    char *dev = nullptr;
+    size_t cap = 0;
+    double *pS = nullptr, *pinfo = nullptr, *plin = nullptr, *pLam = nullptr, *pc0 = nullptr;
+    std::vector<double> lin;
+    hipEvent_t ready = nullptr;
+};
 
 struct xrhip_ba {
     hipStream_t stream = nullptr;
@@ -97,6 +121,12 @@
         double *lam = nullptr;
         double *As = nullptr, *bs = nullptr, *B = nullptr, *V = nullptr, *Ss = nullptr, *ivs = nullptr, *dsi = nullptr, *div = nullptr;
     } marg;
+    xrhip_ba_prior slot[2];
+    int slot_next = 0;
+    xrhip_ba_prior *slot_filling = nullptr;
+    const xrhip_ba_prior *slot_last = nullptr;
+    const xrhip_ba_prior *armed = nullptr;
+    StageScratch scratch;
     int preint_pending = 0;
     size_t preint_o_out = 0, preint_o_st = 0;
     int preint_deferred = 0, preint_def_jac = 0, preint_def_cov = 0;
@@ -342,7 +372,13 @@
 } g_register_ba_launchers;
 }
 
-static int stage_problem(xrhip_ba *c, const xrhip_ba_problem *P, BaDims &d, SolvePlan &pl, BaPtrs &p, Ext &cam, Ext &imu, bool defer_copy = false) {
+static int stage_problem(xrhip_ba *c, const xrhip_ba_problem *P, BaDims &d, SolvePlan &pl, BaPtrs &p, Ext &cam, Ext &imu, bool defer_copy = false,
+                         const xrhip_ba_prior *dp = nullptr) {
+    if (dp)
+        if (const char *why = device_prior_mismatch(dp->valid, dp->NP, dp->lin.data(), P->prior_n, P->prior_lin)) {
+            std::snprintf(xr_err_buf(), 512, "xrhip_ba_use_device_prior: %s", why);
+            return XRHIP_EINVAL;
+        }
     d.F = P->n_frames;
     d.n = 15 * d.F;
     d.PF = round_up(6 * d.F, 16);
@@ -358,18 +394,24 @@
     d.schur_mode = c->schur_mode;
     const int F = d.F, L = d.L, M = d.M, MR = d.MR, NI = d.NI, NP = d.NP, np = d.np, n = d.n;
 
-    std::vector<uint8_t> lact(std::max(L, 1), 0);
+    StageScratch &sc = c->scratch;
+    std::vector<uint8_t> &lact = sc.lact;
+    lact.assign(std::max(L, 1), 0);
     for (int o = 0; o < M; ++o) lact[P->obs_lm[o]] = 1;
     for (int l = 0; l < L; ++l)
         if (P->landmark_fix && P->landmark_fix[l]) lact[l] = 0;
-    std::vector<int> lm_start(L + 1, 0), lm_obs(std::max(M, 1));
+    std::vector<int> &lm_start = sc.lm_start, &lm_obs = sc.lm_obs, &fill = sc.fill;
+    lm_start.assign(L + 1, 0);
+    lm_obs.resize(std::max(M, 1));
     for (int o = 0; o < M; ++o) lm_start[P->obs_lm[o] + 1]++;
     for (int l = 0; l < L; ++l) lm_start[l + 1] += lm_start[l];
     {
-        std::vector<int> fill(lm_start.begin(), lm_start.end() - 1);
+        fill.assign(lm_start.begin(), lm_start.end() - 1);
         for (int o = 0; o < M; ++o) lm_obs[fill[P->obs_lm[o]]++] = o;
     }
-    std::vector<int> pair_start((size_t)F * F + 1, 0), pair_items(std::max(4 * M, 1));
+    std::vector<int> &pair_start = sc.pair_start, &pair_items = sc.pair_items;
+    pair_start.assign((size_t)F * F + 1, 0);
+    pair_items.resize(std::max(4 * M, 1));
     auto pair_count = [&](int a, int b) { pair_start[(size_t)a * F + b + 1]++; };
     for (int o = 0; o < M; ++o) {
         const int t = P->obs_tgt[o], r = P->obs_ref[o];
@@ -380,7 +422,7 @@
     }
     for (size_t i = 0; i < (size_t)F * F; ++i) pair_start[i + 1] += pair_start[i];
     {
-        std::vector<int> fill(pair_start.begin(), pair_start.end() - 1);
+        fill.assign(pair_start.begin(), pair_start.end() - 1);
         for (int o = 0; o < M; ++o) {
             const int t = P->obs_tgt[o], r = P->obs_ref[o];
             pair_items[fill[(size_t)t * F + t]++] = (o << 1) | 0;
@@ -389,20 +431,23 @@
             pair_items[fill[(size_t)r * F + t]++] = (o << 1) | 1;
         }
     }
-    std::vector<int> rotf_start(F + 1, 0), rotf_items(std::max(MR, 1));
+    std::vector<int> &rotf_start = sc.rotf_start, &rotf_items = sc.rotf_items;
+    rotf_start.assign(F + 1, 0);
+    rotf_items.resize(std::max(MR, 1));
     for (int o = 0; o < MR; ++o) rotf_start[P->rot_tgt[o] + 1]++;
     for (int f = 0; f < F; ++f) rotf_start[f + 1] += rotf_start[f];
     {
-        std::vector<int> fill(rotf_start.begin(), rotf_start.end() - 1);
+        fill.assign(rotf_start.begin(), rotf_start.end() - 1);
         for (int o = 0; o < MR; ++o) rotf_items[fill[P->rot_tgt[o]]++] = o;
     }
-    std::vector<int> act_idx;
+    std::vector<int> &act_idx = sc.act_idx, &act_inv = sc.act_inv;
+    act_idx.clear();
     for (int a = 0; a < 15 * F; ++a) {
         const int f = a / 15, k = a % 15;
         if (k < 6 ? !(P->frame_fix[f] & XRHIP_FIX_POSE) : !(P->frame_fix[f] & XRHIP_FIX_MOTION)) act_idx.push_back(a);
     }
     d.na = (int)act_idx.size();
-    std::vector<int> act_inv((size_t)15 * F, -1);
+    act_inv.assign((size_t)15 * F, -1);
     for (size_t i = 0; i < act_idx.size(); ++i) act_inv[act_idx[i]] = (int)i;
     d.nla = 0;
     for (int l = 0; l < L; ++l) d.nla += lact[l] ? 1 : 0;
@@ -412,7 +457,9 @@
     d.nffp = 0;
     for (int o = 0; o < M; ++o)
         d.nffp += (!(P->frame_fix[P->obs_tgt[o]] & XRHIP_FIX_POSE) && !(P->frame_fix[P->obs_ref[o]] & XRHIP_FIX_POSE)) ? 1 : 0;
-    std::vector<int> imuf(2 * F, -1), priorf(F, -1);
+    std::vector<int> &imuf = sc.imuf, &priorf = sc.priorf;
+    imuf.assign(2 * F, -1);
+    priorf.assign(F, -1);
     for (int k = 0; k < NI; ++k) {
         if (imuf[2 * P->imu_j[k]] >= 0 || imuf[2 * P->imu_i[k] + 1] >= 0)
             return xr_fail(XRHIP_EINVAL, "xrhip_ba_solve: a frame may end at most one IMU factor and start at most one");
@@ -423,18 +470,16 @@
 
     Arena &A = c->in;
     A.used = 0;
-    struct Item {
-        size_t off;
-        const void *src;
-        size_t bytes;
-    };
-    std::vector<Item> items;
+    using Item = StageScratch::Item;
+    std::vector<Item> &items = sc.items;
+    items.clear();
     auto put = [&](const void *src, size_t bytes) {
         size_t off = A.take(std::max(bytes, size_t(8)));
         items.push_back({off, src, bytes});
         return off;
     };
-    std::vector<double> bias_ref((size_t)6 * std::max(NI, 1));
+    std::vector<double> &bias_ref = sc.bias_ref;
+    bias_ref.resize((size_t)6 * std::max(NI, 1));
     for (int k = 0; k < NI; ++k)
         for (int i = 0; i < 6; ++i) bias_ref[6 * k + i] = P->frame_state[16 * P->imu_i[k] + 10 + i];
     BaCtl ctl;
@@ -459,9 +504,9 @@
     const size_t o_idata = put(P->imu_data, sizeof(double) * XRHIP_IMU_DIM * NI);
     const size_t o_bref = put(bias_ref.data(), sizeof(double) * 6 * NI);
     const size_t o_pf = put(P->prior_frames, sizeof(int) * NP);
-    const size_t o_pS = put(P->prior_sqrt_info, sizeof(double) * (size_t)np * np);
-    const size_t o_pi = put(P->prior_infovec, sizeof(double) * np);
-    const size_t o_pl = put(P->prior_lin, sizeof(double) * 16 * NP);
+    const size_t o_pS = dp ? 0 : put(P->prior_sqrt_info, sizeof(double) * (size_t)np * np);
+    const size_t o_pi = dp ? 0 : put(P->prior_infovec, sizeof(double) * np);
+    const size_t o_pl = dp ? 0 : put(P->prior_lin, sizeof(double) * 16 * NP);
     const size_t o_lms = put(lm_start.data(), sizeof(int) * (L + 1)), o_lmo = put(lm_obs.data(), sizeof(int) * M);
     const size_t o_ps = put(pair_start.data(), sizeof(int) * ((size_t)F * F + 1));
     const size_t o_pit = put(pair_items.data(), sizeof(int) * 4 * M);
@@ -522,11 +567,20 @@
     p.imu_data = (const double *)(I + o_idata);
     p.bias_ref = (double *)(I + o_bref);
     p.prior_frames = (const int *)(I + o_pf);
-    p.pS = (const double *)(I + o_pS);
-    p.pinfo = (const double *)(I + o_pi);
-    p.plin = (const double *)(I + o_pl);
-    p.pLam = (double *)(W + w_pLam);
-    p.pc0 = (double *)(W + w_pc0);
+    if (dp) {
+        p.pS = dp->pS;
+        p.pinfo = dp->pinfo;
+        p.plin = dp->plin;
+        p.pLam = dp->pLam;
+        p.pc0 = dp->pc0;
+        if (dp->owner != c) XR_HIP(hipStreamWaitEvent(c->stream, dp->ready, 0));
+    } else {
+        p.pS = (const double *)(I + o_pS);
+        p.pinfo = (const double *)(I + o_pi);
+        p.plin = (const double *)(I + o_pl);
+        p.pLam = (double *)(W + w_pLam);
+        p.pc0 = (double *)(W + w_pc0);
+    }
     p.lm_start = (const int *)(I + o_lms);
     p.lm_obs = (const int *)(I + o_lmo);
     p.pair_start = (const int *)(I + o_ps);
@@ -830,6 +884,10 @@
         if (e) hipEventDestroy(e);
     if (c->ev_mid) hipEventDestroy(c->ev_mid);
     if (c->ev_marg) hipEventDestroy(c->ev_marg);
+    for (xrhip_ba_prior &h : c->slot) {
+        if (h.ready) hipEventDestroy(h.ready);
+        hipFree(h.dev);
+    }
     if (c->ev_spec) hipEventDestroy(c->ev_spec);
     if (c->stream2) hipStreamDestroy(c->stream2);
     hipFree(c->in.dev);
@@ -852,11 +910,13 @@
 static int preint_launch_deferred(xrhip_ba *c, const xrhip_ba_problem *P, const double *state_dev);
 static int preint_fill_deferred(xrhip_ba *c, const xrhip_ba_problem *P, const double *state_dev, PreintArgs *out, bool *have);
 
-static int ba_solve_impl(xrhip_ba *c, const xrhip_ba_problem *P, xrhip_ba_summary *summary);
+static int ba_solve_impl(xrhip_ba *c, const xrhip_ba_problem *P, xrhip_ba_summary *summary, const xrhip_ba_prior *dp);
 int xrhip_ba_solve(xrhip_ba *c, const xrhip_ba_problem *P, xrhip_ba_summary *summary) {
     if (!c) return xr_fail(XRHIP_EINVAL, "xrhip_ba_solve: null context");
+    const xrhip_ba_prior *dp = c->armed;
+    c->armed = nullptr;
     if (c->begun.active) return xr_fail(XRHIP_ESTATE, "xrhip_ba_solve: a solve begun on this context has not been collected (xrhip_ba_solve_end)");
-    const int rc = ba_solve_impl(c, P, summary);
+    const int rc = ba_solve_impl(c, P, summary, dp);
     if (rc) c->preint_deferred = 0;
     return rc;
 }
@@ -1099,7 +1159,7 @@
     return rc ? rc : rc1;
 }
 
-static int ba_solve_impl(xrhip_ba *c, const xrhip_ba_problem *P, xrhip_ba_summary *summary) {
+static int ba_solve_impl(xrhip_ba *c, const xrhip_ba_problem *P, xrhip_ba_summary *summary, const xrhip_ba_prior *dp) {
     int rc = validate(P);
     if (rc) return rc;
     rc = preint_deferred_check(c, P);
@@ -1132,7 +1192,7 @@
     const auto t_begin = std::chrono::steady_clock::now();
     {
         HostProfScope hp(8, "ba_solve: stage_problem");
-        rc = stage_problem(c, P, d, pl, p, cam, imu, true);
+        rc = stage_problem(c, P, d, pl, p, cam, imu, true, dp);
     }
     if (rc) return rc;
     HostProfScope hp_rounds(9, "ba_solve: rounds (launch+wait)");
@@ -1157,7 +1217,7 @@
     if (!d.nla) d.lm_rows = 0;
     const double sx = P->sqrt_inv_cov[0], sy = P->sqrt_inv_cov[1];
     hipStream_t s = c->stream;
-    if (d.np && !wbatch) hipLaunchKernelGGL(kb_prior_lambda, dim3(((d.np + 15) / 16) * ((d.np + 15) / 16 + 1)), dim3(256), 0, s, d.np, p.pS, p.pLam, p.pinfo, p.pc0);
+    if (d.np && !wbatch && !dp) hipLaunchKernelGGL(kb_prior_lambda, dim3(((d.np + 15) / 16) * ((d.np + 15) / 16 + 1)), dim3(256), 0, s, d.np, p.pS, p.pLam, p.pinfo, p.pc0);
     bool done = false, relinearise = true;
     bool wfirst = true;
     hipStream_t wstream = wbatch ? group_stream(c->group, GQ_WINDOW) : nullptr;
@@ -1170,7 +1230,7 @@
         wp.relin = relinearise;
         wp.with_stage = wfirst;
         wp.stage = StageArgs{c->stage_src, c->stage_dst, c->stage_n16};
-        wp.np = d.np;
+        wp.np = dp ? 0 : d.np;
         wp.pS = p.pS;
         wp.pLam = p.pLam;
         wp.pinfo = p.pinfo;
@@ -1566,10 +1626,41 @@
     return XRHIP_OK;
 }
 
+static int slot_layout(xrhip_ba *c, xrhip_ba_prior &h, int NP) {
+    const PriorSlotLayout lay = prior_slot_layout(NP);
+    const size_t bytes = lay.bytes;
+    if (bytes > h.cap) {
+        if (h.dev) hipFree(h.dev);
+        h.dev = nullptr;
+        h.cap = 0;
+        XR_HIP(hipMalloc(&h.dev, bytes));
+        h.cap = bytes;
+    }
+    if (!h.ready) XR_HIP(hipEventCreateWithFlags(&h.ready, hipEventDisableTiming));
+    h.owner = c;
+    h.valid = false;
+    h.NP = NP;
+    h.np = 15 * NP;
+    h.pS = (double *)(h.dev + lay.pS);
+    h.pLam = (double *)(h.dev + lay.pLam);
+    h.pinfo = (double *)(h.dev + lay.pinfo);
+    h.pc0 = (double *)(h.dev + lay.pc0);
+    h.plin = (double *)(h.dev + lay.plin);
+    return XRHIP_OK;
+}
+static int slot_lambda(const xrhip_ba_prior &h, hipStream_t s) {
+    if (h.np) hipLaunchKernelGGL(kb_prior_lambda, dim3(((h.np + 15) / 16) * ((h.np + 15) / 16 + 1)), dim3(256), 0, s, h.np, h.pS, h.pLam, h.pinfo, h.pc0);
+    XR_HIP(hipGetLastError());
+    XR_HIP(hipEventRecord(h.ready, s));
+    return XRHIP_OK;
+}
+
 extern "C" {
 
 
 static int marg_launch(xrhip_ba *c, const xrhip_marg_problem *M) {
+    const xrhip_ba_prior *dp = c->armed;
+    c->armed = nullptr;
     if (c->marg.pending) return xr_fail(XRHIP_ESTATE, "xrhip_ba_marginalize: a marginalisation is already in flight");
     if (M->n_frames < 2 || M->victim < 0 || M->victim >= M->n_frames)
         return xr_fail(XRHIP_EINVAL, "xrhip_ba_marginalize: bad frame count / victim");
@@ -1613,12 +1704,17 @@
     SolvePlan pl;
     BaPtrs p;
     Ext cam, imu;
-    rc = stage_problem(c, &P, d, pl, p, cam, imu);
+    rc = stage_problem(c, &P, d, pl, p, cam, imu, false, dp);
     if (rc) return rc;
     d.robust = 0;
     d.schur_mode = 0;
     const int N = d.n, R = N - 15;
     if (R > 512) return xr_fail(XRHIP_EINVAL, "xrhip_ba_marginalize: window too large");
+    const int half = prior_slot_half_to_fill(c->slot_next, dp == &c->slot[0] ? 0 : dp == &c->slot[1] ? 1 : -1);
+    xrhip_ba_prior &out = c->slot[half];
+    if (c->slot_last == &out) c->slot_last = nullptr;
+    rc = slot_layout(c, out, K - 1);
+    if (rc) return rc;
     const size_t D8 = sizeof(double);
     size_t w = 0;
     auto carve = [&](size_t bytes) {
@@ -1628,7 +1724,7 @@
     };
     const size_t o_Hm = carve(D8 * (size_t)N * N), o_bm = carve(D8 * N), o_T2 = carve(D8 * (size_t)R * 15);
     const size_t o_A = carve(D8 * (size_t)R * R), o_bp = carve(D8 * R), o_B = carve(D8 * (size_t)R * R);
-    const size_t o_V = carve(D8 * (size_t)R * R), o_si = carve(D8 * (size_t)R * R), o_iv = carve(D8 * R);
+    const size_t o_V = carve(D8 * (size_t)R * R);
     const size_t o_st = carve(sizeof(int) * 8), o_lam = carve(D8 * 2), o_sup = carve(sizeof(int) * (size_t)R);
     const size_t o_As = carve(D8 * (size_t)R * R), o_bs = carve(D8 * R), o_Ss = carve(D8 * (size_t)R * R), o_ivs = carve(D8 * R);
     rc = ensure_work2(c, w + 256, D8 * ((size_t)R * R + R) + 64 + sizeof(int) * 8);
@@ -1636,11 +1732,11 @@
     char *W2 = c->work2;
     double *Hm = (double *)(W2 + o_Hm), *bm = (double *)(W2 + o_bm), *T2 = (double *)(W2 + o_T2);
     double *A = (double *)(W2 + o_A), *bp = (double *)(W2 + o_bp), *B = (double *)(W2 + o_B), *V = (double *)(W2 + o_V);
-    double *dsi = (double *)(W2 + o_si), *div = (double *)(W2 + o_iv);
+    double *dsi = out.pS, *div = out.pinfo;
     int *dst = (int *)(W2 + o_st);
     hipStream_t s = c->stream;
     XR_HIP(hipMemsetAsync(dst, 0, sizeof(int) * 8, s));
-    if (d.np) hipLaunchKernelGGL(kb_prior_lambda, dim3(((d.np + 15) / 16) * ((d.np + 15) / 16 + 1)), dim3(256), 0, s, d.np, p.pS, p.pLam, p.pinfo, p.pc0);
+    if (d.np && !dp) hipLaunchKernelGGL(kb_prior_lambda, dim3(((d.np + 15) / 16) * ((d.np + 15) / 16 + 1)), dim3(256), 0, s, d.np, p.pS, p.pLam, p.pinfo, p.pc0);
     launch_linearize(c, d, pl, p, cam, imu, M->sqrt_inv_cov[0], M->sqrt_inv_cov[1], false);
     hipLaunchKernelGGL(km_omega, dim3((std::max(d.L, 1) + 255) / 256), dim3(256), 0, s, d, p);
     const int tiles = d.PF / 16;
@@ -1660,6 +1756,15 @@
     hipLaunchKernelGGL(km_jacobi, dim3(1), dim3(1024), (size_t)c->lds_limit, s, dst + 5, lds_doubles, As, bs, B, V, Ss, ivs, 60, dst + 2,
                        dsup, R, dsi, div);
     XR_HIP(hipGetLastError());
+    {
+        const double *st_dev = static_cast<const double *>(p.state);
+        const int v = M->victim;
+        if (v > 0) XR_HIP(hipMemcpyAsync(out.plin, st_dev, D8 * 16 * (size_t)v, hipMemcpyDeviceToDevice, s));
+        if (v < K - 1)
+            XR_HIP(hipMemcpyAsync(out.plin + 16 * (size_t)v, st_dev + 16 * (size_t)(v + 1), D8 * 16 * (size_t)(K - 1 - v), hipMemcpyDeviceToDevice, s));
+        rc = slot_lambda(out, s);
+        if (rc) return rc;
+    }
     XR_HIP(hipMemcpyAsync(hs, dsi, D8 * (size_t)R * R, hipMemcpyDeviceToHost, s));
     XR_HIP(hipMemcpyAsync(hs + (size_t)R * R, div, D8 * R, hipMemcpyDeviceToHost, s));
     XR_HIP(hipMemcpyAsync(hs + (size_t)R * R + R, dst, sizeof(int) * 8, hipMemcpyDeviceToHost, s));
@@ -1682,6 +1787,8 @@
     mp.ivs = ivs;
     mp.dsi = dsi;
     mp.div = div;
+    c->slot_filling = &out;
+    c->slot_next = half ^ 1;
     return XRHIP_OK;
 }
 
@@ -1689,6 +1796,9 @@
     xrhip_ba::MargPending &mp = c->marg;
     if (!mp.pending) return xr_fail(XRHIP_ESTATE, "xrhip_ba_marginalize_end: nothing in flight");
     mp.pending = false;
+    xrhip_ba_prior *filled = c->slot_filling;
+    c->slot_filling = nullptr;
+    c->slot_last = nullptr;
     hipStream_t s = c->stream;
     const size_t D8 = sizeof(double);
     const int R = mp.R, K = mp.K;
@@ -1710,6 +1820,10 @@
                            mp.ivs, 60, mp.dst + 2);
         hipLaunchKernelGGL(km_expand, dim3((R * R + 255) / 256), dim3(256), 0, s, R, mp.dsup, dsn, mp.Ss, mp.ivs, mp.dsi, mp.div);
         XR_HIP(hipGetLastError());
+        if (filled) {
+            const int rc = slot_lambda(*filled, s);
+            if (rc) return rc;
+        }
         XR_HIP(hipMemcpyAsync(hs, mp.dsi, D8 * (size_t)R * R, hipMemcpyDeviceToHost, s));
         XR_HIP(hipMemcpyAsync(hs + (size_t)R * R, mp.div, D8 * R, hipMemcpyDeviceToHost, s));
         XR_HIP(hipStreamSynchronize(s));
@@ -1722,6 +1836,11 @@
         std::memcpy(out_lin + 16 * (size_t)j, mp.lin.data() + 16 * (size_t)i, D8 * 16);
         ++j;
     }
+    if (filled) {
+        filled->lin.assign(out_lin, out_lin + 16 * (size_t)(K - 1));
+        filled->valid = true;
+        c->slot_last = filled;
+    }
     return XRHIP_OK;
 }
 
@@ -1741,6 +1860,25 @@
 int xrhip_ba_marginalize_end(xrhip_ba *c, double *out_sqrt_info, double *out_infovec, double *out_lin) {
     if (!c || !out_sqrt_info || !out_infovec || !out_lin) return xr_fail(XRHIP_EINVAL, "xrhip_ba_marginalize_end: null argument");
     return marg_collect(c, out_sqrt_info, out_infovec, out_lin);
+}
+
+int xrhip_ba_marginalize_prior_handle(xrhip_ba *c, const xrhip_ba_prior **out) {
+    if (!c || !out) return xr_fail(XRHIP_EINVAL, "xrhip_ba_marginalize_prior_handle: null argument");
+    *out = nullptr;
+    if (c->marg.pending) return xr_fail(XRHIP_ESTATE, "xrhip_ba_marginalize_prior_handle: the marginalisation has not been collected (xrhip_ba_marginalize_end)");
+    if (!c->slot_last) return xr_fail(XRHIP_ESTATE, "xrhip_ba_marginalize_prior_handle: no marginalisation has left a prior on this context");
+    *out = c->slot_last;
+    return XRHIP_OK;
+}
+
+int xrhip_ba_use_device_prior(xrhip_ba *c, const xrhip_ba_prior *prior) {
+    if (!c) return xr_fail(XRHIP_EINVAL, "xrhip_ba_use_device_prior: null context");
+    c->armed = nullptr;
+    if (!prior) return XRHIP_OK;
+    if (!prior->owner || !prior->valid) return xr_fail(XRHIP_EINVAL, "xrhip_ba_use_device_prior: the handle holds no prior");
+    if (prior->owner->device != c->device) return xr_fail(XRHIP_EINVAL, "xrhip_ba_use_device_prior: the prior lies on another device");
+    c->armed = prior;
+    return XRHIP_OK;
 }
 
 static int preint_stage(xrhip_ba *c, const double *samples, const int *sample_begin, const int *sample_count,
diff --git a/xrslam_amd/csrc/ba_prior.hpp b/xrslam_amd/csrc/ba_prior.hpp
--- /dev/null
+++ b/xrslam_amd/csrc/ba_prior.hpp
@@ -0,0 +1,27 @@
+#pragma once
+#include <cstddef>
+#include <cstring>
+
+namespace xrhip {
+
+struct PriorSlotLayout {
+    size_t pS, pLam, pinfo, pc0, plin, bytes;
+};
+inline PriorSlotLayout prior_slot_layout(int NP) {
+    const size_t np = 15 * (size_t)NP, D8 = sizeof(double);
+    auto up = [](size_t b) { return (b + 255) & ~size_t(255); };
+    const size_t b_mat = up(D8 * np * np), b_vec = up(D8 * np);
+    return PriorSlotLayout{0, b_mat, 2 * b_mat, 2 * b_mat + b_vec, 2 * b_mat + 2 * b_vec, 2 * b_mat + 2 * b_vec + up(D8 * 16 * (size_t)NP)};
+}
+
+inline int prior_slot_half_to_fill(int next, int armed_half) { return armed_half == next ? next ^ 1 : next; }
+
+inline const char *device_prior_mismatch(bool valid, int NP, const double *lin, int prior_n, const double *prior_lin) {
+    if (!valid) return "the handle holds no prior";
+    if (prior_n != NP) return "the problem's prior_n is not the frame count of the device prior";
+    if (prior_lin && NP > 0 && std::memcmp(prior_lin, lin, sizeof(double) * 16 * (size_t)NP) != 0)
+        return "the problem's prior_lin is not the linearisation point of the device prior";
+    return nullptr;
+}
+
+}
diff --git a/xrslam_amd/csrc/host/map.hpp b/xrslam_amd/csrc/host/map.hpp
--- a/xrslam_amd/csrc/host/map.hpp
+++ b/xrslam_amd/csrc/host/map.hpp
@@ -216,6 +216,7 @@
     std::vector<double> sqrt_info;
     std::vector<double> infovec;
     bool pending = false;
+    const xrhip_ba_prior *device = nullptr;
 };
 
 class Map {
diff --git a/xrslam_amd/csrc/host/pipeline.hpp b/xrslam_amd/csrc/host/pipeline.hpp
--- a/xrslam_amd/csrc/host/pipeline.hpp
+++ b/xrslam_amd/csrc/host/pipeline.hpp
@@ -39,6 +39,8 @@
                             const uint8_t *palette_bgr, int n_palette, void *out, int stride_bytes, int channels, int on_device) __attribute__((weak));
 int xrhip_klt_set_lk_params(xrhip_klt *ctx, const xrhip_lk_params *p) __attribute__((weak));
 int xrhip_ba_covariance(xrhip_ba *ctx, const xrhip_ba_problem *problem, const xrhip_cov_request *req) __attribute__((weak));
+int xrhip_ba_marginalize_prior_handle(xrhip_ba *ctx, const xrhip_ba_prior **out) __attribute__((weak));
+int xrhip_ba_use_device_prior(xrhip_ba *ctx, const xrhip_ba_prior *prior) __attribute__((weak));
 }
 
 namespace xrh {
@@ -690,6 +692,10 @@
     prior->infovec.swap(iv);
     prior->lin.swap(lin);
     prior->pending = false;
+    static const bool host_prior = std::getenv("XRSLAM_AMD_HOST_PRIOR") != nullptr;
+    prior->device = nullptr;
+    if (!host_prior && xrhip_ba_marginalize_prior_handle && xrhip_ba_use_device_prior)
+        hip_check(xrhip_ba_marginalize_prior_handle(P.ba_marg, &prior->device), "xrhip_ba_marginalize_prior_handle");
 }
 
 class BaBuilder {
@@ -928,6 +934,7 @@
         WallTimer wt_w_solve(P_.times.w_solve);
         if (chain_f_ && chain_f_->ba_gen == gen_)
             chain_queued_ = P_.integrate_after_solve_begin(chain_samples_, chain_t_, chain_f_->ba_index, true, true);
+        if (prior_ && prior_->device) hip_check(xrhip_ba_use_device_prior(P_.ba, prior_->device), "xrhip_ba_use_device_prior");
         if (overlap) {
             const int rc = xrhip_ba_solve_overlapped(P_.ba, &pb_, &sm, &Overlap::trampoline, overlap);
             overlap->run();
@@ -1180,7 +1187,10 @@
     {
         WallTimer wt_w_marginalize(P.times.w_marginalize);
         static const bool sync_launch = std::getenv("XRSLAM_AMD_SYNC_MARG_LAUNCH") != nullptr;
+        const xrhip_ba_prior *dev_prior = prior->device;
+        prior->device = nullptr;
         if (sync_launch) {
+            if (dev_prior) hip_check(xrhip_ba_use_device_prior(P.ba_marg, dev_prior), "xrhip_ba_use_device_prior");
             hip_check(xrhip_ba_marginalize_begin(P.ba_marg, &mp), "xrhip_ba_marginalize_begin");
         } else {
             if (!P.marg_launcher) {
@@ -1189,7 +1199,10 @@
                 P.marg_launcher = std::make_unique<JobThread>(dev);
             }
             xrhip_ba *ctx = P.ba_marg;
-            P.marg_launcher->post([ctx, job] { hip_check(xrhip_ba_marginalize_begin(ctx, &job->mp), "xrhip_ba_marginalize_begin"); });
+            P.marg_launcher->post([ctx, job, dev_prior] {
+                if (dev_prior) hip_check(xrhip_ba_use_device_prior(ctx, dev_prior), "xrhip_ba_use_device_prior");
+                hip_check(xrhip_ba_marginalize_begin(ctx, &job->mp), "xrhip_ba_marginalize_begin");
+            });
             P.marg_launch_pending = true;
         }
     }
```

New measurement: 1692. No clear change (-0.3%).
